# fnzhan/EMLight

Hardware: AMD Instinct MI355X
Metric: training images/sec (regression step: DenseNet-BC fwd + Sinkhorn loss + bwd + Adam) (higher is better)
Workload: dtype f32; 1 GPU; RegressionNetwork train step, BASELINE configs[1]; per_gpu_batch=64, global_batch=64, anchors=128, parallelism=single

## Files before the change

### emlight_amd/RegressionNetwork/dense_engine_bwd.py

```python
import ctypes
import os

import torch

from .. import _lib
from .._knobs import knob_choice, knob_flag


def _r16(v):
    return (v + 15) // 16 * 16


def _side_stream(dev, prio):
    if prio <= 0:
        return torch.cuda.Stream(device=dev, priority=prio)
    hip = ctypes.CDLL("libamdhip64.so")
    h = ctypes.c_void_p()
    with torch.cuda.device(dev):
        rc = hip.hipStreamCreateWithPriority(ctypes.byref(h), ctypes.c_uint(1), ctypes.c_int(prio))
    if rc != 0:
        raise RuntimeError("hipStreamCreateWithPriority failed (%d)" % rc)
    return torch.cuda.ExternalStream(h.value, device=dev)


def _masked_stream(dev, n_cu, keep):
    hip = ctypes.CDLL("libamdhip64.so")
    words = (n_cu + 31) // 32
    mask = (ctypes.c_uint32 * words)()
    for i in range(n_cu):
        if keep(i):
            mask[i // 32] |= 1 << (i % 32)
    h = ctypes.c_void_p()
    with torch.cuda.device(dev):
        rc = hip.hipExtStreamCreateWithCUMask(ctypes.byref(h), ctypes.c_uint32(words), mask)
    if rc != 0:
        raise RuntimeError("hipExtStreamCreateWithCUMask failed (%d)" % rc)
    return torch.cuda.ExternalStream(h.value, device=dev)


class _BwdBuffers:
    def gf12(self, r):
        if self.GF12[r] is None:
            self.GF12[r] = self._gf12_new()
        return self.GF12[r]

    def __init__(self, enc, ws, dev):
        f32 = dict(dtype=torch.float32, device=dev)
        self.G = [torch.zeros(blk["P"], blk["ld"], **f32) for blk in ws.blocks]
        self.GF = torch.zeros(ws.F.shape[0], ws.F.shape[1], **f32)
        maxP = ws.blocks[0]["P"]
        self.DZ = torch.empty(2, maxP, 48, **f32)
        self.ring = max(1, int(os.environ.get("EML_WGRAD_RING", 4))) if enc.overlap_wgrad(dev) else 1
        self.GF12 = [None] * self.ring
        self._gf12_new = lambda: torch.empty(maxP, 12, **f32)
        self.N12 = torch.empty(maxP, 12, **f32)
        self.TOP = torch.empty(2 * maxP * 12, **f32) if knob_flag("EML_DGRAD_TOP", True) else None
        kp, ko, g = enc.kp_max, max(enc.ko_max, 48), enc.grid_max
        self.Wd = [[torch.empty(lay["Kp"] * 48, **f32) for lay in blk["layers"]] for blk in ws.blocks]
        self.WdT = [torch.empty(blk["trans"]["Kp"] * blk["trans"]["Ko"], **f32) for blk in ws.blocks]
        self.permutes = None
        self.coef = torch.zeros(8, max(kp, ko), **f32)
        self.part2 = torch.zeros(2, g * kp * 2, dtype=torch.float64, device=dev)
        self.partW = torch.empty(g * max(kp * 48, 2 * 27 * 256, 4 * 1024), **f32)
        i32 = dict(dtype=torch.int32, device=dev)
        self.cond = [[torch.zeros(lay["Kp"], **i32) for lay in blk["layers"]] for blk in ws.blocks]
        self.condT = [torch.zeros(blk["trans"]["Kp"], **i32) for blk in ws.blocks]
        self.any_ill = torch.zeros(1, **i32)
        self.dg_grid = 128
        self.dg_scratch = torch.empty(self.dg_grid * kp, dtype=torch.float64, device=dev)
        self.side = None
        if enc.overlap_wgrad(dev):
            m = int(os.environ.get("EML_CU_SPLIT", 0))
            self.main_masked = None
            if m > 1:
                n_cu = torch.cuda.get_device_properties(dev).multi_processor_count
                self.side = _masked_stream(dev, n_cu, lambda i: i % m == m - 1)
                self.main_masked = _masked_stream(dev, n_cu, lambda i: i % m != m - 1)
            else:
                self.side = _side_stream(dev, int(os.environ.get("EML_SIDE_PRIO", 0)))
            self.partW3 = [torch.empty(g * 2 * 27 * 256, **f32) for _ in range(self.ring)]
            self.ev_ready = [torch.cuda.Event() for _ in range(self.ring)]
            self.ev_done = [None] * self.ring


def run_backward(enc, ws, x, gpooled, need_x=False, need_params=None):
    if getattr(ws, "bwd", None) is None:
        ws.bwd = _BwdBuffers(enc, ws, x.device)
    masked = getattr(ws.bwd, "main_masked", None)
    if masked is None:
        return _run_backward(enc, ws, x, gpooled, need_x, need_params)
    cur = torch.cuda.current_stream(x.device)
    masked.wait_stream(cur)
    with torch.cuda.stream(masked):
        out = _run_backward(enc, ws, x, gpooled, need_x, need_params)
    cur.wait_stream(masked)
    return out


def _run_backward(enc, ws, x, gpooled, need_x, need_params):
    L, p, st = _lib.lib(), _lib.ptr, _lib.current_stream()
    m = enc.model
    f = m.features
    if not m.training:
        raise NotImplementedError("HIP DenseNet backward is implemented for train-mode BatchNorm "
                                  "(EMLight trains and tests in train mode, train.py:42 / test.py:36-37)")
    dev = x.device
    B, _, H, W = x.shape
    G = enc._grid(dev)
    G3 = enc._grid3(dev)
    G3d = enc._tuned("EML_GRID3_DGRAD", 2 * G3 if knob_flag("EML_D3_SHORT", False) else G3)
    Gw = enc._tuned("EML_GRID_WGRAD1", G)
    Gd = enc._tuned("EML_GRID_DGRAD", G)
    Gb = min(enc.grid_max, 4 * enc._cu)
    bw = ws.bwd
    part = ws.partials
    ring = [0]
    if bw.side is not None:
        main = torch.cuda.current_stream(dev)
        st_side = ctypes.c_void_p(bw.side.cuda_stream)
        G3s = enc._tuned("EML_GRID3_SIDE", G3)
        bw.side.wait_stream(main)
    if bw.permutes is None:
        from .dense_engine import _PermuteTable
        bw.permutes = _PermuteTable()
    items = []
    for bi_, blk_ in enumerate(ws.blocks):
        mod_ = getattr(f, "denseblock%d" % (bi_ + 1))
        for l_, lay_ in enumerate(blk_["layers"]):
            items.append((getattr(mod_, "denselayer%d" % (l_ + 1)).conv1.weight, bw.Wd[bi_][l_], 2, 48, lay_["Cin"],
                          lay_["Kp"], 48))
        tr_ = blk_["trans"]
        items.append((getattr(f, "transition%d" % (bi_ + 1)).conv.weight, bw.WdT[bi_], 2, tr_["Cout"], blk_["Ctot"],
                      tr_["Kp"], tr_["Ko"]))
    bw.permutes.launch(L, st, items)
    params = enc.param_list()
    if need_params is None:
        need_params = [True] * len(params)
    from .._dist import grad_slot
    grads = {}
    for q, need in zip(params, need_params):
        slot = grad_slot(q) if need else None
        grads[id(q)] = slot if slot is not None else torch.empty_like(q)
    gr = lambda q: p(grads[id(q)])
    coefs = [tuple(bw.coef[3 * k + i] for i in range(3)) for k in range(2)]
    cA, cB, cC = coefs[0]
    sB, sC = bw.coef[6], bw.coef[7]

    direct = knob_choice("EML_DGAMMA_DIRECT", "always", ("always", "never")) != "never"
    c3_fold = knob_flag("EML_C3_FOLD", True)
    c3_gf = knob_flag("EML_C3_GF", False)
    bw.any_ill.zero_()

    def dgamma_direct(blk, X_ld, Pin, Hin, Win, pool, DY, ld_dy, Zr, ld_z, co, Cout, conv, Cin, scale1, shift1, cond, bn):
        if not direct:
            return
        a, b, c = co if co is not None else (None, None, None)
        _lib.check(L.eml_dense_bn_dgamma_direct_f32(
            p(blk["X"]), X_ld, Pin, Hin, Win, pool, p(DY), ld_dy, p(Zr), ld_z, p(a), p(b), p(c), Cout, p(conv.weight), Cin,
            p(scale1), p(shift1), p(blk["mean"]), p(blk["istd"]), p(cond), p(bw.dg_scratch), gr(bn.weight), bw.dg_grid, st),
            "eml_dense_bn_dgamma_direct_f32")

    def finalize(R, pstride, count, bn, mean, istd, C, Cpad, coef=0, s_acc=None, src=None, c_lo=0, c_hi=None, conv=None,
                 cond=None):
        a, b, c = coefs[coef] if coef is not None else (None, None, None)
        wargs = (p(bn.bias), p(conv.weight), gr(conv.weight), conv.weight.shape[0]) if conv is not None else (None, None, None, 0)
        _lib.check(L.eml_dense_bn_bwd_finalize_f32(
            p(part if src is None else src), R, pstride, float(count), p(bn.weight), p(mean), p(istd), C, Cpad, 1,
            gr(bn.weight), gr(bn.bias), p(a), p(b), p(c),
            p(sB) if s_acc is not None else None, p(sC) if s_acc is not None else None, int(bool(s_acc)),
            c_lo, Cpad if c_hi is None else c_hi, *wargs, p(cond), p(bw.any_ill) if cond is not None else None, st),
            "eml_dense_bn_bwd_finalize_f32")

    def parr(tensors):
        return (ctypes.c_void_p * len(tensors))(*[t.data_ptr() for t in tensors])

    def materialize(Gbuf, blk, c0, n):
        _lib.check(L.eml_dense_grad_materialize_f32(p(Gbuf), blk["ld"], p(blk["X"]), blk["ld"], p(sB), p(sC), c0, n,
                                                    blk["P"], st), "eml_dense_grad_materialize_f32")

    cf, k = enc.trans_cout[-1], enc.avgpool
    ldF = ws.F.shape[1]
    _lib.check(L.eml_dense_head_pool_bwd_f32(p(gpooled), p(ws.F), ldF, cf, B, ws.hf, ws.wf, k, p(bw.GF), ldF, st),
               "eml_dense_head_pool_bwd_f32")
    dY, ld_dy = bw.GF, ldF
    nb = len(ws.blocks)
    for bi in reversed(range(nb)):
        blk, tr = ws.blocks[bi], ws.blocks[bi]["trans"]
        mod = getattr(f, "denseblock%d" % (bi + 1))
        T, LN = getattr(f, "transition%d" % (bi + 1)), getattr(f, "last_norm%d" % (bi + 1))
        P, Hb, Wb, ld, ctot = blk["P"], blk["H"], blk["W"], blk["ld"], blk["Ctot"]
        cout, Ko, kpt = tr["Cout"], tr["Ko"], tr["Kp"]
        Pn = B * (Hb // 2) * (Wb // 2)
        Gbuf = bw.G[bi]
        gl0 = sum(enc.block_layers[:bi])
        top2 = bw.TOP[:2 * P * 12].view(2, P, 12) if bw.TOP is not None else None
        _lib.check(L.eml_dense_bn_bwd_stats_f32(p(dY), ld_dy, p(tr["T"]), Ko, None, 0, 0, cout, Pn, p(tr["tmean"]),
                                                p(tr["tistd"]), p(part), Gb, st), "eml_dense_bn_bwd_stats_f32")
        finalize(Gb, 2 * cout, Pn, LN, tr["tmean"], tr["tistd"], cout, Ko, coef=0)
        _lib.check(L.eml_dense_conv1x1_bwd_weight_f32(
            p(tr["A"]), kpt, Pn, Hb // 2, Wb // 2, 0, kpt, ctot, p(tr["one"]), p(tr["zero"]), p(dY), ld_dy, p(tr["T"]),
            Ko, p(cA), p(cB), p(cC), cout, p(bw.partW), gr(T.conv.weight), G, None, None, 0, None, 0, None, None, st),
            "eml_dense_conv1x1_bwd_weight_f32")
        _lib.check(L.eml_dense_conv1x1_bwd_data_f32(
            p(dY), ld_dy, p(tr["T"]), Ko, p(cA), p(cB), p(cC), Ko, p(bw.WdT[bi]), None, ld, p(tr["scale"]),
            p(tr["shift"]), None, None, Pn, Hb, Wb, 1, kpt, p(Gbuf), ld, 0, p(part), G, p(tr["mask16"]), st),
            "eml_dense_conv1x1_bwd_data_f32")
        finalize(G, 2 * kpt, P, T.norm, blk["mean"], blk["istd"], ctot, kpt, coef=None, s_acc=False, conv=T.conv,
                 cond=bw.condT[bi])
        dgamma_direct(blk, ld, P, Hb, Wb, 1, dY, ld_dy, tr["T"], Ko, coefs[0], cout, T.conv, ctot, tr["scale"], tr["shift"],
                      bw.condT[bi], T.norm)
        def conv2_backward(l, slot, n12=False, narrow_lo=None, top=False):
            lay = blk["layers"][l]
            Lm = getattr(mod, "denselayer%d" % (l + 1))
            cin, kp, z, dz = lay["Cin"], lay["Kp"], blk["Z"][l], bw.DZ[slot]
            gsrc = (p(bw.N12), 12, 0) if n12 else (p(top2[1]), 12, 0) if top else (p(Gbuf), ld, cin)
            r = ring[0] = (ring[0] + 1) % bw.ring
            if bw.side is not None and bw.ev_done[r] is not None:
                main.wait_event(bw.ev_done[r])
            fold = (bw.side is None and c3_fold
                    and L.eml_dense_conv3x3_bwd_fused_supported(gsrc[1], gsrc[2], ld, cin) == 1)
            q = ws.drop_plan[bi][l] if ws.drop_plan is not None else 0.0
            drop = (ws.drop_key, gl0 + l, q) if q > 0 else ()
            if fold:
                fn = "eml_dense_conv3x3_bwd_fused_drop_f32" if drop else "eml_dense_conv3x3_bwd_fused_f32"
                _lib.check(getattr(L, fn)(*gsrc, p(Lm.conv2.weight), p(z), p(lay["zmean"]), p(lay["zistd"]), p(dz), B, Hb, Wb,
                                          p(part), G3d, p(blk["X"]), ld, cin, p(sB), p(sC), p(bw.gf12(r)) if c3_gf else None,
                                          p(lay["scale2"]), p(lay["shift2"]), p(bw.partW), gr(Lm.conv2.weight), *drop, st), fn)
            else:
                fn = "eml_dense_conv3x3_bwd_data_drop_f32" if drop else "eml_dense_conv3x3_bwd_data_f32"
                _lib.check(getattr(L, fn)(*gsrc, p(Lm.conv2.weight), p(z), p(lay["zmean"]), p(lay["zistd"]), p(dz), B, Hb, Wb,
                                          p(part), G3d, p(blk["X"]), ld, cin, p(sB), p(sC), p(bw.gf12(r)), *drop, st), fn)
            if fold:
                pass
            elif bw.side is None:
                _lib.check(L.eml_dense_conv3x3_bwd_weight_f32(p(bw.gf12(r)), 12, 0, p(z), p(lay["scale2"]),
                                                              p(lay["shift2"]), B, Hb, Wb, p(bw.partW),
                                                              gr(Lm.conv2.weight), G3, st),
                           "eml_dense_conv3x3_bwd_weight_f32")
            else:
                bw.ev_ready[r].record(main)
                bw.side.wait_event(bw.ev_ready[r])
                _lib.check(L.eml_dense_conv3x3_bwd_weight_f32(p(bw.gf12(r)), 12, 0, p(z), p(lay["scale2"]),
                                                              p(lay["shift2"]), B, Hb, Wb, p(bw.partW3[r]),
                                                              gr(Lm.conv2.weight), G3s, st_side),
                           "eml_dense_conv3x3_bwd_weight_f32")
                if bw.ev_done[r] is None:
                    bw.ev_done[r] = torch.cuda.Event()
                bw.ev_done[r].record(bw.side)
            finalize(G3d, 96, P, Lm.norm2, lay["zmean"], lay["zistd"], 48, 48, coef=slot)
            a, b, c = coefs[slot]
            _lib.check(L.eml_dense_conv1x1_bwd_weight_f32(
                p(blk["X"]), ld, P, Hb, Wb, 0, kp, cin, p(lay["scale1"]), p(lay["shift1"]), p(dz), 48, p(z), 48,
                p(a), p(b), p(c), 48, p(bw.partW), gr(Lm.conv1.weight), Gw, p(dz),
                *((p(Lm.conv1.weight), narrow_lo, *((p(top2[0]), 12) if top else (p(Gbuf), ld)), p(bw.N12),
                   p(bw.part2[slot])) if narrow_lo is not None
                  else (None, 0, None, 0, None, None)), st), "eml_dense_conv1x1_bwd_weight_f32")
            return Lm

        def dgrad(layers, slots, k_lo, k_hi, top=False):
            lays = [blk["layers"][l] for l in layers]
            if top:
                _lib.check(L.eml_dense_conv1x1_bwd_data_multi_top_f32(
                    parr([bw.DZ[s_] for s_ in slots]), parr([bw.Wd[bi][l_] for l_ in layers]),
                    parr([y["scale1"] for y in lays]), parr([y["shift1"] for y in lays]),
                    parr([bw.part2[s_] for s_ in slots]), (ctypes.c_int * len(layers))(*[y["Kp"] for y in lays]),
                    P, k_hi, p(Gbuf), ld, Gd, parr([y["mask"] for y in lays]), p(top2), st),
                    "eml_dense_conv1x1_bwd_data_multi_top_f32")
                return
            _lib.check(L.eml_dense_conv1x1_bwd_data_multi_f32(
                len(layers), parr([bw.DZ[s_] for s_ in slots]), None, None, None, None,
                parr([bw.Wd[bi][l_] for l_ in layers]),
                parr([y["scale1"] for y in lays]), parr([y["shift1"] for y in lays]),
                parr([bw.part2[s_] for s_ in slots]), (ctypes.c_int * len(layers))(*[y["Kp"] for y in lays]),
                None, ld, None, None, P, k_lo, k_hi, p(Gbuf), ld, Gd,
                parr([y["mask"] for y in lays]), st),
                "eml_dense_conv1x1_bwd_data_multi_f32")

        def bn1_finalize(l, Lm, slot, c_lo, c_hi, rows=None):
            lay = blk["layers"][l]
            finalize(Gd if rows is None else rows, 2 * lay["Kp"], P, Lm.norm1, blk["mean"], blk["istd"], lay["Cin"], lay["Kp"], coef=None,
                     s_acc=True, src=bw.part2[slot], c_lo=c_lo, c_hi=c_hi, conv=Lm.conv1, cond=bw.cond[bi][l])

        def bn1_direct(l, Lm, slot):
            lay = blk["layers"][l]
            dgamma_direct(blk, ld, P, Hb, Wb, 0, bw.DZ[slot], 48, None, 0, None, 48, Lm.conv1, lay["Cin"], lay["scale1"],
                          lay["shift1"], bw.cond[bi][l], Lm.norm1)

        l = len(blk["layers"]) - 1
        have_top = False
        while l >= 0:
            if l >= 1:
                la, lb = l, l - 1
                cin_a, cin_b = blk["layers"][la]["Cin"], blk["layers"][lb]["Cin"]
                Lma = conv2_backward(la, 0, narrow_lo=cin_b, top=have_top)
                bn1_finalize(la, Lma, 0, cin_b, cin_a, rows=Gw)
                Lmb = conv2_backward(lb, 1, n12=True)
                to_top = (top2 is not None and lb >= 2 and blk["layers"][la]["mask"] is not None and bw.side is None
                          and cin_b >= 24 and cin_b % 4 == 0)
                dgrad([la, lb], [0, 1], 0, cin_b, top=to_top)
                have_top = to_top
                bn1_finalize(la, Lma, 0, 0, cin_b)
                bn1_finalize(lb, Lmb, 1, 0, blk["layers"][lb]["Kp"])
                bn1_direct(la, Lma, 0)
                bn1_direct(lb, Lmb, 1)
                l -= 2
            else:
                Lm0 = conv2_backward(l, 0)
                dgrad([l], [0], 0, blk["layers"][l]["Cin"])
                bn1_finalize(l, Lm0, 0, 0, blk["layers"][l]["Kp"])
                bn1_direct(l, Lm0, 0)
                l -= 1
        c0b = blk["C0"]
        norm0_fused = bi == 0 and knob_flag("EML_NORM0_FUSED", True) and c0b % 4 == 0 and c0b <= 32
        if not norm0_fused:
            materialize(Gbuf, blk, 0, c0b)
        dY, ld_dy = Gbuf, ld
    b0 = ws.blocks[0]
    c0 = enc.c_init
    if norm0_fused:
        _lib.check(L.eml_dense_norm0_bwd_stats_f32(p(dY), ld_dy, p(ws.Y0), c0, p(ws.scale0), p(ws.shift0), p(sB), p(sC), c0,
                                                   b0["P"], p(ws.mean0), p(ws.istd0), p(part), Gb, st),
                   "eml_dense_norm0_bwd_stats_f32")
    else:
        _lib.check(L.eml_dense_bn_bwd_stats_f32(p(dY), ld_dy, p(ws.Y0), c0, p(b0["X"]), b0["ld"], 1, c0, b0["P"],
                                                p(ws.mean0), p(ws.istd0), p(part), Gb, st), "eml_dense_bn_bwd_stats_f32")
    finalize(Gb, 2 * c0, b0["P"], f.norm0, ws.mean0, ws.istd0, c0, _r16(c0), coef=0)
    if norm0_fused:
        _lib.check(L.eml_dense_conv0_bwd_weight_fused_f32(p(x), p(dY), ld_dy, p(ws.Y0), c0, p(ws.scale0), p(ws.shift0), p(sB),
                                                          p(sC), p(cA), p(cB), p(cC), B, H, W, p(bw.partW),
                                                          gr(f.conv0.weight), G, st), "eml_dense_conv0_bwd_weight_fused_f32")
    else:
        _lib.check(L.eml_dense_conv0_bwd_weight_f32(p(x), p(dY), ld_dy, p(b0["X"]), b0["ld"], p(ws.Y0), c0, p(cA), p(cB),
                                                    p(cC), B, H, W, p(bw.partW), gr(f.conv0.weight), G, st),
                   "eml_dense_conv0_bwd_weight_f32")
    dx = None
    if need_x:
        dx = torch.empty(B, 3, H, W, dtype=torch.float32, device=dev)
        X1 = (None, 0) if norm0_fused else (p(b0["X"]), b0["ld"])
        _lib.check(L.eml_dense_conv0_bwd_data_f32(p(dY), ld_dy, *X1, p(ws.Y0), c0, p(ws.scale0), p(ws.shift0), p(sB), p(sC),
                                                  p(cA), p(cB), p(cC), p(f.conv0.weight), B, H, W, p(dx), st),
                   "eml_dense_conv0_bwd_data_f32")
    if bw.side is not None:
        main.wait_stream(bw.side)
    return dx, [grads[id(q)] for q in params]
```

### emlight_amd/_lib.py

```python
import ctypes
import os
import threading

_HERE = os.path.dirname(os.path.abspath(__file__))
LIB_PATH = os.environ.get("EML_LIB_PATH") or os.path.join(_HERE, "libemlight_hip.so")

_f32p = ctypes.c_void_p
_i32p = ctypes.c_void_p
_f64p = ctypes.c_void_p
_stream = ctypes.c_void_p
_int = ctypes.c_int
_u64 = ctypes.c_ulonglong

ABI_VERSION = 31

SIGNATURES = {
    "eml_abi_version": (_int, []),
    "eml_last_error": (ctypes.c_char_p, []),
    "eml_sg_rasterise_f32": (_int, [_f32p, _f32p, _f32p, _f32p, _int, _int, _int, _int, _stream]),
    "eml_sg_rasterise_ex_f32": (_int, [_f32p, _f32p, _f32p, _f32p, _int, _int, _int, _int, _int, ctypes.c_void_p, _stream]),
    "eml_sg_rasterise_bwd_colors_f32": (_int, [_f32p, _f32p, _f32p, _f32p, _int, _int, _int, _int, _stream]),
    "eml_emd_anchor_cost_f32": (_int, [_f32p, _f32p, _int, _stream]),
    "eml_sinkhorn_schedule_f32": (_int, [_f32p, _f32p, ctypes.c_long, ctypes.c_double, ctypes.c_double, _int,
                                         ctypes.c_double, _f32p, _f32p, _i32p, _f32p, _stream]),
    "eml_sinkhorn_work_floats": (ctypes.c_size_t, [_int, _int]),
    "eml_sinkhorn_fwd_f32": (_int, [_f32p, _f32p, _f32p, _f32p, _f32p, _f32p, ctypes.c_double, ctypes.c_double, _int,
                                    ctypes.c_double, _f32p, _f32p, _i32p, _f32p, _f32p, _f32p, _f32p, _f32p, _int, _int,
                                    _stream]),
    "eml_sinkhorn_fwd_ex_f32": (_int, [_f32p, _f32p, _f32p, _f32p, _f32p, _f32p, ctypes.c_double, ctypes.c_double, _int,
                                       ctypes.c_double, _f32p, _f32p, _i32p, _f32p, _f32p, _f32p, _f32p, _f32p, _int, _int,
                                       _int, _stream]),
    "eml_sinkhorn_fwd_rho_f32": (_int, [_f32p, _f32p, _f32p, _f32p, _f32p, _f32p, ctypes.c_double, ctypes.c_double, _int,
                                        ctypes.c_double, _f32p, _f32p, _i32p, _f32p, _f32p, _f32p, _f32p, _f32p, _int, _int,
                                        _int, ctypes.c_double, _f32p, _stream]),
    "eml_sinkhorn_bwd_f32": (_int, [_f32p, _f32p, _f32p, _int, _int, _stream]),
    "eml_sinkhorn_dim_work_floats": (ctypes.c_size_t, [_int, _int, _int]),
    "eml_sinkhorn_fwd_dim_f32": (_int, [_f32p, _f32p, _f32p, _f32p, _f32p, _f32p, ctypes.c_double, ctypes.c_double, _int,
                                        ctypes.c_double, _f32p, _f32p, _i32p, _f32p, _f32p, _f32p, _f32p, _f32p, _int, _int,
                                        _int, _int, ctypes.c_double, _f32p, _stream]),
    "eml_sinkhorn_schedule_dim_f32": (_int, [_f32p, _f32p, ctypes.c_long, _int, ctypes.c_double, ctypes.c_double, _int,
                                             ctypes.c_double, _f32p, _f32p, _i32p, _f32p, _stream]),
    "eml_sinkhorn_bwd_weights_f32": (_int, [_f32p, _f32p, _f32p, _f32p, _int, _int, _stream]),
    "eml_l1_pairs_partial_doubles": (ctypes.c_size_t, [_int]),
    "eml_l1_pairs_fwd_f32": (_int, [_int, ctypes.c_void_p, ctypes.c_void_p, ctypes.c_void_p, ctypes.c_void_p, ctypes.c_void_p,
                                    ctypes.c_void_p, _f64p, _f32p, _stream]),
    "eml_l1_pairs_bwd_f32": (_int, [_int, ctypes.c_void_p, ctypes.c_void_p, ctypes.c_void_p, ctypes.c_void_p, ctypes.c_void_p,
                                    ctypes.c_void_p, _f32p, ctypes.c_void_p, ctypes.c_void_p, ctypes.c_void_p, _stream]),
    "eml_colsum_partial_doubles": (ctypes.c_size_t, [_int]),
    "eml_colsum_f32": (_int, [_f32p, ctypes.c_long, _int, _f64p, _f32p, _stream]),
    "eml_gt_anchor_index_i32": (_int, [_f32p, _int, _int, _int, _i32p, _stream]),
    "eml_gt_parametrise_f64": (_int, [_f32p, _i32p, _i32p, _int, _int, _int, _int, _f32p, _f32p, _f32p, _stream]),
    "eml_pano_crop_f32": (_int, [ctypes.c_void_p, _int, _int, _int, _int, _int, _int, ctypes.c_double, ctypes.c_double, _f64p,
                                 ctypes.c_double, _f64p, _f32p, _stream]),
    "eml_pano_resize_area_f32": (_int, [_f32p, _int, _int, _int, _int, _int, ctypes.c_double, _f64p, _f32p, _stream]),
    "eml_tonemap_work_floats": (ctypes.c_size_t, [_int]),
    "eml_tonemap_f32": (_int, [_f32p, _int, ctypes.c_long, _int, ctypes.c_double, ctypes.c_double, ctypes.c_double, _f32p,
                               _int, _f32p, _f32p, _i32p, _f32p, ctypes.c_void_p, _stream]),
    "eml_sphere_tap_table_f32": (_int, [_f32p, _int, _int, _int, _int, _i32p, _f32p, _stream]),
    "eml_sphere_im2col_f32": (_int, [_f32p, _i32p, _f32p, _f32p, _int, _int, _int, _int, _stream]),
    "eml_sphere_col2im_f32": (_int, [_f32p, _i32p, _i32p, _f32p, _f32p, _int, _int, _int, _int, _stream]),
    "eml_sphere_conv_fwd_fused_f32": (_int, [_f32p, _i32p, _f32p, _f32p, _f32p, _f32p, _int, _int, _int, _int, _int, _int,
                                             _stream]),
    "eml_sphere_conv_fwd_fused_ex_f32": (_int, [_f32p, _i32p, _f32p, _f32p, _f32p, _f32p, _int, _int, _int, _int, _int, _int,
                                                _f32p, ctypes.c_float, _int, _stream]),
    "eml_sphere_conv_small_supported": (_int, [_int, _int]),
    "eml_sphere_conv_small_fwd_f32": (_int, [_f32p, _i32p, _f32p, _f32p, _f32p, _f32p, _int, _int, _int, _int, _int,
                                             ctypes.c_float, _stream]),
    "eml_sphere_conv_small_wgrad_partial_floats": (ctypes.c_size_t, [_int, _int, _int, _int]),
    "eml_sphere_conv_small_wgrad_f32": (_int, [_f32p, _i32p, _f32p, _f32p, _f32p, ctypes.c_float, _f32p, _f32p, _f32p, _int,
                                               _int, _int, _int, _int, _stream]),
    "eml_sphere_conv_small_da9_f32": (_int, [_f32p, _f32p, ctypes.c_float, _f32p, _f32p, ctypes.c_long, _int, _int, _stream]),
    "eml_spade_norm_modulate_up2_fwd_f32": (_int, [_f32p, _f32p, _f32p, _int, _int, _int, _int, ctypes.c_float, _f32p, _f32p,
                                                   _stream]),
    "eml_spade_norm_modulate_bwd_cols_f32": (_int, [_f32p, _f32p, _f32p, _f32p, _f32p, _int, _int, _int, _int, _int,
                                                    ctypes.c_float, _f32p, _f32p, _f32p, _int, _stream]),
    "eml_sg_rasterise_bwd_work_floats": (ctypes.c_size_t, [_int, _int, _int, _int]),
    "eml_sg_rasterise_bwd_colors_ex_f32": (_int, [_f32p, _f32p, _f32p, _f32p, _f32p, _int, _int, _int, _int, _int, _stream]),
    "eml_sg_rasterise_bwd_full_work_floats": (ctypes.c_size_t, [_int, _int, _int, _int]),
    "eml_sg_rasterise_bwd_f32": (_int, [_f32p, _f32p, _f32p, _f32p, _f32p, _f32p, _f32p, _f32p, _int, _int, _int, _int, _int,
                                        _stream]),
    "eml_sphere_conv_narrow_supported": (_int, [_int, _int]),
    "eml_sphere_conv_narrow_fwd_f32": (_int, [_f32p, _i32p, _f32p, _f32p, _f32p, _f32p, _int, _int, _int, _int, _int, _stream]),
    "eml_sphere_conv_narrow_dgrad_f32": (_int, [_f32p, _i32p, _f32p, _int, _f32p, _f32p, _int, _int, _int, _int, _int, _stream]),
    "eml_sphere_conv_narrow_wgrad_partial_floats": (ctypes.c_size_t, [_int, _int, _int, _int]),
    "eml_sphere_conv_narrow_wgrad_f32": (_int, [_f32p, _i32p, _f32p, _f32p, _f32p, _f32p, _int, _int, _int, _int, _int, _stream]),
    "eml_sphere_conv_narrow_scratch_floats": (ctypes.c_size_t, [_int, _int]),
    "eml_sphere_conv_narrow_fwd2_f32": (_int, [_f32p, _i32p, _f32p, _f32p, _f32p, _f32p, _f32p, _int, _int, _int, _int, _int, _stream]),
    "eml_sphere_conv_narrow_wgrad2_partial_floats": (ctypes.c_size_t, [_int, _int, _int]),
    "eml_sphere_conv_narrow_dgrad2_f32": (_int, [_f32p, _i32p, _f32p, _int, ctypes.c_void_p, _f32p, _f32p, _f32p, _int, _int, _int,
                                                 _int, _int, _int, _stream]),
    "eml_sphere_conv_narrow_wgrad2_f32": (_int, [_f32p, _i32p, _f32p, _int, ctypes.c_void_p, _f32p, _f32p, _f32p, _f32p, _int, _int,
                                                 _int, _int, _int, _stream]),
    "eml_sphere_conv_spade_supported": (_int, [_int, _int, ctypes.c_long]),
    "eml_sphere_conv_spade_fwd_f32": (_int, [_f32p, _i32p, _f32p, _f32p, _f32p, _f32p, _f32p, _f32p, _f32p, _f32p, _int, _int,
                                             _int, _int, _int, _int, ctypes.c_float, _int, _stream]),
    "eml_spade_norm_modulate_bwd_y_f32": (_int, [_f32p, _f32p, _f32p, _f32p, _f32p, _f32p, _int, _int, _int, _int, _int,
                                                 ctypes.c_float, _f32p, _f32p, _f32p, _int, _stream]),
    "eml_bn_bwd_apply_up2_f32": (_int, [_f32p, _f32p, _int, _int, _int, _int, _f32p, _f32p, _f32p, _f32p, _stream]),
    "eml_spectral_norm_scratch_floats": (ctypes.c_size_t, [_int, _int]),
    "eml_spectral_norm_w2_f32": (_int, [_f32p, _f32p, _f32p, _int, ctypes.c_float, _f32p, _f32p, _f32p, _f32p, _int, _int,
                                        _stream]),
    "eml_spectral_norm_w2_bwd_f32": (_int, [_f32p, _f32p, _f32p, _f32p, _f32p, _f32p, _f32p, _int, _int, _stream]),
    "eml_spectral_norm_w2_batch_f32": (_int, [_int, ctypes.c_void_p, ctypes.c_void_p, ctypes.c_void_p, _int, ctypes.c_float,
                                              ctypes.c_void_p, ctypes.c_void_p, ctypes.c_void_p, ctypes.c_void_p, ctypes.c_void_p,
                                              ctypes.c_void_p, _stream]),
    "eml_spade_heads_w2_f32": (_int, [_f32p, _f32p, _f32p, _f32p, _f32p, _f32p, _int, _int, _int, _stream]),
    "eml_instance_norm_act_fwd_f32": (_int, [_f32p, _f32p, _f32p, _int, _int, _int, _int, ctypes.c_float, ctypes.c_float,
                                             _stream]),
    "eml_instance_norm_act_bwd_f32": (_int, [_f32p, _f32p, _f32p, _f32p, _int, _int, _int, _int, ctypes.c_float, _stream]),
    "eml_sphere_conv_dgrad_fused_f32": (_int, [_f32p, _i32p, _f32p, _i32p, _int, _f32p, _f32p, _int, _int, _int, _int, _int,
                                               _int, _stream]),
    "eml_sphere_conv_lowres_variant": (_int, [_int, _int, _int, _int]),
    "eml_sphere_conv_lowres_table_i32": (_int, [_i32p, _i32p, _i32p, _int, _int, _stream]),
    "eml_sphere_conv_lowres_partial_floats": (ctypes.c_size_t, [ctypes.c_long, _int, _int]),
    "eml_sphere_conv_lowres_f32": (_int, [_f32p, _i32p, _f32p, _i32p, _int, _i32p, _int, _f32p, _f32p, _f32p, _f32p, _int, _int,
                                          _int, _int, _int, _int, _f32p, ctypes.c_float, _stream]),
    "eml_sphere_conv_wgrad_partial_floats": (ctypes.c_size_t, [_int, _int, _int]),
    "eml_sphere_conv_wgrad_fused_f32": (_int, [_f32p, _i32p, _f32p, _f32p, _f32p, _f32p, _int, _int, _int, _int, _int, _int,
                                               _stream]),
    "eml_spade_modulate_fwd_f32": (_int, [_f32p, _int, _f32p, _int, _f32p, _int, ctypes.c_long, _int, ctypes.c_float,
                                          _stream]),
    "eml_spade_modulate_bwd_f32": (_int, [_f32p, _int, _f32p, _int, _f32p, _int, _f32p, _int, _f32p, _int, ctypes.c_long,
                                          _int, ctypes.c_float, _stream]),
    "eml_bn_stats_f32": (_int, [_f32p, _int, ctypes.c_long, _int, _f32p, _int, _stream]),
    "eml_bn_fold_f64": (_int, [_f32p, _int, _int, _f32p, _stream]),
    "eml_bn_finalize_f32": (_int, [_f32p, _int, ctypes.c_float, ctypes.c_float, _f32p, _f32p, _f32p, _f32p, _stream]),
    "eml_spade_norm_modulate_fwd_f32": (_int, [_f32p, _int, _f32p, _int, _f32p, _int, ctypes.c_long, _int, ctypes.c_float,
                                               _f32p, _f32p, _stream]),
    "eml_bn_bwd_apply_f32": (_int, [_f32p, _int, _f32p, _int, ctypes.c_long, _int, _f32p, _f32p, _f32p, _f32p, _int,
                                    _stream]),
    "eml_dense_conv0_fwd_f32": (_int, [_f32p, _f32p, _f32p, _int, _int, _int, _int, _int, _f32p, _int, _stream]),
    "eml_dense_conv0_fwd_mfma_f32": (_int, [_f32p, _f32p, _f32p, _int, _int, _int, _int, _int, _f32p, _int, _stream]),
    "eml_dense_bn_apply_f32": (_int, [_f32p, _int, _f32p, _int, _int, ctypes.c_long, _f32p, _f32p, _int, _f32p,
                                      _int, _stream]),
    "eml_dense_bn_prepare_f32": (_int, [_f32p, _int, _int, _int, _int, ctypes.c_double, _f32p, _f32p, _f32p, _f32p,
                                        _f32p, _f32p, _f32p, _int, _int, ctypes.c_float, ctypes.c_float, _int,
                                        _f32p, _f32p, _stream]),
    "eml_dense_permute_w1_f32": (_int, [_f32p, _int, _int, _int, _f32p, _stream]),
    "eml_dense_permute_w2_f32": (_int, [_f32p, _int, _f32p, _stream]),
    "eml_dense_permute_batch_f32": (_int, [ctypes.c_void_p, _int, _stream]),
    "eml_dense_conv1x1_fwd_f32": (_int, [_f32p, _int, ctypes.c_long, _int, _int, _int, _int, _f32p, _f32p, _f32p,
                                         _int, _f32p, _int, _f32p, _int, ctypes.c_void_p, _stream]),
    "eml_dense_conv3x3_fwd_f32": (_int, [_f32p, _f32p, _f32p, _f32p, _f32p, _int, _int, _int, _int, _int, _f32p,
                                         _int, _stream]),
    "eml_dense_permute_w2_tp_f32": (_int, [_f32p, _f32p, _stream]),
    "eml_dense_conv3x3_fwd_tp_supported": (_int, [_int, _int, _int]),
    "eml_dense_conv3x3_fwd_tp_f32": (_int, [_f32p, _f32p, _f32p, _f32p, _f32p, _int, _int, _int, _int, _int, _int, _f32p,
                                            _int, _stream]),
    "eml_dense_conv3x3_fwd_drop_f32": (_int, [_f32p, _f32p, _f32p, _f32p, _f32p, _int, _int, _int, _int, _int, _f32p,
                                              _int, _u64, _int, ctypes.c_double, _stream]),
    "eml_dense_conv3x3_fwd_tp_drop_f32": (_int, [_f32p, _f32p, _f32p, _f32p, _f32p, _int, _int, _int, _int, _int, _int, _f32p,
                                                 _int, _u64, _int, ctypes.c_double, _stream]),
    "eml_dense_dropout_mask_u16": (_int, [_u64, _int, ctypes.c_double, ctypes.c_long, ctypes.c_void_p, _stream]),
    "eml_dense_pool_act_f32": (_int, [_f32p, _int, _int, _int, _int, _int, _f32p, _f32p, _f32p, _int, ctypes.c_void_p,
                                      _stream]),
    "eml_dense_head_pool_fwd_f32": (_int, [_f32p, _int, _int, _int, _int, _int, _int, _f32p, _stream]),
    "eml_dense_conv3x3_bwd_data_f32": (_int, [_f32p, _int, _int, _f32p, _f32p, _f32p, _f32p, _f32p, _int, _int, _int,
                                              _f32p, _int, _f32p, _int, _int, _f32p, _f32p, _f32p, _stream]),
    "eml_dense_conv3x3_bwd_fused_supported": (_int, [_int, _int, _int, _int]),
    "eml_dense_conv3x3_bwd_fused_f32": (_int, [_f32p, _int, _int, _f32p, _f32p, _f32p, _f32p, _f32p, _int, _int, _int, _f64p, _int,
                                               _f32p, _int, _int, _f32p, _f32p, _f32p, _f32p, _f32p, _f32p, _f32p, _stream]),
    "eml_dense_conv3x3_bwd_data_drop_f32": (_int, [_f32p, _int, _int, _f32p, _f32p, _f32p, _f32p, _f32p, _int, _int, _int,
                                                   _f32p, _int, _f32p, _int, _int, _f32p, _f32p, _f32p, _u64, _int,
                                                   ctypes.c_double, _stream]),
    "eml_dense_conv3x3_bwd_fused_drop_f32": (_int, [_f32p, _int, _int, _f32p, _f32p, _f32p, _f32p, _f32p, _int, _int, _int,
                                                    _f64p, _int, _f32p, _int, _int, _f32p, _f32p, _f32p, _f32p, _f32p, _f32p,
                                                    _f32p, _u64, _int, ctypes.c_double, _stream]),
    "eml_dense_conv3x3_bwd_weight_f32": (_int, [_f32p, _int, _int, _f32p, _f32p, _f32p, _int, _int, _int, _f32p,
                                                _f32p, _int, _stream]),
    "eml_dense_bn_bwd_finalize_f32": (_int, [_f32p, _int, _int, ctypes.c_double, _f32p, _f32p, _f32p, _int, _int,
                                             _int, _f32p, _f32p, _f32p, _f32p, _f32p, _f32p, _f32p, _int, _int, _int,
                                             _f32p, _f32p, _f32p, _int, _i32p, _i32p, _stream]),
    "eml_dense_bn_dgamma_direct_f32": (_int, [_f32p, _int, ctypes.c_long, _int, _int, _int, _f32p, _int, _f32p, _int,
                                              _f32p, _f32p, _f32p, _int, _f32p, _int, _f32p, _f32p, _f32p, _f32p, _i32p,
                                              _f32p, _f32p, _int, _stream]),
    "eml_dense_conv1x1_bwd_weight_f32": (_int, [_f32p, _int, ctypes.c_long, _int, _int, _int, _int, _int, _f32p,
                                                _f32p, _f32p, _int, _f32p, _int, _f32p, _f32p, _f32p, _int, _f32p,
                                                _f32p, _int, _f32p, _f32p, _int, _f32p, _int, _f32p, _f32p, _stream]),
    "eml_dense_conv1x1_bwd_narrow_f32": (_int, [_f32p, _f32p, _int, _int, _f32p, _int, _f32p, _f32p, _f32p, _f32p,
                                                ctypes.c_long, _f32p, _int, _f32p, _f32p, _int, _int, _stream]),
    "eml_dense_permute_w1_bwd_f32": (_int, [_f32p, _int, _int, _int, _int, _f32p, _stream]),
    "eml_dense_conv1x1_bwd_data_f32": (_int, [_f32p, _int, _f32p, _int, _f32p, _f32p, _f32p, _int, _f32p, _f32p,
                                              _int, _f32p, _f32p, _f32p, _f32p, ctypes.c_long, _int, _int, _int,
                                              _int, _f32p, _int, _int, _f32p, _int, ctypes.c_void_p, _stream]),
    "eml_dense_conv1x1_bwd_data_multi_f32": (_int, [_int] + [ctypes.c_void_p] * 10 + [_f32p, _int, _f32p, _f32p,
                                                    ctypes.c_long, _int, _int, _f32p, _int, _int, ctypes.c_void_p,
                                                    _stream]),
    "eml_dense_conv1x1_bwd_data_multi_top_f32": (_int, [ctypes.c_void_p] * 6 + [ctypes.c_long, _int, _f32p, _int, _int,
                                                        ctypes.c_void_p, _f32p, _stream]),
    "eml_dense_grad_materialize_f32": (_int, [_f32p, _int, _f32p, _int, _f32p, _f32p, _int, _int, ctypes.c_long,
                                              _stream]),
    "eml_dense_bn_bwd_stats_f32": (_int, [_f32p, _int, _f32p, _int, _f32p, _int, _int, _int, ctypes.c_long, _f32p,
                                          _f32p, _f32p, _int, _stream]),
    "eml_dense_norm0_bwd_stats_f32": (_int, [_f32p, _int, _f32p, _int, _f32p, _f32p, _f32p, _f32p, _int, ctypes.c_long, _f32p, _f32p,
                                             ctypes.c_void_p, _int, _stream]),
    "eml_dense_conv0_bwd_weight_fused_f32": (_int, [_f32p, _f32p, _int, _f32p, _int, _f32p, _f32p, _f32p, _f32p, _f32p, _f32p, _f32p,
                                                    _int, _int, _int, _f32p, _f32p, _int, _stream]),
    "eml_dense_conv0_bwd_weight_f32": (_int, [_f32p, _f32p, _int, _f32p, _int, _f32p, _int, _f32p, _f32p, _f32p,
                                              _int, _int, _int, _f32p, _f32p, _int, _stream]),
    "eml_dense_conv0_bwd_data_f32": (_int, [_f32p, _int, _f32p, _int, _f32p, _int, _f32p, _f32p, _f32p, _f32p, _f32p, _f32p,
                                            _f32p, _f32p, _int, _int, _int, _f32p, _stream]),
    "eml_dense_head_pool_bwd_f32": (_int, [_f32p, _f32p, _int, _int, _int, _int, _int, _int, _f32p, _int, _stream]),
}

_lock = threading.Lock()
_lib = None


class EmlightHipError(RuntimeError):
    pass


def lib():
    global _lib
    if _lib is not None:
        return _lib
    with _lock:
        if _lib is not None:
            return _lib
        if not os.path.exists(LIB_PATH):
            raise EmlightHipError(
                "libemlight_hip.so not found at %s -- build it with "
                "`python -c 'import __graft_entry__ as g; g.build()'` or `make -C emlight_amd/csrc`. "
                "There is no CPU fallback." % LIB_PATH)
        handle = ctypes.CDLL(LIB_PATH)
        for name, (res, args) in SIGNATURES.items():
            try:
                fn = getattr(handle, name)
            except AttributeError as e:
                raise EmlightHipError("libemlight_hip.so lacks symbol %s" % name) from e
            fn.restype, fn.argtypes = res, args
        got = handle.eml_abi_version()
        if got != ABI_VERSION:
            raise EmlightHipError("libemlight_hip.so has ABI version %d, this binding expects %d -- rebuild it "
                                  "(make -C emlight_amd/csrc)" % (got, ABI_VERSION))
        _lib = handle
    from . import _gemm_selection
    _gemm_selection.ensure_if_requested()
    return _lib


_DEBUG_SYNC = bool(os.environ.get("EML_DEBUG_SYNC"))


def check(rc, what):
    if rc != 0:
        msg = lib().eml_last_error()
        raise EmlightHipError("%s failed (rc=%d): %s" % (what, rc, msg.decode() if msg else "?"))
    if _DEBUG_SYNC:
        import sys
        import torch
        sys.stderr.write("[eml] %s ... " % what)
        sys.stderr.flush()
        torch.cuda.synchronize()
        sys.stderr.write("ok\n")


def ptr(t):
    if t is None:
        return None
    return ctypes.c_void_p(t.data_ptr())


def current_stream():
    import torch
    return ctypes.c_void_p(torch.cuda.current_stream().cuda_stream)


def require_gpu_tensor(t, name, dtype=None):
    import torch
    if not isinstance(t, torch.Tensor) or not t.is_cuda:
        raise EmlightHipError("%s must be a tensor on the MI355X (got %s); there is no CPU path"
                              % (name, getattr(t, "device", type(t))))
    if t.dtype != (dtype or torch.float32):
        raise EmlightHipError("%s must be %s (got %s)" % (name, dtype or torch.float32, t.dtype))
    return t.contiguous()
```

### emlight_amd/csrc/dense_bwd.hip

```cpp
#include "eml_common.h"
#include "eml_dropout.h"

#include <cstdint>
#include <cstdlib>
#include <type_traits>

namespace {

using f32x4 = __attribute__((ext_vector_type(4))) float;

__device__ __forceinline__ f32x4 mfma16(float a, float b, f32x4 c) {
  return __builtin_amdgcn_mfma_f32_16x16x4f32(a, b, c, 0, 0, 0);
}
__device__ __forceinline__ float f4c(const float4& v, int t) { return t == 0 ? v.x : t == 1 ? v.y : t == 2 ? v.z : v.w; }
__device__ __forceinline__ double shfl_xor_d(double v, int m) { return __shfl_xor(v, m, 64); }

constexpr int kTH = 8, kTW = 32, kHH = kTH + 2, kHW = kTW + 2;

constexpr int kPSG = 14;
constexpr int kBD = 512;
constexpr int kGRows = 2;
constexpr int kGPass = kHH / kGRows;

template <bool FUSE, bool WIDE, int TH, bool DROP = false>
// ... 949 lines not shown
          const int b2 = t2 / (ty_n * tx_n), rem2 = t2 - b2 * (ty_n * tx_n);
#ifndef EML_C3_NOZDMA
#pragma unroll
          for (int it = 0; it < kZI; ++it) z_dma(it, b2, (rem2 / tx_n) * kTH, (rem2 % tx_n) * kTW, cur ^ 1);
#endif
          __builtin_amdgcn_sched_barrier(0);
        }
        const bool pin = 4 * (ks & 7) < (ks < 8 ? xl0 : xl1);
        float bv[3];
#pragma unroll
        for (int n = 0; n < 3; ++n) bv[n] = pin ? fmaf(bz[ks & 1][n], scb[n], shb[n]) : 0.f;
#pragma unroll
        for (int i = 0; i < NT; ++i) {
          const float a = (i < 3 || r < 12) ? av[ks & 1][i] : 0.f;
#pragma unroll
          for (int n = 0; n < 3; ++n) accw[i][n] = mfma16(a, bv[n], accw[i][n]);
        }
        if (ks == 2 || ks == 4 || ks == 6) {
          const int n = (ks - 2) >> 1;
          float l1[4] = {0.f, 0.f, 0.f, 0.f}, l2[4] = {0.f, 0.f, 0.f, 0.f};
#pragma unroll
          for (int m = 0; m < 2; ++m) {
            const float4 z = *reinterpret_cast<const float4*>(zc + (kTW * wave + 16 * m + r) * kZS + 16 * n + 4 * kk);
#pragma unroll
            for (int g = 0; g < 4; ++g) {
              const float v = pv[m] ? acc[m][n][g] : 0.f;
              l1[g] += v;
              l2[g] = fmaf(v, f4c(z, g), l2[g]);
            }
          }
#pragma unroll
          for (int g = 0; g < 4; ++g) {
            const float t1 = eml::row16_sum(l1[g]), t2 = eml::row16_sum(l2[g]);
            if (r == 0) {
              double* d = red + (wave * 48 + 16 * n + 4 * kk + g) * 2;
              d[0] += (double)t1;
              d[1] += (double)t2;
            }
          }
        } else if (ks >= 8 && ks < 14) {
          const int si = ks - 8, m = si / 3, n = si - 3 * m;
          if (pv[m])
            *reinterpret_cast<float4*>(DZ + prow[m] + 16 * n + 4 * kk) =
                make_float4(acc[m][n][0], acc[m][n][1], acc[m][n][2], acc[m][n][3]);
        }
        __builtin_amdgcn_sched_barrier(0);
      }
    };
    if (role == 0) phase_b(std::integral_constant<int, 3>{});
    else phase_b(std::integral_constant<int, 4>{});
    EML_C3_STAMP(2);
    eml::lds_barrier();
    EML_C3_STAMP(3);
#ifdef EML_STAMPS
    st_acc[4] += 1;
#endif
    cur ^= 1;
  }
#ifdef EML_STAMPS
  if (tid == 0)
    for (int i = 0; i < 5; ++i) atomicAdd(&eml_c3_stamps[i], st_acc[i]);
#endif
  asm volatile("s_waitcnt vmcnt(0)" ::: "memory");
  __syncthreads();
  float* wsum = smem;
  for (int w8 = 0; w8 < 8; ++w8) {
    if (wave == w8) {
#pragma unroll
      for (int i = 0; i < 4; ++i)
        if (i < 3 + role) {
#pragma unroll
          for (int n = 0; n < 3; ++n)
#pragma unroll
            for (int g = 0; g < 4; ++g) {
              float* q = wsum + ((((3 * role + i) * 3 + n) * 16 + 4 * kk + g) * 16 + r);
              *q = ((w8 & 3) == 0 ? 0.f : *q) + accw[i][n][g];
            }
        }
    }
    __syncthreads();
  }
  for (int e = tid; e < 21 * 256; e += 512) partialW[(size_t)blockIdx.x * (21 * 256) + e] = wsum[e];
  if (tid < 48) {
    double t1 = 0.0, t2 = 0.0;
#pragma unroll
    for (int w8 = 0; w8 < 8; ++w8) {
      t1 += red[(w8 * 48 + tid) * 2 + 0];
      t2 += red[(w8 * 48 + tid) * 2 + 1];
    }
    partials[(size_t)blockIdx.x * 96 + 2 * tid + 0] = t1;
    partials[(size_t)blockIdx.x * 96 + 2 * tid + 1] = (double)zistd[tid] * (t2 - (double)zmean[tid] * t1);
  }
}


__global__ __launch_bounds__(256) void bn_bwd_finalize_kernel(
    const double* __restrict__ partials, int R, int pstride, double count, const float* __restrict__ gamma,
    const float* __restrict__ mean, const float* __restrict__ istd, int C, int Cpad, int training,
    float* __restrict__ dgamma, float* __restrict__ dbeta, float* __restrict__ cA, float* __restrict__ cB,
    float* __restrict__ cC, float* __restrict__ sB, float* __restrict__ sC, int s_accumulate, int c_lo, int c_hi,
    const float* __restrict__ beta, const float* __restrict__ Wc, const float* __restrict__ dWc, int w_rows,
    int* __restrict__ cond , int* __restrict__ any_cond ) {
  const int lane = threadIdx.x & 63, wave = threadIdx.x >> 6;
  const int c = c_lo + blockIdx.x * 4 + wave;
  if (c >= Cpad || c >= c_hi) return;
  float a = 0.f, b = 0.f, d = 0.f;
  if (c < C) {
    double S1 = 0.0, S2 = 0.0;
    for (int g = lane; g < R; g += 64) {
      S1 += partials[(size_t)g * pstride + 2 * c];
      S2 += partials[(size_t)g * pstride + 2 * c + 1];
    }
    double Q = 0.0;
    if (Wc)
      for (int o = lane; o < w_rows; o += 64) Q += (double)Wc[(size_t)o * C + c] * (double)dWc[(size_t)o * C + c];
#pragma unroll
    for (int o = 32; o > 0; o >>= 1) {
      S1 += __shfl_xor(S1, o, 64);
      S2 += __shfl_xor(S2, o, 64);
      Q += __shfl_xor(Q, o, 64);
    }
    if (Wc) {
      const double ga0 = gamma[c], bs = (double)beta[c] * S1, num = Q - bs;
      S2 = fabs(ga0) >= 1e-12 ? num / ga0 : 0.0;
      if (cond && lane == 0) {
        const int ill = fabs(ga0) < 1e-3 * fabs((double)beta[c]) || ga0 == 0.0;
        cond[c] = ill;
        if (ill && any_cond) *any_cond = 1;
      }
    }
    if (lane == 0) {
      dgamma[c] = (float)S2;
      dbeta[c] = (float)S1;
    }
    const double ga = gamma[c], is = istd[c], mu = mean[c];
    a = (float)(ga * is);
    if (training) {
      b = (float)(-ga * is * is * S2 / count);
      d = (float)(-ga * is * S1 / count + ga * is * is * S2 / count * mu);
    }
  }
  if (lane != 0) return;
  if (cA) {
    cA[c] = a;
    cB[c] = b;
    cC[c] = d;
  }
  if (sB) {
    sB[c] = (s_accumulate ? sB[c] : 0.f) + b;
    sC[c] = (s_accumulate ? sC[c] : 0.f) + d;
  }
}

__global__ __launch_bounds__(256) void reduce_rows_kernel(const float* __restrict__ partial, int R, size_t row_stride,
                                                          int mode, int dim0, int dim1, int n0,
                                                          float* __restrict__ out) {
  __shared__ double red[4][64];
  const int tid = threadIdx.x, e = blockIdx.x * 64 + (tid & 63), slice = tid >> 6;
  size_t src = 0, dst = 0;
  bool valid = false;
  if (mode == 0) {
    const int k = e / 48, o = e - 48 * k;
    valid = k < dim0 && o < dim1;
    src = (size_t)e;
    dst = (size_t)(n0 + o) * dim0 + k;
  } else if (mode == 1) {
    const int o = e & 15, ci = (e >> 4) & 15, pair = e >> 8, tap = pair / 3, mc = pair - 3 * tap;
    valid = pair < 27 && o < 12;
    src = (size_t)e;
    dst = (size_t)(o * 48 + 16 * mc + ci) * 9 + tap;
  } else if (mode == 3) {
    const int j = e & 15, i = (e >> 4) & 15, tn = e >> 8, t = tn / 3, n = tn - 3 * t, row = 16 * t + i;
    valid = tn < 21 && row < 108;
    src = (size_t)e;
    dst = (size_t)((row % 12) * 48 + 16 * n + j) * 9 + row / 12;
  } else {
    const int t = e >> 5, o = e & 31;
    valid = t < 27 && o < dim1;
    src = (size_t)e;
    dst = (size_t)o * 27 + t;
  }
  double s = 0.0;
  if (valid) {
#pragma unroll 8
    for (int r = slice; r < R; r += 4) s += (double)partial[(size_t)r * row_stride + src];
  }
  red[slice][tid & 63] = s;
  __syncthreads();
  if (slice == 0 && valid) out[dst] = (float)((red[0][tid] + red[1][tid]) + (red[2][tid] + red[3][tid]));
}

struct NarrowArgs {
  const float* W1;
  const float* G;
  float* N12;
  double* partials;
  int Cin, k_lo, ldg;
};
template <bool POOL, bool NARROW = false, int VEC = 2>
__global__ __launch_bounds__(256, (NARROW || VEC == 4) ? 2 : 1) void conv1x1_bwd_weight_kernel(
    const float* __restrict__ X, int ldx, int P, int Hin, int Win, int Kp, const float* __restrict__ scale1,
    const float* __restrict__ shift1, const float* __restrict__ DY, int ld_dy, const float* __restrict__ Zr,
    int ld_z, const float* __restrict__ cA, const float* __restrict__ cB, const float* __restrict__ cC, int n_valid,
    int n_load ,
    float* __restrict__ partial ,
    float* __restrict__ dz_out ,
    NarrowArgs na) {
  __shared__ __attribute__((aligned(16))) float dz_l[2][64 * 48];
  const int tid = threadIdx.x, lane = tid & 63, wave = tid >> 6;
  const int r = lane & 15, kk = lane >> 4;
  static_assert(VEC == 2 || (VEC == 4 && !POOL), "float4 operand: dense layers only");
  constexpr int GW = 16 * VEC;
  constexpr int MAXG = VEC == 2 ? 3 : 2;
  const int ngroups = (Kp + GW - 1) / GW;
  float nsk[4] = {0.f, 0.f, 0.f, 0.f}, ntk[4] = {0.f, 0.f, 0.f, 0.f};
  double ns1[4] = {0.0, 0.0, 0.0, 0.0};
  const int kq = min(kk, 2);
  if constexpr (NARROW) {
#pragma unroll
    for (int g = 0; g < 4; ++g) {
      nsk[g] = kk < 3 ? scale1[na.k_lo + 4 * kq + g] : 0.f;
      ntk[g] = kk < 3 ? shift1[na.k_lo + 4 * kq + g] : 0.f;
    }
  }

  float sv[MAXG][VEC], tv[MAXG][VEC];
  int coff[MAXG];
  bool gv[MAXG];
#pragma unroll
  for (int i = 0; i < MAXG; ++i) {
    const int cg = wave + 4 * i;
    const int ch = GW * cg + VEC * r;
    gv[i] = cg < ngroups && ch < Kp;
    coff[i] = gv[i] ? ch : 0;
#pragma unroll
    for (int t = 0; t < VEC; ++t) {
      sv[i][t] = gv[i] ? scale1[ch + t] : 0.f;
      tv[i][t] = gv[i] ? shift1[ch + t] : 0.f;
    }
  }
  const int spix = tid >> 2, sq = tid & 3;
  __shared__ __attribute__((aligned(16))) float co_l[3 * 48];
  __shared__ float wn_l[NARROW ? 12 * 64 : 1];
  constexpr bool CO_LDS = NARROW || VEC == 4;
  float4 sa_r[CO_LDS ? 1 : 3], sb_r[CO_LDS ? 1 : 3], sc_r[CO_LDS ? 1 : 3];
  if constexpr (CO_LDS) {
    if (tid < 48) {
      const bool v = tid < n_valid;
      co_l[tid] = v ? cA[tid] : 0.f;
      co_l[48 + tid] = v ? cB[tid] : 0.f;
      co_l[96 + tid] = v ? cC[tid] : 0.f;
    }
  } else {
#pragma unroll
    for (int j = 0; j < 3; ++j) {
      const int col = 4 * (sq + 4 * j);
      float a[4], b[4], c[4];
#pragma unroll
      for (int e = 0; e < 4; ++e) {
        const bool v = col + e < n_valid;
        a[e] = v ? cA[col + e] : 0.f;
        b[e] = v ? cB[col + e] : 0.f;
        c[e] = v ? cC[col + e] : 0.f;
      }
      sa_r[j] = make_float4(a[0], a[1], a[2], a[3]);
      sb_r[j] = make_float4(b[0], b[1], b[2], b[3]);
      sc_r[j] = make_float4(c[0], c[1], c[2], c[3]);
    }
  }
  if constexpr (NARROW) {
    for (int e = tid; e < 12 * 64; e += 256) {
      const int st = e >> 6, l = e & 63, rr = l & 15, k4 = l >> 4;
      wn_l[e] = rr < 12 ? na.W1[(size_t)(4 * st + k4) * na.Cin + na.k_lo + rr] : 0.f;
    }
  }
  __syncthreads();
  f32x4 acc[MAXG][VEC][3];
#pragma unroll
  for (int i = 0; i < MAXG; ++i)
#pragma unroll
    for (int t = 0; t < VEC; ++t)
#pragma unroll
      for (int n = 0; n < 3; ++n) acc[i][t][n] = f32x4{0.f, 0.f, 0.f, 0.f};

  const int Wo = Win >> 1, Ho = Hin >> 1;
  const int nchunks = (P + 63) >> 6;
  const int ngw = (ngroups > wave) ? (ngroups - wave + 3) >> 2 : 0;

  float4 rdy[3], rzr[3];
  bool rpv = false;
  int rp = 0;
  auto stage_load = [&](int chunk) {
    const int p = chunk * 64 + spix;
    rpv = chunk < nchunks && p < P;
    const size_t pc = rpv ? p : 0;
    rp = (int)pc;
#pragma unroll
    for (int j = 0; j < 3; ++j) {
      const int col = 4 * (sq + 4 * j);
      const bool cv = col < n_load;
      rdy[j] = cv ? *reinterpret_cast<const float4*>(DY + pc * ld_dy + col) : make_float4(0.f, 0.f, 0.f, 0.f);
      rzr[j] = cv ? *reinterpret_cast<const float4*>(Zr + pc * ld_z + col) : make_float4(0.f, 0.f, 0.f, 0.f);
    }
  };
  auto stage_write = [&](float* dzb) {
#pragma unroll
    for (int j = 0; j < 3; ++j) {
      const int col = 4 * (sq + 4 * j);
      float4 sa, sb, sc;
      if constexpr (CO_LDS) {
        sa = *reinterpret_cast<const float4*>(co_l + col);
        sb = *reinterpret_cast<const float4*>(co_l + 48 + col);
        sc = *reinterpret_cast<const float4*>(co_l + 96 + col);
      } else {
        sa = sa_r[j];
        sb = sb_r[j];
        sc = sc_r[j];
      }
      float4 v;
      v.x = rpv ? fmaf(sa.x, rdy[j].x, fmaf(sb.x, rzr[j].x, sc.x)) : 0.f;
      v.y = rpv ? fmaf(sa.y, rdy[j].y, fmaf(sb.y, rzr[j].y, sc.y)) : 0.f;
      v.z = rpv ? fmaf(sa.z, rdy[j].z, fmaf(sb.z, rzr[j].z, sc.z)) : 0.f;
      v.w = rpv ? fmaf(sa.w, rdy[j].w, fmaf(sb.w, rzr[j].w, sc.w)) : 0.f;
      *reinterpret_cast<float4*>(dzb + spix * 48 + col) = v;
      if (dz_out && rpv) *reinterpret_cast<float4*>(dz_out + (size_t)rp * 48 + col) = v;
    }
  };
  auto chunk_loop = [&](auto ngw_c) {
    constexpr int NGW = decltype(ngw_c)::value;
#ifdef EML_WGRAD_DEEP
    constexpr int UQ = POOL ? 1 : 2;
    constexpr int NBUF = POOL ? 2 : 4;
#else
    constexpr int UQ = POOL ? 1 : (VEC == 4 ? 2 : 4);
    constexpr int NBUF = 2;
#endif
    constexpr int NS = POOL ? 4 : 1;
    constexpr int NB = 16 / UQ;
    constexpr int AHEAD = NBUF - 1;
    using xv_t = std::conditional_t<VEC == 2, float2, float4>;
    xv_t xr[NBUF][UQ][NGW > 0 ? NGW : 1][NS];
    auto load_batch = [&](int chunk, int q0, xv_t (&dst)[UQ][NGW > 0 ? NGW : 1][NS]) {
#pragma unroll
      for (int u = 0; u < UQ; ++u) {
        const int pc = min(chunk * 64 + 4 * (q0 + u) + kk, P - 1);
        const float* xp;
        if constexpr (POOL) {
          const int b = pc / (Ho * Wo), rem = pc - b * (Ho * Wo);
          const int oy = rem / Wo, ox = rem - oy * Wo;
          xp = X + ((size_t)(b * Hin + 2 * oy) * Win + 2 * ox) * ldx;
        } else {
          xp = X + (size_t)pc * ldx;
        }
#pragma unroll
        for (int i = 0; i < NGW; ++i)
#pragma unroll
          for (int sub = 0; sub < NS; ++sub)
            dst[u][i][sub] = *reinterpret_cast<const xv_t*>(xp + ((sub >> 1) * (size_t)Win + (sub & 1)) * ldx + coff[i]);
      }
    };
    stage_load(blockIdx.x);
    stage_write(dz_l[0]);
    if constexpr (NGW > 0) {
#pragma unroll
      for (int a = 0; a < AHEAD; ++a) load_batch(min((int)blockIdx.x, nchunks - 1), a * UQ, xr[a]);
    }
    __syncthreads();
    int it = 0;
    for (int chunk = blockIdx.x; chunk < nchunks; chunk += gridDim.x, ++it) {
      const float* dzb = dz_l[it & 1];
      stage_load(chunk + gridDim.x);
      float2 nx[2], ng[2];
      const int pn = chunk * 64 + 16 * wave + r;
      if constexpr (NARROW) {
        const size_t pc = (size_t)min(pn, P - 1);
        const float* xs = X + pc * ldx + na.k_lo + 4 * kq;
        const float* gs = na.G + pc * na.ldg + (na.ldg == 12 ? 0 : na.k_lo) + 4 * kq;
        nx[0] = *reinterpret_cast<const float2*>(xs);
        nx[1] = *reinterpret_cast<const float2*>(xs + 2);
        ng[0] = *reinterpret_cast<const float2*>(gs);
        ng[1] = *reinterpret_cast<const float2*>(gs + 2);
      }
      if constexpr (NGW > 0) {
        float bzq[2][3];
#pragma unroll
        for (int n = 0; n < 3; ++n) bzq[0][n] = dzb[kk * 48 + 16 * n + r];
#pragma unroll
        for (int bi = 0; bi < NB; ++bi) {
          const int q0 = bi * UQ;
          if (bi + AHEAD < NB)
            load_batch(chunk, q0 + AHEAD * UQ, xr[(bi + AHEAD) % NBUF]);
          else
            load_batch(min(chunk + (int)gridDim.x, nchunks - 1), (bi + AHEAD - NB) * UQ, xr[(bi + AHEAD) % NBUF]);
          __builtin_amdgcn_sched_barrier(0);
#pragma unroll
          for (int u = 0; u < UQ; ++u) {
            const int pl = 4 * (q0 + u) + kk;
            const bool pvu = chunk * 64 + pl < P;
            float bz[3];
#pragma unroll
            for (int n = 0; n < 3; ++n) bz[n] = bzq[(q0 + u) & 1][n];
            if (q0 + u + 1 < 16) {
#pragma unroll
              for (int n = 0; n < 3; ++n) bzq[(q0 + u + 1) & 1][n] = dzb[(pl + 4) * 48 + 16 * n + r];
            }
#pragma unroll
            for (int i = 0; i < NGW; ++i) {
              float av[VEC];
#pragma unroll
              for (int t = 0; t < VEC; ++t) av[t] = 0.f;
#pragma unroll
              for (int sub = 0; sub < NS; ++sub) {
                const xv_t xv = xr[bi % NBUF][u][i][sub];
                av[0] += fmaxf(fmaf(xv.x, sv[i][0], tv[i][0]), 0.f);
                av[1] += fmaxf(fmaf(xv.y, sv[i][1], tv[i][1]), 0.f);
                if constexpr (VEC == 4) {
                  av[2] += fmaxf(fmaf(xv.z, sv[i][2], tv[i][2]), 0.f);
                  av[3] += fmaxf(fmaf(xv.w, sv[i][3], tv[i][3]), 0.f);
                }
              }
#pragma unroll
              for (int t = 0; t < VEC; ++t) {
                if constexpr (POOL) av[t] *= 0.25f;
                if (!pvu) av[t] = 0.f;
              }
#pragma unroll
              for (int n = 0; n < 3; ++n)
#pragma unroll
                for (int t = 0; t < VEC; ++t) acc[i][t][n] = mfma16(av[t], bz[n], acc[i][t][n]);
            }
          }
          __builtin_amdgcn_sched_barrier(0);
        }
      }
      if constexpr (NARROW) {
        asm volatile("" ::"v"(ng[0].x), "v"(ng[0].y), "v"(ng[1].x), "v"(ng[1].y), "v"(nx[0].x), "v"(nx[0].y), "v"(nx[1].x), "v"(nx[1].y));
        f32x4 an = f32x4{0.f, 0.f, 0.f, 0.f};
#pragma unroll
        for (int st = 0; st < 12; ++st) an = mfma16(wn_l[st * 64 + lane], dzb[(16 * wave + r) * 48 + 4 * st + kk], an);
        const bool nv = pn < P && kk < 3;
        const float xg[4] = {nx[0].x, nx[0].y, nx[1].x, nx[1].y}, gg[4] = {ng[0].x, ng[0].y, ng[1].x, ng[1].y};
        float o4[4];
#pragma unroll
        for (int g = 0; g < 4; ++g) {
          const float dam = (nv && fmaf(xg[g], nsk[g], ntk[g]) > 0.f) ? an[g] : 0.f;
          o4[g] = fmaf(nsk[g], dam, gg[g]);
          ns1[g] += (double)dam;
        }
        if (nv) *reinterpret_cast<float4*>(na.N12 + ((unsigned)pn * 12u + 4u * (unsigned)kk)) = make_float4(o4[0], o4[1], o4[2], o4[3]);
      }
      stage_write(dz_l[(it + 1) & 1]);
      eml::lds_barrier();
    }
  };
  switch (ngw) {
    case 0: chunk_loop(std::integral_constant<int, 0>{}); break;
    case 1: chunk_loop(std::integral_constant<int, 1>{}); break;
    case 2: chunk_loop(std::integral_constant<int, 2>{}); break;
    default: chunk_loop(std::integral_constant<int, MAXG>{}); break;
  }
  float* out = partial + (size_t)blockIdx.x * Kp * 48;
#pragma unroll
  for (int i = 0; i < MAXG; ++i) {
    const int cg = wave + 4 * i;
#pragma unroll
    for (int t = 0; t < VEC; ++t)
#pragma unroll
      for (int g = 0; g < 4; ++g) {
        const int ch = GW * cg + VEC * (4 * kk + g) + t;
        if (cg < ngroups && ch < Kp) {
#pragma unroll
          for (int n = 0; n < 3; ++n) out[(size_t)ch * 48 + 16 * n + r] = acc[i][t][n][g];
        }
      }
  }
  if constexpr (NARROW) {
    __syncthreads();
    double* red = reinterpret_cast<double*>(&dz_l[0][0]);
#pragma unroll
    for (int g = 0; g < 4; ++g) {
#pragma unroll
      for (int o = 1; o < 16; o <<= 1) ns1[g] += shfl_xor_d(ns1[g], o);
      if (r == 0 && kk < 3) red[wave * 12 + 4 * kk + g] = ns1[g];
    }
    __syncthreads();
    if (tid < 12) {
      double* dst = na.partials + ((size_t)blockIdx.x * Kp + na.k_lo + tid) * 2;
      dst[0] = (red[tid] + red[12 + tid]) + (red[24 + tid] + red[36 + tid]);
      dst[1] = 0.0;
    }
  }
}

template <bool POOL, bool RES , int NCH = 4>
__global__ __launch_bounds__(256) void conv1x1_bwd_data_kernel(
    const float* __restrict__ DY, int ld_dy, const float* __restrict__ Zr, int ld_z, const float* __restrict__ cA,
    const float* __restrict__ cB, const float* __restrict__ cC, int Ko, const float* __restrict__ Wd,
    const float* __restrict__ X, int ldx, const float* __restrict__ scale1, const float* __restrict__ shift1,
    const float* __restrict__ mean, const float* __restrict__ istd, int P, int Hin, int Win, int Kp,
    float* __restrict__ Gd, int ldg, int accumulate, double* __restrict__ partials ) {
  extern __shared__ __attribute__((aligned(16))) float smem[];
  double* sacc = reinterpret_cast<double*>(smem);
  const int tid = threadIdx.x, lane = tid & 63, wave = tid >> 6;
  const int r = lane & 15, kk = lane >> 4;
  for (int e = tid; e < 4 * Kp * 2; e += 256) sacc[e] = 0.0;
  __syncthreads();
  double* my = sacc + (size_t)wave * Kp * 2;
  const int nnt = Kp >> 4, njo = Ko >> 4;
  const int ntiles = (P + 255) >> 8;
  const int Wo = Win >> 1, Ho = Hin >> 1;

  for (int tile = blockIdx.x; tile < ntiles; tile += gridDim.x) {
    const int p0 = tile * 256 + wave * 64;
    long prow[4];
    size_t pin[4];
#pragma unroll
    for (int m = 0; m < 4; ++m) {
      prow[m] = min(p0 + 16 * m + r, P - 1);
      if constexpr (POOL) {
        const int b = (int)(prow[m] / (Ho * Wo)), rem = (int)(prow[m] - (long)b * (Ho * Wo));
        const int oy = rem / Wo, ox = rem - oy * Wo;
        pin[m] = (size_t)(b * Hin + 2 * oy) * Win + 2 * ox;
      } else {
        pin[m] = (size_t)prow[m];
      }
    }
    auto load_dz = [&](int jo, float4 (&dz)[4]) {
      const int ch = 16 * jo + 4 * kk;
      const float4 a4 = *reinterpret_cast<const float4*>(cA + ch);
      const float4 b4 = *reinterpret_cast<const float4*>(cB + ch);
      const float4 c4 = *reinterpret_cast<const float4*>(cC + ch);
#pragma unroll
      for (int m = 0; m < 4; ++m) {
        const float4 dy = *reinterpret_cast<const float4*>(DY + prow[m] * ld_dy + ch);
        const float4 zr = *reinterpret_cast<const float4*>(Zr + prow[m] * ld_z + ch);
        dz[m].x = fmaf(a4.x, dy.x, fmaf(b4.x, zr.x, c4.x));
        dz[m].y = fmaf(a4.y, dy.y, fmaf(b4.y, zr.y, c4.y));
        dz[m].z = fmaf(a4.z, dy.z, fmaf(b4.z, zr.z, c4.z));
        dz[m].w = fmaf(a4.w, dy.w, fmaf(b4.w, zr.w, c4.w));
      }
    };
    float4 dzr[3][4];
    if constexpr (RES) {
#pragma unroll
      for (int jo = 0; jo < 3; ++jo) load_dz(jo, dzr[jo]);
    }
    for (int nt0 = 0; nt0 < nnt; nt0 += NCH) {
      f32x4 acc[4][NCH];
#pragma unroll
      for (int m = 0; m < 4; ++m)
#pragma unroll
        for (int n = 0; n < NCH; ++n) acc[m][n] = f32x4{0.f, 0.f, 0.f, 0.f};
      auto mma = [&](int jo, const float4 (&dz)[4]) {
#pragma unroll
        for (int n = 0; n < NCH; ++n) {
          const int nt = min(nt0 + n, nnt - 1);
          const float4 w = *reinterpret_cast<const float4*>(Wd + ((((size_t)nt * njo + jo) * 4 + kk) * 16 + r) * 4);
#pragma unroll
          for (int t = 0; t < 4; ++t)
#pragma unroll
            for (int m = 0; m < 4; ++m) acc[m][n] = mfma16(f4c(w, t), f4c(dz[m], t), acc[m][n]);
        }
      };
      if constexpr (RES) {
#pragma unroll
        for (int jo = 0; jo < 3; ++jo) mma(jo, dzr[jo]);
      } else {
        for (int jo = 0; jo < njo; ++jo) {
          float4 dz[4];
          load_dz(jo, dz);
          mma(jo, dz);
        }
      }
#pragma unroll
      for (int n = 0; n < NCH; ++n) {
        const int nt = nt0 + n;
        if (nt < nnt) {
          const int k4 = 16 * nt + 4 * kk;
          const float4 sk = *reinterpret_cast<const float4*>(scale1 + k4);
          const float4 tk = *reinterpret_cast<const float4*>(shift1 + k4);
          const float4 mu = *reinterpret_cast<const float4*>(mean + k4);
          const float4 is = *reinterpret_cast<const float4*>(istd + k4);
          float l1[4] = {0.f, 0.f, 0.f, 0.f}, l2[4] = {0.f, 0.f, 0.f, 0.f};
#pragma unroll
          for (int m = 0; m < 4; ++m) {
            if (p0 + 16 * m + r < P) {
              const float da[4] = {acc[m][n][0], acc[m][n][1], acc[m][n][2], acc[m][n][3]};
              constexpr int NSUB = POOL ? 4 : 1;
#pragma unroll
              for (int sub = 0; sub < NSUB; ++sub) {
                const size_t pi = pin[m] + (sub >> 1) * (size_t)Win + (sub & 1);
                const float4 xv = *reinterpret_cast<const float4*>(X + pi * ldx + k4);
                float4* gp = reinterpret_cast<float4*>(Gd + pi * ldg + k4);
                float4 g = accumulate ? *gp : make_float4(0.f, 0.f, 0.f, 0.f);
                const float f = POOL ? 0.25f : 1.0f;
                const float d0 = (fmaf(xv.x, sk.x, tk.x) > 0.f) ? f * da[0] : 0.f;
                const float d1 = (fmaf(xv.y, sk.y, tk.y) > 0.f) ? f * da[1] : 0.f;
                const float d2 = (fmaf(xv.z, sk.z, tk.z) > 0.f) ? f * da[2] : 0.f;
                const float d3 = (fmaf(xv.w, sk.w, tk.w) > 0.f) ? f * da[3] : 0.f;
                g.x = fmaf(sk.x, d0, g.x);
                g.y = fmaf(sk.y, d1, g.y);
                g.z = fmaf(sk.z, d2, g.z);
                g.w = fmaf(sk.w, d3, g.w);
                *gp = g;
                l1[0] += d0;
                l1[1] += d1;
                l1[2] += d2;
                l1[3] += d3;
                l2[0] = fmaf(d0, (xv.x - mu.x) * is.x, l2[0]);
                l2[1] = fmaf(d1, (xv.y - mu.y) * is.y, l2[1]);
                l2[2] = fmaf(d2, (xv.z - mu.z) * is.z, l2[2]);
                l2[3] = fmaf(d3, (xv.w - mu.w) * is.w, l2[3]);
              }
            }
          }
#pragma unroll
          for (int g = 0; g < 4; ++g) {
            l1[g] = eml::row16_sum(l1[g]);
            l2[g] = eml::row16_sum(l2[g]);
            if (r == 0) {
              my[2 * (k4 + g)] += (double)l1[g];
              my[2 * (k4 + g) + 1] += (double)l2[g];
            }
          }
        }
      }
    }
  }
  __syncthreads();
  for (int e = tid; e < Kp * 2; e += 256)
    partials[(size_t)blockIdx.x * Kp * 2 + e] =
        (sacc[e] + sacc[(size_t)Kp * 2 + e]) + (sacc[(size_t)2 * Kp * 2 + e] + sacc[(size_t)3 * Kp * 2 + e]);
}

template <int MT, int NCH, bool ACC , bool MASKED = false, int NJO = 0>
__global__ __launch_bounds__(256, 2) void transition_bwd_data_kernel(
    const float* __restrict__ DY, int ld_dy, const float* __restrict__ Zr, int ld_z, const float* __restrict__ cA,
    const float* __restrict__ cB, const float* __restrict__ cC, int Ko, const float* __restrict__ Wd,
    const float* __restrict__ X, int ldx, const float* __restrict__ scale1, const float* __restrict__ shift1,
    const float* __restrict__ mean, const float* __restrict__ istd, int P, int Hin, int Win, int Kp,
    float* __restrict__ Gd, int ldg, double* __restrict__ partials ,
    const unsigned short* __restrict__ mask16) {
  extern __shared__ __attribute__((aligned(16))) float smem[];
// ... 129 lines not shown
          const float4 c4 = *reinterpret_cast<const float4*>(co_l + 2 * Ko + ch);
          float4 dz[MT];
#pragma unroll
          for (int m = 0; m < MT; ++m) {
            dz[m].x = fmaf(a4.x, ry[m].x, fmaf(b4.x, rz[m].x, c4.x));
            dz[m].y = fmaf(a4.y, ry[m].y, fmaf(b4.y, rz[m].y, c4.y));
            dz[m].z = fmaf(a4.z, ry[m].z, fmaf(b4.z, rz[m].z, c4.z));
            dz[m].w = fmaf(a4.w, ry[m].w, fmaf(b4.w, rz[m].w, c4.w));
          }
          group_step(jo, dz);
        }
      }
      if constexpr (MASKED && !ACC) {
        float l1n[NCH][4];
        float4 skn[NCH];
#pragma unroll
        for (int n = 0; n < NCH; ++n) {
          skn[n] = *reinterpret_cast<const float4*>(vec_l + 16 * min(nt0 + n, nnt - 1) + 4 * kk);
#pragma unroll
          for (int g = 0; g < 4; ++g) l1n[n][g] = 0.f;
        }
        const int piece = lane & 7;
        const bool col_ok = nt0 + (piece >> 2) < nnt;
#pragma unroll
        for (int m = 0; m < MT; ++m) {
#pragma unroll
          for (int sub = 0; sub < 4; ++sub) {
#pragma unroll
            for (int n = 0; n < NCH; ++n) {
              const unsigned b = pv[m] ? mk[m][n] >> (4 * sub) : 0u;
              const float d0 = (b & 1u) ? 0.25f * acc[m][n][0] : 0.f, d1 = (b & 2u) ? 0.25f * acc[m][n][1] : 0.f;
              const float d2 = (b & 4u) ? 0.25f * acc[m][n][2] : 0.f, d3 = (b & 8u) ? 0.25f * acc[m][n][3] : 0.f;
              *reinterpret_cast<f32x4*>(stg + r * 36 + 16 * n + 4 * kk) = f32x4{skn[n].x * d0, skn[n].y * d1, skn[n].z * d2, skn[n].w * d3};
              if (nt0 + n < nnt) {
                l1n[n][0] += d0;
                l1n[n][1] += d1;
                l1n[n][2] += d2;
                l1n[n][3] += d3;
              }
            }
            __builtin_amdgcn_fence(__ATOMIC_RELEASE, "wavefront");
            __builtin_amdgcn_wave_barrier();
            __builtin_amdgcn_fence(__ATOMIC_ACQUIRE, "wavefront");
            const size_t suboff = ((size_t)(sub >> 1) * Win + (sub & 1)) * (size_t)ldg + 16 * nt0 + 4 * piece;
#pragma unroll
            for (int h = 0; h < 2; ++h) {
              const f32x4 v = *reinterpret_cast<const f32x4*>(stg + ((lane >> 3) + 8 * h) * 36 + 4 * piece);
              if (pvx[m][h] && col_ok) *reinterpret_cast<f32x4*>(Gd + pinx[m][h] * ldg + suboff) = v;
            }
            __builtin_amdgcn_fence(__ATOMIC_RELEASE, "wavefront");
            __builtin_amdgcn_wave_barrier();
            __builtin_amdgcn_fence(__ATOMIC_ACQUIRE, "wavefront");
          }
        }
#pragma unroll
        for (int n = 0; n < NCH; ++n) {
          if (nt0 + n < nnt) {
            const int k4 = 16 * (nt0 + n) + 4 * kk;
#pragma unroll
            for (int g = 0; g < 4; ++g) {
              const float t1 = eml::row16_sum(l1n[n][g]);
              if (r == 0) my[2 * (k4 + g)] += (double)t1;
            }
          }
        }
      } else {
#pragma unroll
      for (int n = 0; n < NCH; ++n) {
        const int nt = nt0 + n;
        if (nt < nnt) {
          const int k4 = 16 * nt + 4 * kk;
          const float4 sk = *reinterpret_cast<const float4*>(vec_l + k4);
          const float4 tk = *reinterpret_cast<const float4*>(vec_l + Kp + k4);
          const float4 mu = *reinterpret_cast<const float4*>(vec_l + 2 * Kp + k4);
          const float4 is = *reinterpret_cast<const float4*>(vec_l + 3 * Kp + k4);
          float l1[4] = {0.f, 0.f, 0.f, 0.f}, l2[4] = {0.f, 0.f, 0.f, 0.f};
#pragma unroll
          for (int m = 0; m < MT; ++m) {
            const float da0 = 0.25f * acc[m][n][0], da1 = 0.25f * acc[m][n][1];
            const float da2 = 0.25f * acc[m][n][2], da3 = 0.25f * acc[m][n][3];
#pragma unroll
            for (int sub = 0; sub < 4; ++sub) {
              float4 g = make_float4(0.f, 0.f, 0.f, 0.f);
              if constexpr (ACC) g = gs[m][n][sub];
              float d0, d1, d2, d3;
              float4 x = make_float4(0.f, 0.f, 0.f, 0.f);
              if constexpr (MASKED) {
                const unsigned b = pv[m] ? mk[m][n] >> (4 * sub) : 0u;
                d0 = (b & 1u) ? da0 : 0.f;
                d1 = (b & 2u) ? da1 : 0.f;
                d2 = (b & 4u) ? da2 : 0.f;
                d3 = (b & 8u) ? da3 : 0.f;
              } else {
                x = xv[m][n][sub];
                d0 = (pv[m] && fmaf(x.x, sk.x, tk.x) > 0.f) ? da0 : 0.f;
                d1 = (pv[m] && fmaf(x.y, sk.y, tk.y) > 0.f) ? da1 : 0.f;
                d2 = (pv[m] && fmaf(x.z, sk.z, tk.z) > 0.f) ? da2 : 0.f;
                d3 = (pv[m] && fmaf(x.w, sk.w, tk.w) > 0.f) ? da3 : 0.f;
              }
              g.x = fmaf(sk.x, d0, g.x);
              g.y = fmaf(sk.y, d1, g.y);
              g.z = fmaf(sk.z, d2, g.z);
              g.w = fmaf(sk.w, d3, g.w);
              if (pv[m]) {
                const size_t pi = pin[m] + (sub >> 1) * (size_t)Win + (sub & 1);
                *reinterpret_cast<float4*>(Gd + pi * ldg + k4) = g;
              }
              l1[0] += d0;
              l1[1] += d1;
              l1[2] += d2;
              l1[3] += d3;
              if constexpr (!MASKED) {
                l2[0] = fmaf(d0, (x.x - mu.x) * is.x, l2[0]);
                l2[1] = fmaf(d1, (x.y - mu.y) * is.y, l2[1]);
                l2[2] = fmaf(d2, (x.z - mu.z) * is.z, l2[2]);
                l2[3] = fmaf(d3, (x.w - mu.w) * is.w, l2[3]);
              }
            }
          }
#pragma unroll
          for (int g = 0; g < 4; ++g) {
            l1[g] = eml::row16_sum(l1[g]);
            if constexpr (!MASKED) l2[g] = eml::row16_sum(l2[g]);
            if (r == 0) {
              my[2 * (k4 + g)] += (double)l1[g];
              if constexpr (!MASKED) my[2 * (k4 + g) + 1] += (double)l2[g];
            }
          }
        }
      }
      }
    }
  }
  __syncthreads();
  for (int e = tid; e < Kp * 2; e += 256)
    partials[(size_t)blockIdx.x * Kp * 2 + e] =
        (sacc[e] + sacc[(size_t)Kp * 2 + e]) + (sacc[(size_t)2 * Kp * 2 + e] + sacc[(size_t)3 * Kp * 2 + e]);
}

struct BwdLayer {
  const float* DZ;
  const float* Zr;
  const float* cA;
  const float* cB;
  const float* cC;
  const float* Wd;
  const float* scale1;
  const float* shift1;
  double* partials;
  int Kp;
};

template <int NL, int MT , bool RAW = false ,
          bool MASKED = false, bool TOP = false>
__global__ __launch_bounds__(256, 2) void conv1x1_bwd_data_multi_kernel(BwdLayer L0, BwdLayer L1,
                                                                        const float* __restrict__ X, int ldx,
                                                                        const float* __restrict__ mean,
                                                                        const float* __restrict__ istd, int P,
                                                                        int k_lo, int k_hi, float* __restrict__ Gd,
                                                                        int ldg, int KpMax,
                                                                        const unsigned long long* __restrict__ M0,
                                                                        const unsigned long long* __restrict__ M1,
                                                                        float* __restrict__ Top) {
  extern __shared__ __attribute__((aligned(16))) float smem[];
  double* sacc = reinterpret_cast<double*>(smem);
  float* vec_l = reinterpret_cast<float*>(sacc + (size_t)NL * 4 * KpMax * 2);
  const int tid = threadIdx.x, lane = tid & 63, wave = tid >> 6;
  const int r = lane & 15, kk = lane >> 4;
  const BwdLayer Ls[2] = {L0, L1};
  for (int e = tid; e < NL * 4 * KpMax * 2; e += 256) sacc[e] = 0.0;
  for (int e = tid; e < KpMax; e += 256) {
    vec_l[e] = MASKED ? 0.f : mean[e];
    vec_l[KpMax + e] = MASKED ? 0.f : istd[e];
#pragma unroll
    for (int j = 0; j < NL; ++j) {
      vec_l[(2 + 2 * j) * KpMax + e] = e < Ls[j].Kp ? Ls[j].scale1[e] : 0.f;
      vec_l[(3 + 2 * j) * KpMax + e] = e < Ls[j].Kp ? Ls[j].shift1[e] : 0.f;
    }
  }
  __syncthreads();
  constexpr int TP = 64 * MT;
  const int ntiles = (P + TP - 1) / TP;
  const int nt_lo = k_lo >> 4, nt_hi = (k_hi + 15) >> 4;
  constexpr int NCH = 2;

  float4 wq[2][3][NCH];
  auto load_w = [&](int j, int nt0, float4 (&dst)[3][NCH]) {
    const int nnt = Ls[j].Kp >> 4;
#pragma unroll
    for (int jo = 0; jo < 3; ++jo)
#pragma unroll
      for (int n = 0; n < NCH; ++n) {
        const int nt = min(nt0 + n, nnt - 1);
        dst[jo][n] = *reinterpret_cast<const float4*>(Ls[j].Wd + ((((size_t)nt * 3 + jo) * 4 + kk) * 16 + r) * 4);
      }
  };
  load_w(0, nt_lo, wq[0]);
  int wsel = 0;

  for (int tile = blockIdx.x; tile < ntiles; tile += gridDim.x) {
    const int p0 = tile * TP + wave * 16 * MT;
    long prow[MT];
    bool pv[MT];
#pragma unroll
    for (int m = 0; m < MT; ++m) {
      pv[m] = p0 + 16 * m + r < P;
      prow[m] = min(p0 + 16 * m + r, P - 1);
    }
    unsigned long long pvb[MT];
#pragma unroll
    for (int m = 0; m < MT; ++m) pvb[m] = MASKED ? __ballot(pv[m]) : 0ull;
    float4 dz[NL][3][MT];
#pragma unroll
    for (int j = 0; j < NL; ++j)
#pragma unroll
      for (int jo = 0; jo < 3; ++jo) {
        const int ch = 16 * jo + 4 * kk;
        if constexpr (RAW) {
#pragma unroll
          for (int m = 0; m < MT; ++m) dz[j][jo][m] = *reinterpret_cast<const float4*>(Ls[j].DZ + prow[m] * 48 + ch);
        } else {
          const float4 a4 = *reinterpret_cast<const float4*>(Ls[j].cA + ch);
          const float4 b4 = *reinterpret_cast<const float4*>(Ls[j].cB + ch);
          const float4 c4 = *reinterpret_cast<const float4*>(Ls[j].cC + ch);
#pragma unroll
          for (int m = 0; m < MT; ++m) {
            const float4 dy = *reinterpret_cast<const float4*>(Ls[j].DZ + prow[m] * 48 + ch);
            const float4 zr = *reinterpret_cast<const float4*>(Ls[j].Zr + prow[m] * 48 + ch);
            dz[j][jo][m].x = fmaf(a4.x, dy.x, fmaf(b4.x, zr.x, c4.x));
            dz[j][jo][m].y = fmaf(a4.y, dy.y, fmaf(b4.y, zr.y, c4.y));
            dz[j][jo][m].z = fmaf(a4.z, dy.z, fmaf(b4.z, zr.z, c4.z));
            dz[j][jo][m].w = fmaf(a4.w, dy.w, fmaf(b4.w, zr.w, c4.w));
          }
        }
      }
    for (int nt0 = nt_lo; nt0 < nt_hi; nt0 += NCH) {
      float4 gs[MT][NCH], xv[MT][NCH];
#pragma unroll
      for (int n = 0; n < NCH; ++n) {
        const int k4 = 16 * min(nt0 + n, nt_hi - 1) + 4 * kk;
        const int k4l = (k4 + 3 >= k_lo && k4 < k_hi) ? k4 : (k_lo & ~3);
#pragma unroll
        for (int m = 0; m < MT; ++m) {
          gs[m][n] = *reinterpret_cast<const float4*>(Gd + prow[m] * ldg + k4l);
          if constexpr (!MASKED) xv[m][n] = *reinterpret_cast<const float4*>(X + prow[m] * ldx + k4l);
        }
      }
      const int nt_next = nt0 + NCH < nt_hi ? nt0 + NCH : nt_lo;
#pragma unroll
      for (int j = 0; j < NL; ++j) {
        const int nnt = Ls[j].Kp >> 4;
        unsigned long long mk[MT][NCH][4];
        if constexpr (MASKED) {
          const unsigned long long* __restrict__ Mj = j == 0 ? M0 : M1;
#pragma unroll
          for (int m = 0; m < MT; ++m)
#pragma unroll
            for (int n = 0; n < NCH; ++n) {
              const size_t wi =
                  ((size_t)__builtin_amdgcn_readfirstlane((p0 >> 4) + m) * nnt + min(nt0 + n, nnt - 1)) * 4;
#pragma unroll
              for (int g = 0; g < 4; ++g) mk[m][n][g] = Mj[wi + g];
            }
        }
        const int cur = NL == 2 ? j : wsel;
        if (j + 1 < NL)
          load_w(j + 1, nt0, wq[cur ^ 1]);
        else
          load_w(0, nt_next, wq[cur ^ 1]);
        __builtin_amdgcn_sched_barrier(0);
        f32x4 acc[MT][NCH];
#pragma unroll
        for (int m = 0; m < MT; ++m)
#pragma unroll
          for (int n = 0; n < NCH; ++n) acc[m][n] = f32x4{0.f, 0.f, 0.f, 0.f};
#pragma unroll
        for (int jo = 0; jo < 3; ++jo)
#pragma unroll
          for (int t = 0; t < 4; ++t)
#pragma unroll
            for (int n = 0; n < NCH; ++n)
#pragma unroll
              for (int m = 0; m < MT; ++m) acc[m][n] = mfma16(f4c(wq[cur][jo][n], t), f4c(dz[j][jo][m], t), acc[m][n]);
        if (NL == 1) wsel ^= 1;
        double* my = sacc + ((size_t)(j * 4 + wave) * KpMax) * 2;
#pragma unroll
        for (int n = 0; n < NCH; ++n) {
          const int nt = nt0 + n;
          if (nt < nnt && nt < nt_hi) {
            const int k4 = 16 * nt + 4 * kk;
            const float4 mu = *reinterpret_cast<const float4*>(vec_l + k4);
            const float4 is = *reinterpret_cast<const float4*>(vec_l + KpMax + k4);
            const float4 sk = *reinterpret_cast<const float4*>(vec_l + (2 + 2 * j) * KpMax + k4);
            const float4 tk = *reinterpret_cast<const float4*>(vec_l + (3 + 2 * j) * KpMax + k4);
            const bool in0 = k4 + 0 >= k_lo && k4 + 0 < k_hi, in1 = k4 + 1 >= k_lo && k4 + 1 < k_hi;
            const bool in2 = k4 + 2 >= k_lo && k4 + 2 < k_hi, in3 = k4 + 3 >= k_lo && k4 + 3 < k_hi;
            unsigned long long inb[4] = {0ull, 0ull, 0ull, 0ull};
            if constexpr (MASKED) {
              inb[0] = __ballot(in0);
              inb[1] = __ballot(in1);
              inb[2] = __ballot(in2);
              inb[3] = __ballot(in3);
            }
            float l1[4] = {0.f, 0.f, 0.f, 0.f}, l2[4] = {0.f, 0.f, 0.f, 0.f};
#pragma unroll
            for (int m = 0; m < MT; ++m) {
              float d0, d1, d2, d3;
              if constexpr (MASKED) {
                d0 = __builtin_amdgcn_inverse_ballot_w64(mk[m][n][0] & pvb[m] & inb[0]) ? acc[m][n][0] : 0.f;
                d1 = __builtin_amdgcn_inverse_ballot_w64(mk[m][n][1] & pvb[m] & inb[1]) ? acc[m][n][1] : 0.f;
                d2 = __builtin_amdgcn_inverse_ballot_w64(mk[m][n][2] & pvb[m] & inb[2]) ? acc[m][n][2] : 0.f;
                d3 = __builtin_amdgcn_inverse_ballot_w64(mk[m][n][3] & pvb[m] & inb[3]) ? acc[m][n][3] : 0.f;
              } else {
                const float4 x = xv[m][n];
                d0 = (pv[m] && in0 && fmaf(x.x, sk.x, tk.x) > 0.f) ? acc[m][n][0] : 0.f;
                d1 = (pv[m] && in1 && fmaf(x.y, sk.y, tk.y) > 0.f) ? acc[m][n][1] : 0.f;
                d2 = (pv[m] && in2 && fmaf(x.z, sk.z, tk.z) > 0.f) ? acc[m][n][2] : 0.f;
                d3 = (pv[m] && in3 && fmaf(x.w, sk.w, tk.w) > 0.f) ? acc[m][n][3] : 0.f;
                l2[0] = fmaf(d0, (x.x - mu.x) * is.x, l2[0]);
                l2[1] = fmaf(d1, (x.y - mu.y) * is.y, l2[1]);
                l2[2] = fmaf(d2, (x.z - mu.z) * is.z, l2[2]);
                l2[3] = fmaf(d3, (x.w - mu.w) * is.w, l2[3]);
              }
              gs[m][n].x = fmaf(sk.x, d0, gs[m][n].x);
              gs[m][n].y = fmaf(sk.y, d1, gs[m][n].y);
              gs[m][n].z = fmaf(sk.z, d2, gs[m][n].z);
              gs[m][n].w = fmaf(sk.w, d3, gs[m][n].w);
              l1[0] += d0;
              l1[1] += d1;
              l1[2] += d2;
              l1[3] += d3;
            }
#pragma unroll
            for (int g = 0; g < 4; ++g) {
              l1[g] = eml::row16_sum(l1[g]);
              if constexpr (!MASKED) l2[g] = eml::row16_sum(l2[g]);
              if (r == 0) {
                my[2 * (k4 + g)] += (double)l1[g];
                if constexpr (!MASKED) my[2 * (k4 + g) + 1] += (double)l2[g];
              }
            }
          }
        }
      }
#pragma unroll
      for (int n = 0; n < NCH; ++n) {
        const int nt = nt0 + n;
        if (nt < nt_hi) {
          const int k4 = 16 * nt + 4 * kk;
          const bool act = k4 + 3 >= k_lo && k4 < k_hi;
          if constexpr (TOP) {
            const int t = k4 - (k_hi - 24);
            float* cdst = Top + (t >= 12 ? (size_t)P * 12 + (t - 12) : (size_t)max(t, 0));
#pragma unroll
            for (int m = 0; m < MT; ++m) {
              float* dst = t >= 0 ? cdst + prow[m] * 12 : Gd + prow[m] * ldg + k4;
              if (pv[m] && act) *reinterpret_cast<float4*>(dst) = gs[m][n];
            }
          } else {
#pragma unroll
            for (int m = 0; m < MT; ++m) {
              if (pv[m] && act) *reinterpret_cast<float4*>(Gd + prow[m] * ldg + k4) = gs[m][n];
            }
          }
        }
      }
    }
  }
  __syncthreads();
#pragma unroll
  for (int j = 0; j < NL; ++j) {
    const int Kp = Ls[j].Kp;
    const double* base = sacc + (size_t)j * 4 * KpMax * 2;
    for (int e = tid; e < Kp * 2; e += 256)
      Ls[j].partials[(size_t)blockIdx.x * Kp * 2 + e] = (base[e] + base[(size_t)KpMax * 2 + e]) +
                                                        (base[(size_t)2 * KpMax * 2 + e] + base[(size_t)3 * KpMax * 2 + e]);
  }
}

template <int MT>
__global__ __launch_bounds__(256, 2) void conv1x1_bwd_narrow_kernel(
    const float* __restrict__ DZ, const float* __restrict__ W1 , int Cin, int k_lo,
    const float* __restrict__ X, int ldx, const float* __restrict__ scale1, const float* __restrict__ shift1,
    const float* __restrict__ mean, const float* __restrict__ istd, int P, const float* __restrict__ Gd, int ldg,
    float* __restrict__ N12, double* __restrict__ partials , int Kp) {
  __shared__ double red[4][12][2];
  const int tid = threadIdx.x, lane = tid & 63, wave = tid >> 6;
  const int r = lane & 15, kk = lane >> 4;
  float aw[3][4];
#pragma unroll
  for (int jo = 0; jo < 3; ++jo)
#pragma unroll
    for (int t = 0; t < 4; ++t) aw[jo][t] = r < 12 ? W1[(size_t)(16 * jo + 4 * kk + t) * Cin + k_lo + r] : 0.f;
  const bool cv = kk < 3;
  const int cq = k_lo + 4 * (cv ? kk : 2);
  float sk[4], tk[4], mu[4], is[4];
#pragma unroll
  for (int g = 0; g < 4; ++g) {
    sk[g] = scale1[cq + g];
    tk[g] = shift1[cq + g];
    mu[g] = mean[cq + g];
    is[g] = istd[cq + g];
  }
  double s1[4] = {0.0, 0.0, 0.0, 0.0}, s2[4] = {0.0, 0.0, 0.0, 0.0};
  constexpr int TP = 64 * MT;
  const int ntiles = (P + TP - 1) / TP;
  for (int tile = blockIdx.x; tile < ntiles; tile += gridDim.x) {
    const int p0 = tile * TP + wave * 16 * MT;
    size_t prow[MT];
    bool pv[MT];
    float4 dz[MT][3];
    float2 xa[MT], xb[MT], ga[MT], gb[MT];
#pragma unroll
    for (int m = 0; m < MT; ++m) {
      pv[m] = p0 + 16 * m + r < P;
      prow[m] = (size_t)min(p0 + 16 * m + r, P - 1);
#pragma unroll
      for (int jo = 0; jo < 3; ++jo) dz[m][jo] = *reinterpret_cast<const float4*>(DZ + prow[m] * 48 + 16 * jo + 4 * kk);
      xa[m] = *reinterpret_cast<const float2*>(X + prow[m] * ldx + cq);
      xb[m] = *reinterpret_cast<const float2*>(X + prow[m] * ldx + cq + 2);
      ga[m] = *reinterpret_cast<const float2*>(Gd + prow[m] * ldg + cq);
      gb[m] = *reinterpret_cast<const float2*>(Gd + prow[m] * ldg + cq + 2);
    }
    f32x4 acc[MT];
#pragma unroll
    for (int m = 0; m < MT; ++m) acc[m] = f32x4{0.f, 0.f, 0.f, 0.f};
#pragma unroll
    for (int jo = 0; jo < 3; ++jo)
#pragma unroll
      for (int t = 0; t < 4; ++t)
#pragma unroll
        for (int m = 0; m < MT; ++m) acc[m] = mfma16(aw[jo][t], f4c(dz[m][jo], t), acc[m]);
#pragma unroll
    for (int m = 0; m < MT; ++m) {
      const float x[4] = {xa[m].x, xa[m].y, xb[m].x, xb[m].y};
      const float gold[4] = {ga[m].x, ga[m].y, gb[m].x, gb[m].y};
      float o[4];
#pragma unroll
      for (int g = 0; g < 4; ++g) {
        const float d = (pv[m] && cv && fmaf(x[g], sk[g], tk[g]) > 0.f) ? acc[m][g] : 0.f;
        o[g] = fmaf(sk[g], d, gold[g]);
        s1[g] += (double)d;
        s2[g] += (double)(d * ((x[g] - mu[g]) * is[g]));
      }
      if (pv[m] && cv) *reinterpret_cast<float4*>(N12 + prow[m] * 12 + 4 * kk) = make_float4(o[0], o[1], o[2], o[3]);
    }
  }
#pragma unroll
  for (int g = 0; g < 4; ++g) {
#pragma unroll
    for (int o = 1; o < 16; o <<= 1) {
      s1[g] += shfl_xor_d(s1[g], o);
      s2[g] += shfl_xor_d(s2[g], o);
    }
    if (r == 0 && cv) {
      red[wave][4 * kk + g][0] = s1[g];
      red[wave][4 * kk + g][1] = s2[g];
    }
  }
  __syncthreads();
  if (tid < 24) {
    const int c = tid >> 1, e = tid & 1;
    partials[((size_t)blockIdx.x * Kp + k_lo + c) * 2 + e] = (red[0][c][e] + red[1][c][e]) + (red[2][c][e] + red[3][c][e]);
  }
}

__global__ void permute_w1_bwd_kernel(const float* __restrict__ W, int Cout, int Cin, int Kp, int Ko,
                                      float* __restrict__ Wd) {
  const size_t total = (size_t)Kp * Ko;
  for (size_t e = (size_t)blockIdx.x * blockDim.x + threadIdx.x; e < total; e += (size_t)gridDim.x * blockDim.x) {
    const int t = (int)(e & 3), col = (int)((e >> 2) & 15), kk = (int)((e >> 6) & 3);
    const size_t rest = e >> 8;
    const int jo = (int)(rest % (Ko >> 4)), nt = (int)(rest / (Ko >> 4));
    const int o = 16 * jo + 4 * kk + t, k = 16 * nt + col;
    Wd[e] = (o < Cout && k < Cin) ? W[(size_t)o * Cin + k] : 0.f;
  }
}

__global__ __launch_bounds__(256) void grad_materialize_kernel(float* __restrict__ Gd, int ldg,
                                                               const float* __restrict__ X, int ldx,
                                                               const float* __restrict__ sB,
                                                               const float* __restrict__ sC, int c0, int n, size_t P) {
  const int nh = n >> 1;
  const size_t total = P * nh;
  for (size_t e = (size_t)blockIdx.x * 256 + threadIdx.x; e < total; e += (size_t)gridDim.x * 256) {
    const size_t p = e / nh;
    const int c = c0 + 2 * (int)(e - p * nh);
    const float2 x = *reinterpret_cast<const float2*>(X + p * ldx + c);
    float2* gp = reinterpret_cast<float2*>(Gd + p * ldg + c);
    float2 g = *gp;
    g.x += fmaf(sB[c], x.x, sC[c]);
    g.y += fmaf(sB[c + 1], x.y, sC[c + 1]);
    *gp = g;
  }
}

__global__ __launch_bounds__(256) void bn_bwd_stats_kernel(const float* __restrict__ DY, int ld_dy,
                                                           const float* __restrict__ raw, int ld_raw,
                                                           const float* __restrict__ out, int ld_out, int relu, int C,
                                                           size_t P, const float* __restrict__ mean,
                                                           const float* __restrict__ istd,
                                                           double* __restrict__ partials ) {
  extern __shared__ __attribute__((aligned(16))) float smem[];
  double* red = reinterpret_cast<double*>(smem);
  const int tid = threadIdx.x, lane = tid & 63, wave = tid >> 6;
  const int nk = (C + 63) >> 6;
  float mu[6], is[6];
  double a1[6], a2[6];
#pragma unroll
  for (int k = 0; k < 6; ++k) {
    const int c = lane + 64 * k;
    mu[k] = (k < nk && c < C) ? mean[c] : 0.f;
    is[k] = (k < nk && c < C) ? istd[c] : 0.f;
    a1[k] = a2[k] = 0.0;
  }
  constexpr int kUN = 4;
  for (size_t p0 = ((size_t)blockIdx.x * 4 + wave) * kUN; p0 < P; p0 += (size_t)gridDim.x * 4 * kUN) {
#pragma unroll
    for (int k = 0; k < 6; ++k) {
      if (k < nk) {
// ... 382 lines not shown
    co[2][o] = Zr ? cC[o] : 0.f;
  }
  const long per = (P + gridDim.x - 1) / gridDim.x, p_lo = (long)blockIdx.x * per, p_hi = min(P, p_lo + per);
  const int Ho = Hin >> 1, Wo = Win >> 1;
  for (int li = 0; li < n; ++li) {
    const int c = list[li];
    __syncthreads();
    for (int o = tid; o < Cout; o += 256) wcol[o] = W[(size_t)o * Cin + c];
    __syncthreads();
    const float s1 = scale1[c], t1 = shift1[c];
    const double mu = mean[c], is = istd[c];
    double acc = 0.0;
    for (long p = p_lo + tid; p < p_hi; p += 256) {
      const float x = X[(size_t)p * ldx + c];
      if (fmaf(x, s1, t1) > 0.f) {
        long pp = p;
        if (pool) {
          const long b = p / ((long)Hin * Win), rem = p - b * (long)Hin * Win;
          const int y = (int)(rem / Win), xx = (int)(rem - (long)y * Win);
          pp = (b * Ho + (y >> 1)) * Wo + (xx >> 1);
        }
        const float* dy = DY + (size_t)pp * ld_dy;
        const float* zr = Zr ? Zr + (size_t)pp * ld_z : dy;
        double d = 0.0;
        for (int o = 0; o < Cout; ++o) d += (double)wcol[o] * (double)fmaf(co[0][o], dy[o], fmaf(co[1][o], zr[o], co[2][o]));
        if (pool) d *= 0.25;
        acc += d * (((double)x - mu) * is);
      }
    }
#pragma unroll
    for (int o = 32; o > 0; o >>= 1) acc += shfl_xor_d(acc, o);
    if ((tid & 63) == 0) red[tid >> 6] = acc;
    __syncthreads();
    if (tid == 0) partial[(size_t)blockIdx.x * Cin + c] = (red[0] + red[1]) + (red[2] + red[3]);
  }
}

__global__ __launch_bounds__(256) void bn_dgamma_direct_reduce_kernel(const double* __restrict__ partial, int R, int Cin,
                                                                      const int* __restrict__ cond,
                                                                      float* __restrict__ dgamma) {
  const int c = blockIdx.x * 256 + threadIdx.x;
  if (c >= Cin || !cond[c]) return;
  double s = 0.0;
  for (int g = 0; g < R; ++g) s += partial[(size_t)g * Cin + c];
  dgamma[c] = (float)s;
}

extern "C" int eml_dense_conv3x3_bwd_data_f32(const float* G, int ldg, int c0, const float* W2, const float* Z,
                                              const float* zmean, const float* zistd, float* DZ, int B, int H, int W,
                                              double* partials, int grid, const float* X, int ldx, int cx,
                                              const float* sB, const float* sC, float* GF, eml_stream_t stream) {
  if (!G || !W2 || !Z || !zmean || !zistd || !DZ || !partials || B < 1 || H < 1 || W < 1 || grid < 1 || (c0 & 1) ||
      (ldg & 1))
    return eml::fail(EML_EINVAL, "eml_dense_conv3x3_bwd_data_f32: bad arguments");
  if (X) {
    if (!sB || !sC || !GF || (ldx & 1))
      return eml::fail(EML_EINVAL, "eml_dense_conv3x3_bwd_data_f32: fused affine needs X, sB, sC, GF");
    if (cx < 0 || (cx & 1)) return eml::fail(EML_EINVAL, "eml_dense_conv3x3_bwd_data_f32: cx must be even");
  }
  static const bool narrow = [] { const char* v = getenv("EML_D3_NARROW"); return v && v[0] == '1'; }();
  static const bool tall = [] { const char* v = getenv("EML_D3_SHORT"); return !(v && v[0] == '1'); }();
  const auto al16 = [](const void* q) { return (reinterpret_cast<uintptr_t>(q) & 15) == 0; };
  const bool wide = !narrow && (ldg & 3) == 0 && (c0 & 3) == 0 && al16(G) &&
                    (!X || ((ldx & 3) == 0 && (cx & 3) == 0 && al16(X) && al16(sB) && al16(sC) && al16(GF)));
#define EML_LAUNCH_D3(FUSEV, WIDEV, THV)                                                                                \
  hipLaunchKernelGGL((conv3x3_bwd_data_kernel<FUSEV, WIDEV, THV>), dim3(grid), dim3(THV * 64), 0, (hipStream_t)stream, G, ldg, \
                     c0, W2, Z, zmean, zistd, DZ, B, H, W, partials, X, ldx, cx, sB, sC, GF, eml::DropKey{})
  if (X) {
    if (tall) { if (wide) EML_LAUNCH_D3(true, true, 8); else EML_LAUNCH_D3(true, false, 8); }
    else      { EML_LAUNCH_D3(true, false, 4); }
  } else {
    if (tall) { if (wide) EML_LAUNCH_D3(false, true, 8); else EML_LAUNCH_D3(false, false, 8); }
    else      { if (wide) EML_LAUNCH_D3(false, true, 4); else EML_LAUNCH_D3(false, false, 4); }
  }
#undef EML_LAUNCH_D3
  return eml::check_launch("eml_dense_conv3x3_bwd_data_f32");
}

extern "C" int eml_dense_conv3x3_bwd_data_drop_f32(const float* G, int ldg, int c0, const float* W2, const float* Z,
                                                   const float* zmean, const float* zistd, float* DZ, int B, int H, int W,
                                                   double* partials, int grid, const float* X, int ldx, int cx,
                                                   const float* sB, const float* sC, float* GF, unsigned long long seed,
                                                   int layer, double p, eml_stream_t stream) {
  if (!G || !W2 || !Z || !zmean || !zistd || !DZ || !partials || B < 1 || H < 1 || W < 1 || grid < 1 || (c0 & 1) ||
      (ldg & 1))
    return eml::fail(EML_EINVAL, "eml_dense_conv3x3_bwd_data_drop_f32: bad arguments");
  if (!X || !sB || !sC || !GF || (ldx & 1))
    return eml::fail(EML_EINVAL, "eml_dense_conv3x3_bwd_data_drop_f32: fused affine needs X, sB, sC, GF");
  if (cx < 0 || (cx & 1)) return eml::fail(EML_EINVAL, "eml_dense_conv3x3_bwd_data_drop_f32: cx must be even");
  if (!(p >= 0.0 && p <= 1.0) || layer < 0)
    return eml::fail(EML_EINVAL, "eml_dense_conv3x3_bwd_data_drop_f32: p must be in [0, 1] and layer >= 0 (p = %g, layer = %d)", p,
                     layer);
  if ((long long)B * H * W > 0x7FFFFFFFll)
    return eml::fail(EML_EINVAL, "eml_dense_conv3x3_bwd_data_drop_f32: B*H*W must fit the 32-bit pixel counter");
  static const bool narrow = [] { const char* v = getenv("EML_D3_NARROW"); return v && v[0] == '1'; }();
  static const bool tall = [] { const char* v = getenv("EML_D3_SHORT"); return !(v && v[0] == '1'); }();
  const auto al16 = [](const void* q) { return (reinterpret_cast<uintptr_t>(q) & 15) == 0; };
  const bool wide = !narrow && (ldg & 3) == 0 && (c0 & 3) == 0 && al16(G) && (ldx & 3) == 0 && (cx & 3) == 0 && al16(X) &&
                    al16(sB) && al16(sC) && al16(GF);
  const eml::DropKey dk = eml_drop_key(seed, layer, p);
#define EML_LAUNCH_D3(WIDEV, THV)                                                                                       \
  hipLaunchKernelGGL((conv3x3_bwd_data_kernel<true, WIDEV, THV, true>), dim3(grid), dim3(THV * 64), 0, (hipStream_t)stream, G, \
                     ldg, c0, W2, Z, zmean, zistd, DZ, B, H, W, partials, X, ldx, cx, sB, sC, GF, dk)
  if (tall) { if (wide) EML_LAUNCH_D3(true, 8); else EML_LAUNCH_D3(false, 8); }
  else      { EML_LAUNCH_D3(false, 4); }
#undef EML_LAUNCH_D3
  return eml::check_launch("eml_dense_conv3x3_bwd_data_drop_f32");
}

extern "C" int eml_dense_conv3x3_bwd_weight_f32(const float* G, int ldg, int c0, const float* Z, const float* scale2,
                                                const float* shift2, int B, int H, int W, float* partial, float* dW2,
                                                int grid, eml_stream_t stream) {
  if (!G || !Z || !scale2 || !shift2 || !partial || !dW2 || B < 1 || H < 1 || W < 1 || grid < 1)
    return eml::fail(EML_EINVAL, "eml_dense_conv3x3_bwd_weight_f32: bad arguments");
  static const bool greg = [] { const char* v = getenv("EML_W3_GREG"); return v && v[0] == '1'; }();
  if (!greg && (ldg & 3) == 0 && (c0 & 3) == 0 && (reinterpret_cast<uintptr_t>(G) & 15) == 0) {
    const size_t lds = (size_t)(2 * kHH * kHW * kPSW + 2 * kGL) * sizeof(float);
    EML_ENSURE_LDS((&conv3x3_bwd_weight_kernel<true>), lds);
    hipLaunchKernelGGL(conv3x3_bwd_weight_kernel<true>, dim3(grid), dim3(kBW), lds, (hipStream_t)stream, G, ldg, c0, Z,
                       scale2, shift2, B, H, W, partial);
  } else {
    const size_t lds = (size_t)(2 * kHH * kHW * kPSW) * sizeof(float);
    EML_ENSURE_LDS((&conv3x3_bwd_weight_kernel<false>), lds);
    hipLaunchKernelGGL(conv3x3_bwd_weight_kernel<false>, dim3(grid), dim3(kBW), lds, (hipStream_t)stream, G, ldg, c0, Z,
                       scale2, shift2, B, H, W, partial);
  }
  int rc = eml::check_launch("eml_dense_conv3x3_bwd_weight_f32");
  if (rc) return rc;
  hipLaunchKernelGGL(reduce_rows_kernel, dim3(27 * 256 / 64), dim3(256), 0, (hipStream_t)stream, partial, 2 * grid,
                     (size_t)27 * 256, 1, 0, 0, 0, dW2);
  return eml::check_launch("eml_dense_conv3x3_bwd_weight_f32(reduce)");
}

#ifdef EML_STAMPS
extern "C" int eml_c3_read_stamps(unsigned long long* out, int reset) {
  if (hipMemcpyFromSymbol(out, HIP_SYMBOL(eml_c3_stamps), 8 * sizeof(unsigned long long)) != hipSuccess) return -1;
  if (reset) {
    const unsigned long long z[8] = {0};
    if (hipMemcpyToSymbol(HIP_SYMBOL(eml_c3_stamps), z, sizeof(z)) != hipSuccess) return -1;
  }
  return 0;
}
#endif
extern "C" int eml_dense_conv3x3_bwd_fused_supported(int ldg, int c0, int ldx, int cx) {
  return ((ldg & 1) == 0 && (c0 & 1) == 0 && (ldx & 1) == 0 && (cx & 1) == 0) ? 1 : 0;
}
template <bool DROP>
static int conv3x3_bwd_fused_launch(const char* name, const float* G, int ldg, int c0, const float* W2, const float* Z,
                                    const float* zmean, const float* zistd, float* DZ, int B, int H, int W, double* partials,
                                    int grid, const float* X, int ldx, int cx, const float* sB, const float* sC, float* GF,
                                    const float* scale2, const float* shift2, float* partialW, float* dW2, eml::DropKey dk,
                                    eml_stream_t stream) {
  if (!G || !W2 || !Z || !zmean || !zistd || !DZ || !partials || !X || !sB || !sC || !scale2 || !shift2 || !partialW ||
      !dW2 || B < 1 || H < 1 || W < 1 || grid < 1 || cx < 0)
    return eml::fail(EML_EINVAL, "%s: bad arguments", name);
  const auto al16 = [](const void* q) { return (reinterpret_cast<uintptr_t>(q) & 15) == 0; };
  if (!eml_dense_conv3x3_bwd_fused_supported(ldg, c0, ldx, cx) || !al16(G) || !al16(X) || !al16(GF) || !al16(Z) || !al16(scale2) ||
      !al16(shift2))
    return eml::fail(EML_EINVAL, "%s: needs even ldg, c0, ldx, cx and 16-byte aligned buffers", name);
  const bool a16 = (ldg & 3) == 0 && (c0 & 3) == 0 && (ldx & 3) == 0 && (cx & 3) == 0;
#ifndef EML_C3_WTP
#define EML_C3_WTP 1
#endif
#if EML_C3_WTP
  const size_t lds = (size_t)(2 * kHH * kHW * kPSG + 2 * kTH * kTW * 48 + 27 * 3 * 64 + 32) * sizeof(float) + 8 * 48 * 2 * sizeof(double);
  if (a16) {
    if (GF) {
      EML_ENSURE_LDS((&conv3x3_bwd_fused_tp_kernel<true, DROP, true>), lds);
      hipLaunchKernelGGL((conv3x3_bwd_fused_tp_kernel<true, DROP, true>), dim3(grid), dim3(512), lds, (hipStream_t)stream, G, ldg, c0, W2, Z,
                         zmean, zistd, DZ, B, H, W, partials, X, ldx, cx, sB, sC, GF, scale2, shift2, partialW, dk);
    } else {
      EML_ENSURE_LDS((&conv3x3_bwd_fused_tp_kernel<true, DROP, false>), lds);
      hipLaunchKernelGGL((conv3x3_bwd_fused_tp_kernel<true, DROP, false>), dim3(grid), dim3(512), lds, (hipStream_t)stream, G, ldg, c0, W2, Z,
                         zmean, zistd, DZ, B, H, W, partials, X, ldx, cx, sB, sC, GF, scale2, shift2, partialW, dk);
    }
  } else {
    if (GF) {
      EML_ENSURE_LDS((&conv3x3_bwd_fused_tp_kernel<false, DROP, true>), lds);
      hipLaunchKernelGGL((conv3x3_bwd_fused_tp_kernel<false, DROP, true>), dim3(grid), dim3(512), lds, (hipStream_t)stream, G, ldg, c0, W2, Z,
                         zmean, zistd, DZ, B, H, W, partials, X, ldx, cx, sB, sC, GF, scale2, shift2, partialW, dk);
    } else {
      EML_ENSURE_LDS((&conv3x3_bwd_fused_tp_kernel<false, DROP, false>), lds);
      hipLaunchKernelGGL((conv3x3_bwd_fused_tp_kernel<false, DROP, false>), dim3(grid), dim3(512), lds, (hipStream_t)stream, G, ldg, c0, W2, Z,
                         zmean, zistd, DZ, B, H, W, partials, X, ldx, cx, sB, sC, GF, scale2, shift2, partialW, dk);
    }
  }
  int rc = eml::check_launch(name);
  if (rc) return rc;
  hipLaunchKernelGGL(reduce_rows_kernel, dim3(21 * 256 / 64), dim3(256), 0, (hipStream_t)stream, partialW, grid,
                     (size_t)21 * 256, 3, 0, 0, 0, dW2);
  return eml::check_launch(DROP ? "eml_dense_conv3x3_bwd_fused_drop_f32(reduce)" : "eml_dense_conv3x3_bwd_fused_f32(reduce)");
#else
  const size_t lds = (size_t)(2 * kHH * kHW * kPSG + kHH * kHW * kPSW + 27 * 3 * 64 + 32) * sizeof(float) + 8 * 48 * 2 * sizeof(double);
  if (a16) {
    if (GF) {
      EML_ENSURE_LDS((&conv3x3_bwd_fused_kernel<true, DROP, true>), lds);
      hipLaunchKernelGGL((conv3x3_bwd_fused_kernel<true, DROP, true>), dim3(grid), dim3(512), lds, (hipStream_t)stream, G, ldg, c0, W2, Z, zmean,
                         zistd, DZ, B, H, W, partials, X, ldx, cx, sB, sC, GF, scale2, shift2, partialW, dk);
    } else {
      EML_ENSURE_LDS((&conv3x3_bwd_fused_kernel<true, DROP, false>), lds);
      hipLaunchKernelGGL((conv3x3_bwd_fused_kernel<true, DROP, false>), dim3(grid), dim3(512), lds, (hipStream_t)stream, G, ldg, c0, W2, Z, zmean,
                         zistd, DZ, B, H, W, partials, X, ldx, cx, sB, sC, GF, scale2, shift2, partialW, dk);
    }
  } else {
    if (GF) {
      EML_ENSURE_LDS((&conv3x3_bwd_fused_kernel<false, DROP, true>), lds);
      hipLaunchKernelGGL((conv3x3_bwd_fused_kernel<false, DROP, true>), dim3(grid), dim3(512), lds, (hipStream_t)stream, G, ldg, c0, W2, Z, zmean,
                         zistd, DZ, B, H, W, partials, X, ldx, cx, sB, sC, GF, scale2, shift2, partialW, dk);
    } else {
      EML_ENSURE_LDS((&conv3x3_bwd_fused_kernel<false, DROP, false>), lds);
      hipLaunchKernelGGL((conv3x3_bwd_fused_kernel<false, DROP, false>), dim3(grid), dim3(512), lds, (hipStream_t)stream, G, ldg, c0, W2, Z, zmean,
                         zistd, DZ, B, H, W, partials, X, ldx, cx, sB, sC, GF, scale2, shift2, partialW, dk);
    }
  }
  int rc = eml::check_launch(name);
  if (rc) return rc;
  hipLaunchKernelGGL(reduce_rows_kernel, dim3(27 * 256 / 64), dim3(256), 0, (hipStream_t)stream, partialW, 2 * grid,
                     (size_t)27 * 256, 1, 0, 0, 0, dW2);
  return eml::check_launch(DROP ? "eml_dense_conv3x3_bwd_fused_drop_f32(reduce)" : "eml_dense_conv3x3_bwd_fused_f32(reduce)");
#endif
}

extern "C" int eml_dense_conv3x3_bwd_fused_f32(const float* G, int ldg, int c0, const float* W2, const float* Z,
                                               const float* zmean, const float* zistd, float* DZ, int B, int H, int W,
                                               double* partials, int grid, const float* X, int ldx, int cx,
                                               const float* sB, const float* sC, float* GF, const float* scale2,
                                               const float* shift2, float* partialW, float* dW2, eml_stream_t stream) {
  return conv3x3_bwd_fused_launch<false>("eml_dense_conv3x3_bwd_fused_f32", G, ldg, c0, W2, Z, zmean, zistd, DZ, B, H, W, partials,
                                         grid, X, ldx, cx, sB, sC, GF, scale2, shift2, partialW, dW2, eml::DropKey{}, stream);
}

extern "C" int eml_dense_conv3x3_bwd_fused_drop_f32(const float* G, int ldg, int c0, const float* W2, const float* Z,
                                                    const float* zmean, const float* zistd, float* DZ, int B, int H, int W,
                                                    double* partials, int grid, const float* X, int ldx, int cx,
                                                    const float* sB, const float* sC, float* GF, const float* scale2,
                                                    const float* shift2, float* partialW, float* dW2, unsigned long long seed,
                                                    int layer, double p, eml_stream_t stream) {
  if (!(p >= 0.0 && p <= 1.0) || layer < 0)
    return eml::fail(EML_EINVAL, "eml_dense_conv3x3_bwd_fused_drop_f32: p must be in [0, 1] and layer >= 0 (p = %g, layer = %d)", p,
                     layer);
  if ((long long)B * H * W > 0x7FFFFFFFll)
    return eml::fail(EML_EINVAL, "eml_dense_conv3x3_bwd_fused_drop_f32: B*H*W must fit the 32-bit pixel counter");
  return conv3x3_bwd_fused_launch<true>("eml_dense_conv3x3_bwd_fused_drop_f32", G, ldg, c0, W2, Z, zmean, zistd, DZ, B, H, W,
                                        partials, grid, X, ldx, cx, sB, sC, GF, scale2, shift2, partialW, dW2,
                                        eml_drop_key(seed, layer, p), stream);
}

namespace {
__global__ __launch_bounds__(256) void dropout_mask_kernel(eml::DropKey dk, unsigned P, unsigned short* __restrict__ out) {
  for (unsigned q = blockIdx.x * 256u + threadIdx.x; q < P; q += gridDim.x * 256u) {
    unsigned m = 0;
#pragma unroll
    for (unsigned grp = 0; grp < 3; ++grp) {
      const uint4 d = eml::drop_draws(dk, q, grp);
#pragma unroll
      for (int w = 0; w < 4; ++w)
        if ((unsigned long long)eml::draw_word(d, w) >= dk.thr) m |= 1u << (4 * grp + w);
    }
    out[q] = (unsigned short)m;
  }
}
}

extern "C" int eml_dense_dropout_mask_u16(unsigned long long seed, int layer, double p, long P, unsigned short* mask,
                                          eml_stream_t stream) {
  if (!mask || P < 1 || P > 0x7FFFFFFFl || layer < 0 || !(p >= 0.0 && p <= 1.0))
    return eml::fail(EML_EINVAL, "eml_dense_dropout_mask_u16: bad arguments (mask null, P outside [1, 2^31), layer < 0 or p "
                                 "outside [0, 1])");
  const unsigned grid = (unsigned)std::min<long>((P + 255) / 256, 4096);
  hipLaunchKernelGGL(dropout_mask_kernel, dim3(grid), dim3(256), 0, (hipStream_t)stream, eml_drop_key(seed, layer, p), (unsigned)P,
                     mask);
  return eml::check_launch("eml_dense_dropout_mask_u16");
}

extern "C" int eml_dense_bn_bwd_finalize_f32(const double* partials, int R, int pstride, double count,
                                             const float* gamma, const float* mean, const float* istd, int C, int Cpad,
                                             int training, float* dgamma, float* dbeta, float* cA, float* cB,
                                             float* cC, float* sB, float* sC, int s_accumulate, int c_lo,
                                             int c_hi, const float* beta, const float* W, const float* dW, int w_rows,
                                             int* cond, int* any_cond, eml_stream_t stream) {
  if (!partials || !gamma || !mean || !istd || !dgamma || !dbeta || C < 1 || Cpad < C || R < 1 ||
      (cA && (!cB || !cC)) || (sB && !sC) || c_lo < 0 || c_hi <= c_lo)
    return eml::fail(EML_EINVAL, "eml_dense_bn_bwd_finalize_f32: bad arguments");
  if (W && (!dW || !beta || w_rows < 1))
    return eml::fail(EML_EINVAL, "eml_dense_bn_bwd_finalize_f32: W given without dW / beta / w_rows");
  if (c_hi > Cpad) c_hi = Cpad;
  hipLaunchKernelGGL(bn_bwd_finalize_kernel, dim3((c_hi - c_lo + 3) / 4), dim3(256), 0, (hipStream_t)stream, partials,
                     R, pstride, count, gamma, mean, istd, C, Cpad, training, dgamma, dbeta, cA, cB, cC, sB, sC,
                     s_accumulate, c_lo, c_hi, beta, W, dW, w_rows, W ? cond : nullptr, W ? any_cond : nullptr);
  return eml::check_launch("eml_dense_bn_bwd_finalize_f32");
}

extern "C" int eml_dense_bn_dgamma_direct_f32(const float* X, int ldx, long P, int Hin, int Win, int pool, const float* DY,
                                              int ld_dy, const float* Zr, int ld_z, const float* cA, const float* cB,
                                              const float* cC, int Cout, const float* W, int Cin, const float* scale1,
                                              const float* shift1, const float* mean, const float* istd, const int* cond,
                                              double* scratch, float* dgamma, int grid, eml_stream_t stream) {
  if (!X || !DY || !W || !scale1 || !shift1 || !mean || !istd || !cond || !scratch || !dgamma || P < 1 || grid < 1 ||
      Cin < 1 || Cin > 384 || Cout < 1 || Cout > 192 || Cin > ldx || Cout > ld_dy || (Zr && (!cA || !cB || !cC || Cout > ld_z)) ||
      (pool && ((Hin | Win) & 1)))
    return eml::fail(EML_EINVAL, "eml_dense_bn_dgamma_direct_f32: bad arguments (Cin <= 384, Cout <= 192, even maps when pooled)");
  hipLaunchKernelGGL(bn_dgamma_direct_partial_kernel, dim3(grid), dim3(256), 0, (hipStream_t)stream, X, ldx, P, Hin, Win,
                     pool, DY, ld_dy, Zr, ld_z, cA, cB, cC, Cout, W, Cin, scale1, shift1, mean, istd, cond, scratch);
  int rc = eml::check_launch("eml_dense_bn_dgamma_direct_f32(partial)");
  if (rc) return rc;
  hipLaunchKernelGGL(bn_dgamma_direct_reduce_kernel, dim3((Cin + 255) / 256), dim3(256), 0, (hipStream_t)stream, scratch,
                     grid, Cin, cond, dgamma);
  return eml::check_launch("eml_dense_bn_dgamma_direct_f32(reduce)");
}

extern "C" int eml_dense_conv1x1_bwd_weight_f32(const float* X, int ldx, long P, int Hin, int Win, int pool, int Kp,
                                                int Cin, const float* scale1, const float* shift1, const float* DY,
                                                int ld_dy, const float* Zr, int ld_z, const float* cA, const float* cB,
                                                const float* cC, int Cout, float* partial, float* dW, int grid,
                                                float* dz_out, const float* W1, int k_lo, const float* G, int ldg,
                                                float* N12, double* partials_n, eml_stream_t stream) {
  if (dz_out && (Cout != 48 || pool))
    return eml::fail(EML_EINVAL, "eml_dense_conv1x1_bwd_weight_f32: dz_out is for dense layers (Cout == 48, no pool)");
  if (N12 && (Cout != 48 || pool || !W1 || !G || !partials_n || k_lo < 0 || (k_lo & 1) || k_lo + 12 > Cin || (ldg & 1) ||
              (ldg != 12 && k_lo + 12 > ldg)))
    return eml::fail(EML_EINVAL, "eml_dense_conv1x1_bwd_weight_f32: fused narrow pass needs a dense layer, W1, G, partials_n "
                                 "and an even k_lo with k_lo + 12 <= Cin (k_lo=%d, Cin=%d)", k_lo, Cin);
  if (!X || !scale1 || !shift1 || !DY || !Zr || !cA || !cB || !cC || !partial || !dW || P < 1 || grid < 1 || Kp < 32 ||
      (Kp & 15) || Cin > Kp || Cout < 1)
    return eml::fail(EML_EINVAL, "eml_dense_conv1x1_bwd_weight_f32: bad arguments");
  const int nchunks = (Cout + 47) / 48;
  for (int ch = 0; ch < nchunks; ++ch) {
    const int n0 = ch * 48, nv = (Cout - n0 < 48) ? Cout - n0 : 48;
    int n_load = ((ld_dy < ld_z ? ld_dy : ld_z) - n0) & ~3;
    if (n_load > 48) n_load = 48;
    if (n_load < nv) return eml::fail(EML_EINVAL, "eml_dense_conv1x1_bwd_weight_f32: DY/Zr rows narrower than Cout");
    const NarrowArgs na{W1, G, N12, partials_n, Cin, k_lo, ldg};
    static const int vec_env = [] { const char* v = getenv("EML_W1_VEC"); return v ? atoi(v) : 0; }();
    const bool vec4 = !pool && (ldx & 3) == 0 && (reinterpret_cast<uintptr_t>(X) & 15) == 0 &&
                      vec_env == 4;
    if (vec4 && N12 && vec_env == 4)
      hipLaunchKernelGGL((conv1x1_bwd_weight_kernel<false, true, 4>), dim3(grid), dim3(256), 0, (hipStream_t)stream, X, ldx,
                         (int)P, Hin, Win, Kp, scale1, shift1, DY + n0, ld_dy, Zr + n0, ld_z, cA + n0, cB + n0, cC + n0,
                         nv, n_load, partial, dz_out, na);
    else if (vec4 && !N12)
      hipLaunchKernelGGL((conv1x1_bwd_weight_kernel<false, false, 4>), dim3(grid), dim3(256), 0, (hipStream_t)stream, X, ldx,
                         (int)P, Hin, Win, Kp, scale1, shift1, DY + n0, ld_dy, Zr + n0, ld_z, cA + n0, cB + n0, cC + n0,
                         nv, n_load, partial, dz_out, na);
    else if (pool)
      hipLaunchKernelGGL((conv1x1_bwd_weight_kernel<true, false>), dim3(grid), dim3(256), 0, (hipStream_t)stream, X, ldx,
                         (int)P, Hin, Win, Kp, scale1, shift1, DY + n0, ld_dy, Zr + n0, ld_z, cA + n0, cB + n0, cC + n0,
                         nv, n_load, partial, nullptr, na);
    else if (N12)
      hipLaunchKernelGGL((conv1x1_bwd_weight_kernel<false, true>), dim3(grid), dim3(256), 0, (hipStream_t)stream, X, ldx,
                         (int)P, Hin, Win, Kp, scale1, shift1, DY + n0, ld_dy, Zr + n0, ld_z, cA + n0, cB + n0, cC + n0,
                         nv, n_load, partial, dz_out, na);
    else
      hipLaunchKernelGGL((conv1x1_bwd_weight_kernel<false, false>), dim3(grid), dim3(256), 0, (hipStream_t)stream, X, ldx,
                         (int)P, Hin, Win, Kp, scale1, shift1, DY + n0, ld_dy, Zr + n0, ld_z, cA + n0, cB + n0, cC + n0,
                         nv, n_load, partial, dz_out, na);
    int rc = eml::check_launch("eml_dense_conv1x1_bwd_weight_f32");
    if (rc) return rc;
    hipLaunchKernelGGL(reduce_rows_kernel, dim3((Cin * 48 + 63) / 64), dim3(256), 0, (hipStream_t)stream, partial,
                       grid, (size_t)Kp * 48, 0, Cin, nv, n0, dW);
    rc = eml::check_launch("eml_dense_conv1x1_bwd_weight_f32(reduce)");
    if (rc) return rc;
  }
  return EML_OK;
}

extern "C" int eml_dense_permute_w1_bwd_f32(const float* W, int Cout, int Cin, int Kp, int Ko, float* Wd,
                                            eml_stream_t stream) {
  if (!W || !Wd || Cout < 1 || Cin < 1 || Kp < Cin || (Kp & 15) || Ko < Cout || (Ko & 15))
    return eml::fail(EML_EINVAL, "eml_dense_permute_w1_bwd_f32: bad arguments");
  hipLaunchKernelGGL(permute_w1_bwd_kernel, dim3(64), dim3(256), 0, (hipStream_t)stream, W, Cout, Cin, Kp, Ko, Wd);
  return eml::check_launch("eml_dense_permute_w1_bwd_f32");
}

extern "C" int eml_dense_conv1x1_bwd_data_f32(const float* DY, int ld_dy, const float* Zr, int ld_z, const float* cA,
                                              const float* cB, const float* cC, int Ko, const float* Wd,
                                              const float* X, int ldx, const float* scale1, const float* shift1,
                                              const float* mean, const float* istd, long P, int Hin, int Win, int pool,
                                              int Kp, float* G, int ldg, int accumulate, double* partials, int grid,
                                              const unsigned short* relu_mask16, eml_stream_t stream) {
  if (!DY || !Zr || !cA || !cB || !cC || !Wd || (!relu_mask16 && (!X || !mean || !istd)) || !scale1 || !shift1 || !G ||
      !partials || P < 1 || grid < 1 || (Kp & 15) || (Ko & 15) || Ko > ld_dy || Ko > ld_z || (ld_dy & 3) || (ld_z & 3) ||
      (ldx & 3) || (ldg & 3) || (!relu_mask16 && Kp > ldx) || Kp > ldg)
    return eml::fail(EML_EINVAL, "eml_dense_conv1x1_bwd_data_f32: bad arguments");
  if (relu_mask16 && !(pool && Ko != 48))
    return eml::fail(EML_EINVAL, "eml_dense_conv1x1_bwd_data_f32: relu_mask16 is for the transition form (pool, Ko != 48)");
  const size_t lds = (size_t)4 * Kp * 2 * sizeof(double);
#define EML_LAUNCH_BWD_DATA(POOLV, RESV, NCHV)                                                                        \
  hipLaunchKernelGGL((conv1x1_bwd_data_kernel<POOLV, RESV, NCHV>), dim3(grid), dim3(256), lds, (hipStream_t)stream, DY, \
                     ld_dy, Zr, ld_z, cA, cB, cC, Ko, Wd, X, ldx, scale1, shift1, mean, istd, (int)P, Hin, Win, Kp, G, \
                     ldg, accumulate, partials)
  if (pool) {
    if (Ko == 48) {
      EML_LAUNCH_BWD_DATA(true, true, 4);
    } else {
      const size_t lds_t = lds + (size_t)(4 * Kp + 3 * Ko + 4 * 16 * 36) * sizeof(float);
#define EML_LAUNCH_TRANSITION(ACCV, MSKV)                                                                              \
  do {                                                                                                                \
    EML_ENSURE_LDS((&transition_bwd_data_kernel<2, 2, ACCV, MSKV>), lds_t);                                 \
    hipLaunchKernelGGL((transition_bwd_data_kernel<2, 2, ACCV, MSKV>), dim3(grid), dim3(256), lds_t,                   \
                       (hipStream_t)stream, DY, ld_dy, Zr, ld_z, cA, cB, cC, Ko, Wd, X, ldx, scale1, shift1, mean, istd, \
                       (int)P, Hin, Win, Kp, G, ldg, partials, relu_mask16);                                           \
  } while (0)
#define EML_LAUNCH_TRANSITION_RES(NJOV)                                                                                \
  do {                                                                                                                \
    EML_ENSURE_LDS((&transition_bwd_data_kernel<2, 2, false, true, NJOV>), lds_t);                                     \
    hipLaunchKernelGGL((transition_bwd_data_kernel<2, 2, false, true, NJOV>), dim3(grid), dim3(256), lds_t,            \
                       (hipStream_t)stream, DY, ld_dy, Zr, ld_z, cA, cB, cC, Ko, Wd, X, ldx, scale1, shift1, mean, istd, \
                       (int)P, Hin, Win, Kp, G, ldg, partials, relu_mask16);                                           \
  } while (0)
      if (relu_mask16 && !accumulate && Ko == 112) EML_LAUNCH_TRANSITION_RES(7);
      else if (relu_mask16 && !accumulate && Ko == 160) EML_LAUNCH_TRANSITION_RES(10);
      else if (relu_mask16 && !accumulate && Ko == 176) EML_LAUNCH_TRANSITION_RES(11);
      else if (relu_mask16) {
        if (accumulate) EML_LAUNCH_TRANSITION(true, true); else EML_LAUNCH_TRANSITION(false, true);
      } else {
        if (accumulate) EML_LAUNCH_TRANSITION(true, false); else EML_LAUNCH_TRANSITION(false, false);
      }
#undef EML_LAUNCH_TRANSITION
#undef EML_LAUNCH_TRANSITION_RES
    }
  } else {
    if (Ko == 48) EML_LAUNCH_BWD_DATA(false, true, 2); else EML_LAUNCH_BWD_DATA(false, false, 4);
  }
#undef EML_LAUNCH_BWD_DATA
  return eml::check_launch("eml_dense_conv1x1_bwd_data_f32");
}

namespace {
int launch_bwd_data_multi(int n_layers, const float* const* DZ, const float* const* Zr, const float* const* cA,
                          const float* const* cB, const float* const* cC, const float* const* Wd,
                          const float* const* scale1, const float* const* shift1, double* const* partials, const int* Kp,
                          const float* X, int ldx, const float* mean, const float* istd, long P, int k_lo, int k_hi,
                          float* G, int ldg, int grid, const unsigned long long* const* relu_masks, float* top,
                          eml_stream_t stream) {
  if (top && (n_layers != 2 || !relu_masks || Zr || k_lo != 0 || k_hi < 24 || (k_hi & 3) || P * 12 > 2147483647L))
    return eml::fail(EML_EINVAL, "eml_dense_conv1x1_bwd_data_multi_top_f32: the compact top-24 output needs two layers, "
                                 "relu_masks, materialised dz, k_lo == 0 and k_hi >= 24, a multiple of 4 (k_hi=%d)", k_hi);
  if (n_layers < 1 || n_layers > 2 || !DZ || !Wd || !scale1 || !shift1 || !partials ||
      !Kp || (!relu_masks && (!X || !mean || !istd)) || !G || P < 1 || grid < 1 || k_lo < 0 || k_hi <= k_lo ||
      (ldx & 3) || (ldg & 3))
    return eml::fail(EML_EINVAL, "eml_dense_conv1x1_bwd_data_multi_f32: bad arguments");
  const bool raw = Zr == nullptr;
  if (!raw && (!cA || !cB || !cC))
    return eml::fail(EML_EINVAL, "eml_dense_conv1x1_bwd_data_multi_f32: Zr given without cA/cB/cC");
  if (relu_masks && !raw)
    return eml::fail(EML_EINVAL, "eml_dense_conv1x1_bwd_data_multi_f32: relu_masks needs the materialised dz (Zr == NULL)");
  BwdLayer L[2];
  const unsigned long long* Mk[2] = {nullptr, nullptr};
  int kmax = 0;
  for (int j = 0; j < 2; ++j) {
    const int s = j < n_layers ? j : 0;
    const unsigned long long* mk = relu_masks ? relu_masks[s] : nullptr;
    Mk[j] = mk;
    L[j] = raw ? BwdLayer{DZ[s], nullptr, nullptr, nullptr, nullptr, Wd[s], scale1[s], shift1[s], partials[s], Kp[s]}
               : BwdLayer{DZ[s], Zr[s], cA[s], cB[s], cC[s], Wd[s], scale1[s], shift1[s], partials[s], Kp[s]};
    if (!DZ[s] || (!raw && !Zr[s]) || !Wd[s] || !partials[s] || (relu_masks && !mk) || (Kp[s] & 15) ||
        (!relu_masks && Kp[s] > ldx) || Kp[s] > ldg)
      return eml::fail(EML_EINVAL, "eml_dense_conv1x1_bwd_data_multi_f32: bad layer %d", s);
    if (Kp[s] > kmax) kmax = Kp[s];
  }
  if (((k_hi + 15) & ~15) > kmax) return eml::fail(EML_EINVAL, "eml_dense_conv1x1_bwd_data_multi_f32: range beyond Kp");
  const size_t lds = (size_t)n_layers * 4 * kmax * 2 * sizeof(double) + (size_t)(2 + 2 * n_layers) * kmax * sizeof(float);
  if (lds > 80 * 1024) return eml::fail(EML_EINVAL, "eml_dense_conv1x1_bwd_data_multi_f32: Kp=%d does not fit LDS", kmax);
#define EML_LAUNCH_MULTI(NLV, MTV, RAWV, MSKV)                                                                       \
  do {                                                                                                              \
    EML_ENSURE_LDS((&conv1x1_bwd_data_multi_kernel<NLV, MTV, RAWV, MSKV>), lds);                                 \
    hipLaunchKernelGGL((conv1x1_bwd_data_multi_kernel<NLV, MTV, RAWV, MSKV>), dim3(grid), dim3(256), lds,            \
                       (hipStream_t)stream, L[0], L[1], X, ldx, mean, istd, (int)P, k_lo, k_hi, G, ldg, kmax,        \
                       Mk[0], Mk[1], (float*)nullptr);                                                              \
  } while (0)
  if (n_layers == 1) {
    if (relu_masks) EML_LAUNCH_MULTI(1, 4, true, true);
    else if (raw) EML_LAUNCH_MULTI(1, 4, true, false);
    else EML_LAUNCH_MULTI(1, 4, false, false);
  } else if (top) {
    EML_ENSURE_LDS((&conv1x1_bwd_data_multi_kernel<2, 2, true, true, true>), lds);
    hipLaunchKernelGGL((conv1x1_bwd_data_multi_kernel<2, 2, true, true, true>), dim3(grid), dim3(256), lds,
                       (hipStream_t)stream, L[0], L[1], X, ldx, mean, istd, (int)P, k_lo, k_hi, G, ldg, kmax, Mk[0], Mk[1],
                       top);
  } else {
    if (relu_masks) EML_LAUNCH_MULTI(2, 2, true, true);
    else if (raw) EML_LAUNCH_MULTI(2, 2, true, false);
    else EML_LAUNCH_MULTI(2, 2, false, false);
  }
#undef EML_LAUNCH_MULTI
  return eml::check_launch("eml_dense_conv1x1_bwd_data_multi_f32");
}
}

extern "C" int eml_dense_conv1x1_bwd_data_multi_f32(int n_layers, const float* const* DZ, const float* const* Zr,
                                                    const float* const* cA, const float* const* cB,
                                                    const float* const* cC, const float* const* Wd,
                                                    const float* const* scale1, const float* const* shift1,
                                                    double* const* partials, const int* Kp, const float* X, int ldx,
                                                    const float* mean, const float* istd, long P, int k_lo, int k_hi,
                                                    float* G, int ldg, int grid,
                                                    const unsigned long long* const* relu_masks, eml_stream_t stream) {
  return launch_bwd_data_multi(n_layers, DZ, Zr, cA, cB, cC, Wd, scale1, shift1, partials, Kp, X, ldx, mean, istd, P, k_lo,
                               k_hi, G, ldg, grid, relu_masks, nullptr, stream);
}

extern "C" int eml_dense_conv1x1_bwd_data_multi_top_f32(const float* const* DZ, const float* const* Wd,
                                                        const float* const* scale1, const float* const* shift1,
                                                        double* const* partials, const int* Kp, long P, int k_hi,
                                                        float* G, int ldg, int grid,
                                                        const unsigned long long* const* relu_masks, float* top,
                                                        eml_stream_t stream) {
  if (!top) return eml::fail(EML_EINVAL, "eml_dense_conv1x1_bwd_data_multi_top_f32: top is NULL");
  return launch_bwd_data_multi(2, DZ, nullptr, nullptr, nullptr, nullptr, Wd, scale1, shift1, partials, Kp, nullptr, 0,
                               nullptr, nullptr, P, 0, k_hi, G, ldg, grid, relu_masks, top, stream);
}

extern "C" int eml_dense_conv1x1_bwd_narrow_f32(const float* DZ, const float* W1, int Cin, int k_lo, const float* X,
                                                int ldx, const float* scale1, const float* shift1, const float* mean,
                                                const float* istd, long P, const float* G, int ldg, float* N12,
                                                double* partials, int Kp, int grid, eml_stream_t stream) {
  if (!DZ || !W1 || !X || !scale1 || !shift1 || !mean || !istd || !G || !N12 || !partials || P < 1 || grid < 1 ||
      k_lo < 0 || (k_lo & 1) || k_lo + 12 > Cin || Cin > Kp || (ldx & 1) || (ldg & 1) || Kp > ldx || Kp > ldg)
    return eml::fail(EML_EINVAL, "eml_dense_conv1x1_bwd_narrow_f32: bad arguments");
  hipLaunchKernelGGL((conv1x1_bwd_narrow_kernel<4>), dim3(grid), dim3(256), 0, (hipStream_t)stream, DZ, W1, Cin, k_lo, X,
                     ldx, scale1, shift1, mean, istd, (int)P, G, ldg, N12, partials, Kp);
  return eml::check_launch("eml_dense_conv1x1_bwd_narrow_f32");
}

extern "C" int eml_dense_grad_materialize_f32(float* G, int ldg, const float* X, int ldx, const float* sB,
                                              const float* sC, int c0, int n, long P, eml_stream_t stream) {
  if (!G || !X || !sB || !sC || P < 1 || n < 2 || (n & 1) || (c0 & 1) || (ldg & 1) || (ldx & 1))
    return eml::fail(EML_EINVAL, "eml_dense_grad_materialize_f32: bad arguments");
  const size_t total = (size_t)P * (n >> 1);
  const int grid = (int)((total + 255) / 256 < 8192 ? (total + 255) / 256 : 8192);
  hipLaunchKernelGGL(grad_materialize_kernel, dim3(grid), dim3(256), 0, (hipStream_t)stream, G, ldg, X, ldx, sB, sC, c0,
                     n, (size_t)P);
  return eml::check_launch("eml_dense_grad_materialize_f32");
}

extern "C" int eml_dense_bn_bwd_stats_f32(const float* DY, int ld_dy, const float* raw, int ld_raw, const float* out,
                                          int ld_out, int relu, int C, long P, const float* mean, const float* istd,
                                          double* partials, int grid, eml_stream_t stream) {
  if (!DY || !raw || !mean || !istd || !partials || (relu && !out) || C < 1 || C > 384 || P < 1 || grid < 1)
    return eml::fail(EML_EINVAL, "eml_dense_bn_bwd_stats_f32: bad arguments");
  auto a16 = [](const void* q) { return (reinterpret_cast<size_t>(q) & 15) == 0; };
  if (C <= 32 && (C & 3) == 0 && ((ld_dy | ld_raw | (relu ? ld_out : 0)) & 3) == 0 && a16(DY) && a16(raw) && (!relu || a16(out)) &&
      a16(mean) && a16(istd)) {
    hipLaunchKernelGGL(bn_bwd_stats_small_kernel, dim3(grid), dim3(256), 0, (hipStream_t)stream, DY, ld_dy, raw, ld_raw, out, ld_out,
                       relu, C, (size_t)P, mean, istd, partials);
    return eml::check_launch("eml_dense_bn_bwd_stats_f32");
  }
  const size_t lds = (size_t)4 * ((C + 63) / 64) * 64 * 2 * sizeof(double);
  hipLaunchKernelGGL(bn_bwd_stats_kernel, dim3(grid), dim3(256), lds, (hipStream_t)stream, DY, ld_dy, raw, ld_raw, out,
                     ld_out, relu, C, (size_t)P, mean, istd, partials);
  return eml::check_launch("eml_dense_bn_bwd_stats_f32");
}

extern "C" int eml_dense_conv0_bwd_weight_f32(const float* x, const float* G, int ldg, const float* X1, int ldx,
                                              const float* Y0, int C0, const float* cA, const float* cB,
                                              const float* cC, int B, int H, int W, float* partial, float* dW0,
                                              int grid, eml_stream_t stream) {
  if (!x || !G || !X1 || !Y0 || !cA || !cB || !cC || !partial || !dW0 || C0 < 1 || C0 > 32 || B < 1 || grid < 1)
    return eml::fail(EML_EINVAL, "eml_dense_conv0_bwd_weight_f32: bad arguments");
  hipLaunchKernelGGL(conv0_bwd_weight_kernel<false>, dim3(grid), dim3(256), 0, (hipStream_t)stream, x, G, ldg, X1, ldx, Y0, C0,
                     cA, cB, cC, B, H, W, partial, nullptr, nullptr, nullptr, nullptr);
  int rc = eml::check_launch("eml_dense_conv0_bwd_weight_f32");
  if (rc) return rc;
  hipLaunchKernelGGL(reduce_rows_kernel, dim3(27 * 32 / 64 + 1), dim3(256), 0, (hipStream_t)stream, partial, grid * 4,
                     (size_t)1024, 2, 0, C0, 0, dW0);
  return eml::check_launch("eml_dense_conv0_bwd_weight_f32(reduce)");
}

extern "C" int eml_dense_head_pool_bwd_f32(const float* gpooled, const float* F, int ldf, int C, int B, int H, int W,
                                           int k, float* dF, int ldd, eml_stream_t stream) {
  if (!gpooled || !F || !dF || C < 1 || B < 1 || k < 1) return eml::fail(EML_EINVAL, "eml_dense_head_pool_bwd_f32: bad arguments");
  const size_t total = (size_t)B * H * W * C;
  const int grid = (int)((total + 255) / 256 < 4096 ? (total + 255) / 256 : 4096);
  hipLaunchKernelGGL(head_pool_bwd_kernel, dim3(grid), dim3(256), 0, (hipStream_t)stream, gpooled, F, ldf, C, B, H, W, k,
                     dF, ldd);
  return eml::check_launch("eml_dense_head_pool_bwd_f32");
}

extern "C" int eml_dense_norm0_bwd_stats_f32(const float* G, int ldg, const float* Y0, int ld_y0, const float* scale0,
                                             const float* shift0, const float* sB, const float* sC, int C, long P,
                                             const float* mean, const float* istd, double* partials, int grid,
                                             eml_stream_t stream) {
  auto a16 = [](const void* q) { return (reinterpret_cast<size_t>(q) & 15) == 0; };
  if (!G || !Y0 || !scale0 || !shift0 || !sB || !sC || !mean || !istd || !partials || C < 4 || C > 32 || (C & 3) || P < 1 ||
      grid < 1 || ((ldg | ld_y0) & 3) || !a16(G) || !a16(Y0) || !a16(scale0) || !a16(shift0) || !a16(sB) || !a16(sC) || !a16(mean) ||
      !a16(istd))
    return eml::fail(EML_EINVAL, "eml_dense_norm0_bwd_stats_f32: bad arguments (C a multiple of 4 <= 32, 16-byte aligned operands)");
  hipLaunchKernelGGL(norm0_bwd_stats_kernel, dim3(grid), dim3(256), 0, (hipStream_t)stream, G, ldg, Y0, ld_y0, scale0, shift0, sB,
                     sC, C, (size_t)P, mean, istd, partials);
  return eml::check_launch("eml_dense_norm0_bwd_stats_f32");
}

extern "C" int eml_dense_conv0_bwd_weight_fused_f32(const float* x, const float* G, int ldg, const float* Y0, int C0,
                                                    const float* scale0, const float* shift0, const float* sB, const float* sC,
                                                    const float* cA, const float* cB, const float* cC, int B, int H, int W,
                                                    float* partial, float* dW0, int grid, eml_stream_t stream) {
  if (!x || !G || !Y0 || !scale0 || !shift0 || !sB || !sC || !cA || !cB || !cC || !partial || !dW0 || C0 < 1 || C0 > 32 || B < 1 ||
      grid < 1)
    return eml::fail(EML_EINVAL, "eml_dense_conv0_bwd_weight_fused_f32: bad arguments");
  hipLaunchKernelGGL(conv0_bwd_weight_kernel<true>, dim3(grid), dim3(256), 0, (hipStream_t)stream, x, G, ldg, nullptr, 0, Y0, C0, cA,
                     cB, cC, B, H, W, partial, scale0, shift0, sB, sC);
  int rc = eml::check_launch("eml_dense_conv0_bwd_weight_fused_f32");
  if (rc) return rc;
  hipLaunchKernelGGL(reduce_rows_kernel, dim3(27 * 32 / 64 + 1), dim3(256), 0, (hipStream_t)stream, partial, grid * 4,
                     (size_t)1024, 2, 0, C0, 0, dW0);
  return eml::check_launch("eml_dense_conv0_bwd_weight_fused_f32(reduce)");
}

extern "C" int eml_dense_conv0_bwd_data_f32(const float* G, int ldg, const float* X1, int ldx, const float* Y0, int C0,
                                            const float* scale0, const float* shift0, const float* sB, const float* sC,
                                            const float* cA, const float* cB, const float* cC, const float* W0, int B, int H,
                                            int W, float* dX, eml_stream_t stream) {
  auto a16 = [](const void* q) { return (reinterpret_cast<size_t>(q) & 15) == 0; };
  const bool fused = X1 == nullptr;
  if (!G || !Y0 || !cA || !cB || !cC || !W0 || !dX || (fused && (!scale0 || !shift0 || !sB || !sC)))
    return eml::fail(EML_EINVAL, "eml_dense_conv0_bwd_data_f32: null pointer");
  if (C0 != kC0dC || B < 1 || H < 1 || W < 1 || ldg < C0 || (ldg & 3) || (!fused && (ldx < C0 || (ldx & 3))))
    return eml::fail(EML_EINVAL, "eml_dense_conv0_bwd_data_f32: bad shape (C0 == 24, B, H, W >= 1, ldg / ldx >= 24 and multiples of 4)");
  if (!a16(G) || !a16(Y0) || (!fused && !a16(X1)) || !a16(cA) || !a16(cB) || !a16(cC) ||
      (fused && (!a16(scale0) || !a16(shift0) || !a16(sB) || !a16(sC))))
    return eml::fail(EML_EINVAL, "eml_dense_conv0_bwd_data_f32: G, X1, Y0 and the coefficient vectors must be 16-byte aligned");
  const size_t tiles = (size_t)B * ((H + kC0dTH - 1) / kC0dTH) * ((W + kC0dTW - 1) / kC0dTW);
  if (tiles > 0x7fffffff) return eml::fail(EML_EINVAL, "eml_dense_conv0_bwd_data_f32: more than 2^31 - 1 tiles of 8 x 32 pixels");
  const int grid = (int)tiles;
  if (fused)
    hipLaunchKernelGGL(conv0_bwd_data_kernel<true>, dim3(grid), dim3(256), 0, (hipStream_t)stream, G, ldg, nullptr, 0, Y0,
                       scale0, shift0, sB, sC, cA, cB, cC, W0, B, H, W, dX);
  else
    hipLaunchKernelGGL(conv0_bwd_data_kernel<false>, dim3(grid), dim3(256), 0, (hipStream_t)stream, G, ldg, X1, ldx, Y0,
                       nullptr, nullptr, nullptr, nullptr, cA, cB, cC, W0, B, H, W, dX);
  return eml::check_launch("eml_dense_conv0_bwd_data_f32");
}
```

### include/emlight_hip.h

```cpp
#ifndef EMLIGHT_HIP_H
#define EMLIGHT_HIP_H

#include <stddef.h>
#include <stdint.h>

#ifdef __cplusplus
extern "C" {
#endif

typedef void* eml_stream_t;

#define EML_OK 0
#define EML_EINVAL (-1)
#define EML_ELAUNCH (-2)

#define EML_MAX_EPS 64

#define EML_ABI_VERSION 31
int eml_abi_version(void);
const char* eml_last_error(void);

int eml_sg_rasterise_f32(const float* dirs, const float* sizes, const float* colors,
                         float* out, int B, int N, int H, int W, eml_stream_t stream);

#define EML_SG_EXHAUSTIVE 1
int eml_sg_rasterise_ex_f32(const float* dirs, const float* sizes, const float* colors, float* out,
                            int B, int N, int H, int W, int flags, unsigned long long* executed_exp,
                            eml_stream_t stream);

int eml_sg_rasterise_bwd_colors_f32(const float* dirs, const float* sizes, const float* gout,
                                    float* gcolors, int B, int N, int H, int W,
                                    eml_stream_t stream);
size_t eml_sg_rasterise_bwd_work_floats(int B, int N, int H, int W);
int eml_sg_rasterise_bwd_colors_ex_f32(const float* dirs, const float* sizes, const float* gout, float* gcolors, float* work,
                                       int B, int N, int H, int W, int flags, eml_stream_t stream);
size_t eml_sg_rasterise_bwd_full_work_floats(int B, int N, int H, int W);
int eml_sg_rasterise_bwd_f32(const float* dirs, const float* sizes, const float* colors, const float* gout, float* gdirs,
                             float* gsizes, float* gcolors, float* work, int B, int N, int H, int W, int flags,
                             eml_stream_t stream);

int eml_emd_anchor_cost_f32(const float* anchors, float* M, int N, eml_stream_t stream);

int eml_sinkhorn_schedule_f32(const float* x, const float* y, long n, double blur,
                              double scaling, int p, double diameter, const float* range_lo_hi,
                              float* eps_out, int* n_eps_out, float* diameter_out, eml_stream_t stream);

size_t eml_sinkhorn_work_floats(int B, int N);
int eml_sinkhorn_fwd_f32(const float* x, const float* y, const float* M, const float* Mt,
                         const float* alpha, const float* beta, double blur, double scaling, int p,
                         double diameter, const float* range_lo_hi, float* eps_out, int* n_eps_out,
                         float* diameter_out, float* loss, float* gx, float* gy, float* work, int B, int N,
                         eml_stream_t stream);

#define EML_SINKHORN_NO_SPLIT 1
#define EML_SINKHORN_FORCE_SPLIT 2
#define EML_SINKHORN_TEST_STALL 4
int eml_sinkhorn_fwd_ex_f32(const float* x, const float* y, const float* M, const float* Mt,
                            const float* alpha, const float* beta, double blur, double scaling, int p,
                            double diameter, const float* range_lo_hi, float* eps_out, int* n_eps_out,
                            float* diameter_out, float* loss, float* gx, float* gy, float* work, int B, int N,
                            int flags, eml_stream_t stream);

int eml_sinkhorn_fwd_rho_f32(const float* x, const float* y, const float* M, const float* Mt,
                             const float* alpha, const float* beta, double blur, double scaling, int p,
                             double diameter, const float* range_lo_hi, float* eps_out, int* n_eps_out,
                             float* diameter_out, float* loss, float* gx, float* gy, float* work, int B, int N,
                             int flags, double rho, float* lam_out, eml_stream_t stream);

int eml_sinkhorn_bwd_f32(const float* gloss, const float* gunit, float* gout, int B, int N,
                         eml_stream_t stream);

#define EML_SINKHORN_MAX_DIM 8
size_t eml_sinkhorn_dim_work_floats(int B, int N, int D);
int eml_sinkhorn_fwd_dim_f32(const float* x, const float* y, const float* M, const float* Mt,
                             const float* alpha, const float* beta, double blur, double scaling, int p,
                             double diameter, const float* range_lo_hi, float* eps_out, int* n_eps_out,
                             float* diameter_out, float* loss, float* gx, float* gy, float* work, int B, int N,
                             int D, int flags, double rho, float* lam_out, eml_stream_t stream);

int eml_sinkhorn_schedule_dim_f32(const float* x, const float* y, long n, int D, double blur, double scaling, int p,
                                  double diameter, const float* range_lo_hi, float* eps_out, int* n_eps_out,
                                  float* diameter_out, eml_stream_t stream);

int eml_sinkhorn_bwd_weights_f32(const float* gloss, const float* work, float* galpha, float* gbeta, int B, int N,
                                 eml_stream_t stream);



int eml_dense_conv0_fwd_f32(const float* x, const float* w0, float* X, int ldx, int B, int H, int W,
                            int C0, double* partials, int grid, eml_stream_t stream);
int eml_dense_conv0_fwd_mfma_f32(const float* x, const float* w0, float* X, int ldx, int B, int H, int W,
                                 int C0, double* partials, int grid, eml_stream_t stream);

int eml_dense_bn_apply_f32(const float* src, int ld_src, float* dst, int ld_dst, int C, long P,
                           const float* scale, const float* shift, int relu, double* partials,
                           int grid, eml_stream_t stream);

int eml_dense_bn_prepare_f32(const double* partials, int G, int pstride, int n_new, int c_new0,
                             double count, float* mean, float* var, float* istd, const float* gamma,
                             const float* beta, float* rmean, float* rvar, int C, int Cpad, float eps,
                             float momentum, int training, float* scale, float* shift,
                             eml_stream_t stream);

int eml_dense_permute_w1_f32(const float* W, int Cout, int Cin, int Kp, float* Wp, eml_stream_t stream);
int eml_dense_permute_w2_f32(const float* W2, int Cout, float* W2p, eml_stream_t stream);

typedef struct eml_permute_desc {
  const float* src;
  float* dst;
  int kind, Cout, Cin, Kp, Ko, reserved;
} eml_permute_desc;
int eml_dense_permute_batch_f32(const eml_permute_desc* descs, int n, eml_stream_t stream);

int eml_dense_conv1x1_fwd_f32(const float* X, int ldx, long P, int Hin, int Win, int pool, int Kp,
                              const float* scale, const float* shift, const float* Wp, int Cout,
                              float* out, int ldo, double* partials, int grid,
                              unsigned long long* relu_mask, eml_stream_t stream);

int eml_dense_conv3x3_fwd_f32(const float* Z, const float* scale2, const float* shift2,
                              const float* W2p, float* X, int ldx, int c_out0, int B, int H, int W,
                              double* partials, int grid, eml_stream_t stream);

int eml_dense_permute_w2_tp_f32(const float* W2, float* W2t, eml_stream_t stream);
int eml_dense_conv3x3_fwd_tp_supported(int B, int H, int W);
int eml_dense_conv3x3_fwd_tp_f32(const float* Z, const float* scale2, const float* shift2,
                                 const float* W2t, float* X, int ldx, int c_out0, int B, int H, int W,
                                 int band_rows, double* partials, int grid, eml_stream_t stream);

int eml_dense_conv3x3_fwd_drop_f32(const float* Z, const float* scale2, const float* shift2,
                                   const float* W2p, float* X, int ldx, int c_out0, int B, int H, int W,
                                   double* partials, int grid, unsigned long long seed, int layer, double p,
                                   eml_stream_t stream);
int eml_dense_conv3x3_fwd_tp_drop_f32(const float* Z, const float* scale2, const float* shift2,
                                      const float* W2t, float* X, int ldx, int c_out0, int B, int H, int W,
                                      int band_rows, double* partials, int grid, unsigned long long seed, int layer,
                                      double p, eml_stream_t stream);
int eml_dense_dropout_mask_u16(unsigned long long seed, int layer, double p, long P, unsigned short* mask,
                               eml_stream_t stream);

int eml_dense_pool_act_f32(const float* X, int ldx, int B, int Hin, int Win, int Kp, const float* scale,
                           const float* shift, float* A, int lda, unsigned short* relu_mask16,
                           eml_stream_t stream);

int eml_dense_head_pool_fwd_f32(const float* F, int ldf, int C, int B, int H, int W, int k,
                                float* out, eml_stream_t stream);


int eml_dense_conv3x3_bwd_data_f32(const float* G, int ldg, int c0, const float* W2, const float* Z,
                                   const float* zmean, const float* zistd, float* DZ, int B, int H,
                                   int W, double* partials, int grid, const float* X, int ldx, int cx,
                                   const float* sB, const float* sC, float* GF, eml_stream_t stream);

int eml_dense_conv3x3_bwd_fused_supported(int ldg, int c0, int ldx, int cx);
int eml_dense_conv3x3_bwd_fused_f32(const float* G, int ldg, int c0, const float* W2, const float* Z,
                                    const float* zmean, const float* zistd, float* DZ, int B, int H, int W,
                                    double* partials, int grid, const float* X, int ldx, int cx,
                                    const float* sB, const float* sC, float* GF, const float* scale2,
                                    const float* shift2, float* partialW, float* dW2, eml_stream_t stream);

int eml_dense_conv3x3_bwd_data_drop_f32(const float* G, int ldg, int c0, const float* W2, const float* Z,
                                        const float* zmean, const float* zistd, float* DZ, int B, int H,
                                        int W, double* partials, int grid, const float* X, int ldx, int cx,
                                        const float* sB, const float* sC, float* GF, unsigned long long seed,
                                        int layer, double p, eml_stream_t stream);
int eml_dense_conv3x3_bwd_fused_drop_f32(const float* G, int ldg, int c0, const float* W2, const float* Z,
                                         const float* zmean, const float* zistd, float* DZ, int B, int H, int W,
                                         double* partials, int grid, const float* X, int ldx, int cx,
                                         const float* sB, const float* sC, float* GF, const float* scale2,
                                         const float* shift2, float* partialW, float* dW2, unsigned long long seed,
                                         int layer, double p, eml_stream_t stream);

int eml_dense_conv3x3_bwd_weight_f32(const float* G, int ldg, int c0, const float* Z,
                                     const float* scale2, const float* shift2, int B, int H, int W,
                                     float* partial, float* dW2, int grid, eml_stream_t stream);

int eml_dense_bn_bwd_finalize_f32(const double* partials, int R, int pstride, double count,
                                  const float* gamma, const float* mean, const float* istd, int C,
                                  int Cpad, int training, float* dgamma, float* dbeta, float* cA,
                                  float* cB, float* cC, float* sB, float* sC, int s_accumulate,
                                  int c_lo, int c_hi, const float* beta, const float* W, const float* dW,
                                  int w_rows, int* cond, int* any_cond, eml_stream_t stream);

int eml_dense_bn_dgamma_direct_f32(const float* X, int ldx, long P, int Hin, int Win, int pool,
                                   const float* DY, int ld_dy, const float* Zr, int ld_z, const float* cA,
                                   const float* cB, const float* cC, int Cout, const float* W, int Cin,
                                   const float* scale1, const float* shift1, const float* mean,
                                   const float* istd, const int* cond, double* scratch, float* dgamma,
                                   int grid, eml_stream_t stream);

int eml_dense_conv1x1_bwd_weight_f32(const float* X, int ldx, long P, int Hin, int Win, int pool,
                                     int Kp, int Cin, const float* scale1, const float* shift1,
                                     const float* DY, int ld_dy, const float* Zr, int ld_z,
                                     const float* cA, const float* cB, const float* cC, int Cout,
                                     float* partial, float* dW, int grid, float* dz_out,
                                     const float* W1, int k_lo, const float* G, int ldg, float* N12,
                                     double* partials_n, eml_stream_t stream);

int eml_dense_permute_w1_bwd_f32(const float* W, int Cout, int Cin, int Kp, int Ko, float* Wd,
                                 eml_stream_t stream);

int eml_dense_conv1x1_bwd_data_f32(const float* DY, int ld_dy, const float* Zr, int ld_z,
                                   const float* cA, const float* cB, const float* cC, int Ko,
                                   const float* Wd, const float* X, int ldx, const float* scale1,
                                   const float* shift1, const float* mean, const float* istd, long P,
                                   int Hin, int Win, int pool, int Kp, float* G, int ldg,
                                   int accumulate, double* partials, int grid,
                                   const unsigned short* relu_mask16, eml_stream_t stream);

int eml_dense_conv1x1_bwd_data_multi_f32(int n_layers, const float* const* DZ, const float* const* Zr,
                                         const float* const* cA, const float* const* cB,
                                         const float* const* cC, const float* const* Wd,
                                         const float* const* scale1, const float* const* shift1,
                                         double* const* partials, const int* Kp, const float* X, int ldx,
                                         const float* mean, const float* istd, long P, int k_lo,
                                         int k_hi, float* G, int ldg, int grid,
                                         const unsigned long long* const* relu_masks, eml_stream_t stream);

int eml_dense_conv1x1_bwd_data_multi_top_f32(const float* const* DZ, const float* const* Wd,
                                             const float* const* scale1, const float* const* shift1,
                                             double* const* partials, const int* Kp, long P, int k_hi, float* G,
                                             int ldg, int grid, const unsigned long long* const* relu_masks,
                                             float* top, eml_stream_t stream);

int eml_dense_conv1x1_bwd_narrow_f32(const float* DZ, const float* W1, int Cin, int k_lo, const float* X,
                                     int ldx, const float* scale1, const float* shift1,
                                     const float* mean, const float* istd, long P, const float* G, int ldg,
                                     float* N12, double* partials, int Kp, int grid, eml_stream_t stream);

int eml_dense_grad_materialize_f32(float* G, int ldg, const float* X, int ldx, const float* sB,
                                   const float* sC, int c0, int n, long P, eml_stream_t stream);

int eml_dense_bn_bwd_stats_f32(const float* DY, int ld_dy, const float* raw, int ld_raw,
                               const float* out, int ld_out, int relu, int C, long P,
                               const float* mean, const float* istd, double* partials, int grid,
                               eml_stream_t stream);

int eml_dense_conv0_bwd_weight_f32(const float* x, const float* G, int ldg, const float* X1, int ldx,
                                   const float* Y0, int C0, const float* cA, const float* cB,
                                   const float* cC, int B, int H, int W, float* partial, float* dW0,
                                   int grid, eml_stream_t stream);

int eml_dense_norm0_bwd_stats_f32(const float* G, int ldg, const float* Y0, int ld_y0, const float* scale0,
                                  const float* shift0, const float* sB, const float* sC, int C, long P,
                                  const float* mean, const float* istd, double* partials, int grid, eml_stream_t stream);
int eml_dense_conv0_bwd_weight_fused_f32(const float* x, const float* G, int ldg, const float* Y0, int C0,
                                         const float* scale0, const float* shift0, const float* sB, const float* sC,
                                         const float* cA, const float* cB, const float* cC, int B, int H, int W,
                                         float* partial, float* dW0, int grid, eml_stream_t stream);

int eml_dense_conv0_bwd_data_f32(const float* G, int ldg, const float* X1, int ldx, const float* Y0, int C0,
                                 const float* scale0, const float* shift0, const float* sB, const float* sC,
                                 const float* cA, const float* cB, const float* cC, const float* W0, int B, int H, int W,
                                 float* dX, eml_stream_t stream);

int eml_dense_head_pool_bwd_f32(const float* gpooled, const float* F, int ldf, int C, int B, int H,
                                int W, int k, float* dF, int ldd, eml_stream_t stream);


int eml_sphere_tap_table_f32(const float* grid, int H, int W, int Ho, int Wo, int* idx, float* wgt,
                             eml_stream_t stream);

int eml_sphere_im2col_f32(const float* X, const int* idx, const float* wgt, float* A9, int B, int HW,
                          int Po, int C, eml_stream_t stream);

int eml_sphere_col2im_f32(const float* dA9, const int* ptr, const int* src, const float* w, float* dX,
                          int B, int HW, int Po, int C, eml_stream_t stream);

int eml_sphere_conv_fwd_fused_f32(const float* X, const int* idx, const float* wgt, const float* W2,
                                  const float* bias, float* Y, int B, int HW, int Po, int C, int O, int ke,
                                  eml_stream_t stream);
#define EML_TAP_ROWSHARE 1
int eml_sphere_conv_fwd_fused_ex_f32(const float* X, const int* idx, const float* wgt, const float* W2,
                                     const float* bias, float* Y, int B, int HW, int Po, int C, int O, int ke,
                                     const float* residual, float act_slope, int table_flags, eml_stream_t stream);
int eml_sphere_conv_small_supported(int C, int O);
int eml_sphere_conv_small_fwd_f32(const float* X, const int* idx, const float* wgt, const float* W2, const float* bias,
                                  float* Y, int B, int HW, int Po, int C, int O, float act_slope, eml_stream_t stream);
size_t eml_sphere_conv_small_wgrad_partial_floats(int B, int Po, int C, int O);
int eml_sphere_conv_small_wgrad_f32(const float* X, const int* idx, const float* wgt, const float* dY, const float* Yact,
                                    float act_slope, float* partial, float* dW2, float* db, int B, int HW, int Po, int C,
                                    int O, eml_stream_t stream);
int eml_sphere_conv_small_da9_f32(const float* dY, const float* Yact, float act_slope, const float* W2, float* dA9, long M,
                                  int C, int O, eml_stream_t stream);
int eml_sphere_conv_narrow_supported(int C, int O);
int eml_sphere_conv_narrow_fwd_f32(const float* X, const int* idx, const float* wgt, const float* W2, const float* bias, float* Y,
                                   int B, int HW, int Po, int C, int O, eml_stream_t stream);
int eml_sphere_conv_narrow_dgrad_f32(const float* dY, const int* tidx, const float* twgt, int ke, const float* W2, float* dX, int B,
                                     int HW, int Po, int C, int O, eml_stream_t stream);
size_t eml_sphere_conv_narrow_wgrad_partial_floats(int B, int Po, int C, int O);
int eml_sphere_conv_narrow_wgrad_f32(const float* X, const int* idx, const float* wgt, const float* dY, float* partial, float* dW2,
                                     int B, int HW, int Po, int C, int O, eml_stream_t stream);

size_t eml_sphere_conv_narrow_scratch_floats(int B, int HW);
int eml_sphere_conv_narrow_fwd2_f32(const float* X, const int* idx, const float* wgt, const float* W2, const float* bias,
                                    float* Y, float* scratch, int B, int HW, int Po, int C, int O, eml_stream_t stream);
size_t eml_sphere_conv_narrow_wgrad2_partial_floats(int B, int HW, int C);
int eml_sphere_conv_narrow_wgrad2_f32(const float* X, const int* tidx, const float* twgt, int ke,
                                      const unsigned char* rowmax, const float* dY, float* scratch, float* partial, float* dW2, int B, int HW, int Po, int C, int O,
                                      eml_stream_t stream);
int eml_sphere_conv_narrow_dgrad2_f32(const float* dY, const int* tidx, const float* twgt, int ke,
                                      const unsigned char* rowmax, const float* W2, float* dX, float* scratch,
                                      int scratch_has_v, int B, int HW, int Po, int C, int O, eml_stream_t stream);
int eml_sphere_conv_dgrad_fused_f32(const float* dY, const int* tidx, const float* twgt, const unsigned char* rowmax,
                                    int ke, const float* W2t, float* dX, int B, int HW, int Po, int C, int O,
                                    int table_flags, eml_stream_t stream);
int eml_sphere_conv_lowres_variant(int C, int O, int Po, int fp_max);
int eml_sphere_conv_lowres_table_i32(const int* idx, const int* fp, int* lidx, int Po, int ke, eml_stream_t stream);
size_t eml_sphere_conv_lowres_partial_floats(long M, int O, int split);
int eml_sphere_conv_lowres_f32(const float* X, const int* lidx, const float* wgt, const unsigned char* rowmax, int ke,
                               const int* fp, int fp_max, const float* W2, const float* bias, float* Y, float* partial,
                               int split, int B, int HW, int Po, int C, int O, const float* residual, float act_slope,
                               eml_stream_t stream);
size_t eml_sphere_conv_wgrad_partial_floats(int C, int O, int split_k);
int eml_sphere_conv_wgrad_fused_f32(const float* X, const int* idx, const float* wgt, const float* dY,
                                    float* partial, float* dW2, int B, int HW, int Po, int C, int O,
                                    int split_k, eml_stream_t stream);

int eml_spade_modulate_fwd_f32(const float* xn, int ld_x, const float* gb, int ld_gb, float* y, int ld_y,
                               long rows, int C, float slope, eml_stream_t stream);
int eml_spade_modulate_bwd_f32(const float* gy, int ld_gy, const float* xn, int ld_x, const float* gb,
                               int ld_gb, float* dxn, int ld_dx, float* dgb, int ld_dgb, long rows, int C,
                               float slope, eml_stream_t stream);

int eml_bn_stats_f32(const float* x, int ld, long rows, int C, double* partials, int grid, eml_stream_t stream);
int eml_bn_fold_f64(const double* partials, int R, int n, double* sums, eml_stream_t stream);
int eml_bn_finalize_f32(const double* sums, int C, float eps, float momentum, float* mean, float* istd,
                        float* running_mean, float* running_var, eml_stream_t stream);
int eml_spade_norm_modulate_fwd_f32(const float* x, int ld_x, const float* gb, int ld_gb, float* y, int ld_y,
                                    long rows, int C, float slope, const float* mean, const float* istd,
                                    eml_stream_t stream);
int eml_bn_bwd_apply_f32(const float* dxn, int ld_d, const float* x, int ld_x, long rows, int C,
                         const float* mean, const float* istd, const double* sums, float* dx, int ld_o,
                         eml_stream_t stream);

int eml_spade_norm_modulate_up2_fwd_f32(const float* x_lo, const float* gb, float* y, int B, int H, int W, int C, float slope,
                                        const float* mean, const float* istd, eml_stream_t stream);
int eml_bn_bwd_apply_up2_f32(const float* dxn, const float* x_lo, int B, int H, int W, int C, const float* mean,
                             const float* istd, const double* sums, float* dx_lo, eml_stream_t stream);

int eml_spade_norm_modulate_bwd_cols_f32(const float* gy, const float* x, const float* gb, float* dxn, float* dgb, int B, int H,
                                         int W, int C, int up2, float slope, const float* mean, const float* istd,
                                         double* partials, int grid, eml_stream_t stream);

int eml_sphere_conv_spade_supported(int Cin, int Cn, long HW);
int eml_sphere_conv_spade_fwd_f32(const float* actv, const int* idx, const float* wgt, const float* W2r, const float* bias_r,
                                  const float* x, const float* mean, const float* istd, float* Y, float* gamma_out, int B, int H,
                                  int W, int Cin, int Cn, int up2, float act_slope, int table_flags, eml_stream_t stream);
int eml_spade_norm_modulate_bwd_y_f32(const float* gy, const float* x, const float* gamma, const float* y, float* dxn, float* dgb,
                                      int B, int H, int W, int C, int up2, float slope, const float* mean, const float* istd,
// ... 50 lines not shown
```

Measured before the change: 569.1 images/s.

## Add one-pass wide transition wgrad, batched conv3x3 dW reduce, odd-tail dgrad variant

Adds a wide conv1x1 weight-gradient kernel for transition layers. It covers several 48-column output chunks per launch, so the input activations are streamed fewer times. It also defers the per-layer conv3x3 weight-gradient row reductions and issues them together as one batched reduce kernel per dense block, using host-built descriptor arrays. A third change adds an ODD template variant of the multi-layer dgrad kernel to handle an odd number of 16-channel tiles. Together these aim to cut redundant memory passes and kernel launches, in exchange for more scratch memory per layer and more template instantiations.

Result: no change. 566.9 images/s (-0.4%).

```diff
diff --git a/emlight_amd/RegressionNetwork/dense_engine_bwd.py b/emlight_amd/RegressionNetwork/dense_engine_bwd.py
--- a/emlight_amd/RegressionNetwork/dense_engine_bwd.py
+++ b/emlight_amd/RegressionNetwork/dense_engine_bwd.py
@@ -1,10 +1,14 @@
 import ctypes
 import os
 
+import numpy as np
 import torch
 
 from .. import _lib
 from .._knobs import knob_choice, knob_flag
+
+_REDUCE_DESC = np.dtype([("partial", "<u8"), ("dst", "<u8"), ("row_stride", "<u8"), ("rows", "<i4"), ("mode", "<i4"),
+                         ("dim0", "<i4"), ("dim1", "<i4"), ("n0", "<i4"), ("nblocks", "<i4")])
 
 
 def _r16(v):
@@ -39,6 +43,13 @@
 
 
 class _BwdBuffers:
+    def part_w2(self, i, grid):
+        while len(self.partW2) <= i:
+            self.partW2.append(None)
+        if self.partW2[i] is None or self.partW2[i].numel() < grid * 21 * 256:
+            self.partW2[i] = self._partW2_new(grid)
+        return self.partW2[i]
+
     def gf12(self, r):
         if self.GF12[r] is None:
             self.GF12[r] = self._gf12_new()
@@ -61,7 +72,13 @@
         self.permutes = None
         self.coef = torch.zeros(8, max(kp, ko), **f32)
         self.part2 = torch.zeros(2, g * kp * 2, dtype=torch.float64, device=dev)
-        self.partW = torch.empty(g * max(kp * 48, 2 * 27 * 256, 4 * 1024), **f32)
+        self.trans_onepass = knob_flag("EML_TRANS_WGRAD_ONEPASS", True)
+        wide = [_lib.lib().eml_dense_conv1x1_bwd_weight_wide_scratch_floats(g, blk["trans"]["Kp"], blk["trans"]["Cout"])
+                for blk in ws.blocks] if self.trans_onepass else []
+        self.partW = torch.empty(max([g * max(kp * 48, 2 * 27 * 256, 4 * 1024)] + wide), **f32)
+        self.dw2_batch = knob_flag("EML_C3_DW2_BATCH", True)
+        self.partW2 = []
+        self._partW2_new = lambda grid: torch.empty(grid * 21 * 256, **f32)
         i32 = dict(dtype=torch.int32, device=dev)
         self.cond = [[torch.zeros(lay["Kp"], **i32) for lay in blk["layers"]] for blk in ws.blocks]
         self.condT = [torch.zeros(blk["trans"]["Kp"], **i32) for blk in ws.blocks]
@@ -197,10 +214,15 @@
         _lib.check(L.eml_dense_bn_bwd_stats_f32(p(dY), ld_dy, p(tr["T"]), Ko, None, 0, 0, cout, Pn, p(tr["tmean"]),
                                                 p(tr["tistd"]), p(part), Gb, st), "eml_dense_bn_bwd_stats_f32")
         finalize(Gb, 2 * cout, Pn, LN, tr["tmean"], tr["tistd"], cout, Ko, coef=0)
-        _lib.check(L.eml_dense_conv1x1_bwd_weight_f32(
-            p(tr["A"]), kpt, Pn, Hb // 2, Wb // 2, 0, kpt, ctot, p(tr["one"]), p(tr["zero"]), p(dY), ld_dy, p(tr["T"]),
-            Ko, p(cA), p(cB), p(cC), cout, p(bw.partW), gr(T.conv.weight), G, None, None, 0, None, 0, None, None, st),
-            "eml_dense_conv1x1_bwd_weight_f32")
+        if bw.trans_onepass:
+            _lib.check(L.eml_dense_conv1x1_bwd_weight_wide_f32(
+                p(tr["A"]), kpt, Pn, kpt, ctot, p(tr["one"]), p(tr["zero"]), p(dY), ld_dy, p(tr["T"]), Ko, p(cA), p(cB),
+                p(cC), cout, p(bw.partW), bw.partW.numel(), gr(T.conv.weight), G, st), "eml_dense_conv1x1_bwd_weight_wide_f32")
+        else:
+            _lib.check(L.eml_dense_conv1x1_bwd_weight_f32(
+                p(tr["A"]), kpt, Pn, Hb // 2, Wb // 2, 0, kpt, ctot, p(tr["one"]), p(tr["zero"]), p(dY), ld_dy, p(tr["T"]),
+                Ko, p(cA), p(cB), p(cC), cout, p(bw.partW), gr(T.conv.weight), G, None, None, 0, None, 0, None, None, st),
+                "eml_dense_conv1x1_bwd_weight_f32")
         _lib.check(L.eml_dense_conv1x1_bwd_data_f32(
             p(dY), ld_dy, p(tr["T"]), Ko, p(cA), p(cB), p(cC), Ko, p(bw.WdT[bi]), None, ld, p(tr["scale"]),
             p(tr["shift"]), None, None, Pn, Hb, Wb, 1, kpt, p(Gbuf), ld, 0, p(part), G, p(tr["mask16"]), st),
@@ -223,9 +245,13 @@
             drop = (ws.drop_key, gl0 + l, q) if q > 0 else ()
             if fold:
                 fn = "eml_dense_conv3x3_bwd_fused_drop_f32" if drop else "eml_dense_conv3x3_bwd_fused_f32"
+                pw = bw.part_w2(len(dw2_pending), G3d) if bw.dw2_batch else bw.partW
                 _lib.check(getattr(L, fn)(*gsrc, p(Lm.conv2.weight), p(z), p(lay["zmean"]), p(lay["zistd"]), p(dz), B, Hb, Wb,
                                           p(part), G3d, p(blk["X"]), ld, cin, p(sB), p(sC), p(bw.gf12(r)) if c3_gf else None,
-                                          p(lay["scale2"]), p(lay["shift2"]), p(bw.partW), gr(Lm.conv2.weight), *drop, st), fn)
+                                          p(lay["scale2"]), p(lay["shift2"]), p(pw),
+                                          None if bw.dw2_batch else gr(Lm.conv2.weight), *drop, st), fn)
+                if bw.dw2_batch:
+                    dw2_pending.append((pw, grads[id(Lm.conv2.weight)]))
             else:
                 fn = "eml_dense_conv3x3_bwd_data_drop_f32" if drop else "eml_dense_conv3x3_bwd_data_f32"
                 _lib.check(getattr(L, fn)(*gsrc, p(Lm.conv2.weight), p(z), p(lay["zmean"]), p(lay["zistd"]), p(dz), B, Hb, Wb,
@@ -286,6 +312,7 @@
             dgamma_direct(blk, ld, P, Hb, Wb, 0, bw.DZ[slot], 48, None, 0, None, 48, Lm.conv1, lay["Cin"], lay["scale1"],
                           lay["shift1"], bw.cond[bi][l], Lm.norm1)
 
+        dw2_pending = []
         l = len(blk["layers"]) - 1
         have_top = False
         while l >= 0:
@@ -310,6 +337,12 @@
                 bn1_finalize(l, Lm0, 0, 0, blk["layers"][l]["Kp"])
                 bn1_direct(l, Lm0, 0)
                 l -= 1
+        for i in range(0, len(dw2_pending), 32):
+            host = np.zeros(len(dw2_pending[i:i + 32]), dtype=_REDUCE_DESC)
+            for j, (pw, dw) in enumerate(dw2_pending[i:i + 32]):
+                host[j] = (pw.data_ptr(), dw.data_ptr(), 21 * 256, G3d, 3, 0, 0, 0, 21 * 256 // 64)
+            _lib.check(L.eml_dense_reduce_rows_batch_f32(host.ctypes.data_as(ctypes.c_void_p), len(host), st),
+                       "eml_dense_reduce_rows_batch_f32")
         c0b = blk["C0"]
         norm0_fused = bi == 0 and knob_flag("EML_NORM0_FUSED", True) and c0b % 4 == 0 and c0b <= 32
         if not norm0_fused:
diff --git a/emlight_amd/_lib.py b/emlight_amd/_lib.py
--- a/emlight_amd/_lib.py
+++ b/emlight_amd/_lib.py
@@ -174,6 +174,11 @@
     "eml_dense_bn_dgamma_direct_f32": (_int, [_f32p, _int, ctypes.c_long, _int, _int, _int, _f32p, _int, _f32p, _int,
                                               _f32p, _f32p, _f32p, _int, _f32p, _int, _f32p, _f32p, _f32p, _f32p, _i32p,
                                               _f32p, _f32p, _int, _stream]),
+    "eml_dense_conv1x1_bwd_weight_wide_scratch_floats": (ctypes.c_size_t, [_int, _int, _int]),
+    "eml_dense_conv1x1_bwd_weight_wide_f32": (_int, [_f32p, _int, ctypes.c_long, _int, _int, _f32p, _f32p, _f32p, _int, _f32p,
+                                                     _int, _f32p, _f32p, _f32p, _int, _f32p, ctypes.c_size_t, _f32p, _int,
+                                                     _stream]),
+    "eml_dense_reduce_rows_batch_f32": (_int, [ctypes.c_void_p, _int, _stream]),
     "eml_dense_conv1x1_bwd_weight_f32": (_int, [_f32p, _int, ctypes.c_long, _int, _int, _int, _int, _int, _f32p,
                                                 _f32p, _f32p, _int, _f32p, _int, _f32p, _f32p, _f32p, _int, _f32p,
                                                 _f32p, _int, _f32p, _f32p, _int, _f32p, _int, _f32p, _f32p, _stream]),
diff --git a/emlight_amd/csrc/dense_bwd.hip b/emlight_amd/csrc/dense_bwd.hip
--- a/emlight_amd/csrc/dense_bwd.hip
+++ b/emlight_amd/csrc/dense_bwd.hip
@@ -1125,11 +1125,10 @@
   }
 }
 
-__global__ __launch_bounds__(256) void reduce_rows_kernel(const float* __restrict__ partial, int R, size_t row_stride,
-                                                          int mode, int dim0, int dim1, int n0,
-                                                          float* __restrict__ out) {
-  __shared__ double red[4][64];
-  const int tid = threadIdx.x, e = blockIdx.x * 64 + (tid & 63), slice = tid >> 6;
+__device__ __forceinline__ void reduce_rows_block(const float* __restrict__ partial, int R, size_t row_stride, int mode,
+                                                  int dim0, int dim1, int n0, float* __restrict__ out, int bx,
+                                                  double (&red)[4][64]) {
+  const int tid = threadIdx.x, e = bx * 64 + (tid & 63), slice = tid >> 6;
   size_t src = 0, dst = 0;
   bool valid = false;
   if (mode == 0) {
@@ -1161,6 +1160,24 @@
   red[slice][tid & 63] = s;
   __syncthreads();
   if (slice == 0 && valid) out[dst] = (float)((red[0][tid] + red[1][tid]) + (red[2][tid] + red[3][tid]));
+}
+__global__ __launch_bounds__(256) void reduce_rows_kernel(const float* __restrict__ partial, int R, size_t row_stride,
+                                                          int mode, int dim0, int dim1, int n0,
+                                                          float* __restrict__ out) {
+  __shared__ double red[4][64];
+  reduce_rows_block(partial, R, row_stride, mode, dim0, dim1, n0, out, blockIdx.x, red);
+}
+constexpr int kReduceBatchMax = 32;
+struct ReduceBatchArgs {
+  eml_reduce_desc d[kReduceBatchMax];
+};
+__global__ __launch_bounds__(256) void reduce_rows_batch_kernel(const ReduceBatchArgs args) {
+  __shared__ double red[4][64];
+  const eml_reduce_desc& d = args.d[blockIdx.y];
+  for (int bx = blockIdx.x; bx < d.nblocks; bx += gridDim.x) {
+    if (bx != (int)blockIdx.x) __syncthreads();
+    reduce_rows_block(d.partial, d.rows, (size_t)d.row_stride, d.mode, d.dim0, d.dim1, d.n0, d.dst, bx, red);
+  }
 }
 
 struct NarrowArgs {
@@ -1462,6 +1479,172 @@
       dst[0] = (red[tid] + red[12 + tid]) + (red[24 + tid] + red[36 + tid]);
       dst[1] = 0.0;
     }
+  }
+}
+
+template <int NT , int MAXG >
+__global__ __launch_bounds__(256, 1) void conv1x1_bwd_weight_wide_kernel(
+    const float* __restrict__ X, int ldx, int P, int Kp, const float* __restrict__ scale1, const float* __restrict__ shift1,
+    const float* __restrict__ DY, int ld_dy, const float* __restrict__ Zr, int ld_z, const float* __restrict__ cA,
+    const float* __restrict__ cB, const float* __restrict__ cC, int n_valid,
+    int n_load ,
+    float* __restrict__ partial , size_t chunk_stride ) {
+  constexpr int NCOL = 16 * NT;
+  constexpr int S = (NCOL % 32 == 0) ? NCOL + 16 : NCOL;
+  __shared__ __attribute__((aligned(16))) float dz_l[2][64 * S];
+  __shared__ __attribute__((aligned(16))) float co_l[3 * NCOL];
+  const int tid = threadIdx.x, lane = tid & 63, wave = tid >> 6;
+  const int r = lane & 15, kk = lane >> 4;
+  const int ngroups = (Kp + 31) / 32;
+
+  float sv[MAXG][2], tv[MAXG][2];
+  int coff[MAXG];
+  bool gv[MAXG];
+#pragma unroll
+  for (int i = 0; i < MAXG; ++i) {
+    const int cg = wave + 4 * i;
+    const int ch = 32 * cg + 2 * r;
+    gv[i] = cg < ngroups && ch < Kp;
+    coff[i] = gv[i] ? ch : 0;
+#pragma unroll
+    for (int t = 0; t < 2; ++t) {
+      sv[i][t] = gv[i] ? scale1[ch + t] : 0.f;
+      tv[i][t] = gv[i] ? shift1[ch + t] : 0.f;
+    }
+  }
+  const int spix = tid >> 2, sq = tid & 3;
+  for (int e = tid; e < NCOL; e += 256) {
+    const bool v = e < n_valid;
+    co_l[e] = v ? cA[e] : 0.f;
+    co_l[NCOL + e] = v ? cB[e] : 0.f;
+    co_l[2 * NCOL + e] = v ? cC[e] : 0.f;
+  }
+  __syncthreads();
+  f32x4 acc[MAXG][2][NT];
+#pragma unroll
+  for (int i = 0; i < MAXG; ++i)
+#pragma unroll
+    for (int t = 0; t < 2; ++t)
+#pragma unroll
+      for (int n = 0; n < NT; ++n) acc[i][t][n] = f32x4{0.f, 0.f, 0.f, 0.f};
+
+  const int nchunks = (P + 63) >> 6;
+  const int ngw = (ngroups > wave) ? (ngroups - wave + 3) >> 2 : 0;
+
+  float4 rdy[NT], rzr[NT];
+  bool rpv = false;
+  auto stage_load = [&](int chunk) {
+    const int p = chunk * 64 + spix;
+    rpv = chunk < nchunks && p < P;
+    const size_t pc = rpv ? p : 0;
+#pragma unroll
+    for (int j = 0; j < NT; ++j) {
+      const int col = 4 * (sq + 4 * j);
+      const bool cv = col < n_load;
+      rdy[j] = cv ? *reinterpret_cast<const float4*>(DY + pc * ld_dy + col) : make_float4(0.f, 0.f, 0.f, 0.f);
+      rzr[j] = cv ? *reinterpret_cast<const float4*>(Zr + pc * ld_z + col) : make_float4(0.f, 0.f, 0.f, 0.f);
+    }
+  };
+  auto stage_write = [&](float* dzb) {
+#pragma unroll
+    for (int j = 0; j < NT; ++j) {
+      const int col = 4 * (sq + 4 * j);
+      const float4 sa = *reinterpret_cast<const float4*>(co_l + col);
+      const float4 sb = *reinterpret_cast<const float4*>(co_l + NCOL + col);
+      const float4 sc = *reinterpret_cast<const float4*>(co_l + 2 * NCOL + col);
+      float4 v;
+      v.x = rpv ? fmaf(sa.x, rdy[j].x, fmaf(sb.x, rzr[j].x, sc.x)) : 0.f;
+      v.y = rpv ? fmaf(sa.y, rdy[j].y, fmaf(sb.y, rzr[j].y, sc.y)) : 0.f;
+      v.z = rpv ? fmaf(sa.z, rdy[j].z, fmaf(sb.z, rzr[j].z, sc.z)) : 0.f;
+      v.w = rpv ? fmaf(sa.w, rdy[j].w, fmaf(sb.w, rzr[j].w, sc.w)) : 0.f;
+      *reinterpret_cast<float4*>(dzb + spix * S + col) = v;
+    }
+  };
+  auto chunk_loop = [&](auto ngw_c) {
+    constexpr int NGW = decltype(ngw_c)::value;
+    constexpr int UQ = 4;
+    constexpr int NB = 16 / UQ;
+    float2 xr[2][UQ][NGW > 0 ? NGW : 1];
+    auto load_batch = [&](int chunk, int q0, float2 (&dst)[UQ][NGW > 0 ? NGW : 1]) {
+#pragma unroll
+      for (int u = 0; u < UQ; ++u) {
+        const int pc = min(chunk * 64 + 4 * (q0 + u) + kk, P - 1);
+        const float* xp = X + (size_t)pc * ldx;
+#pragma unroll
+        for (int i = 0; i < NGW; ++i) dst[u][i] = *reinterpret_cast<const float2*>(xp + coff[i]);
+      }
+    };
+    stage_load(blockIdx.x);
+    stage_write(dz_l[0]);
+    if constexpr (NGW > 0) load_batch(min((int)blockIdx.x, nchunks - 1), 0, xr[0]);
+    __syncthreads();
+    int it = 0;
+    for (int chunk = blockIdx.x; chunk < nchunks; chunk += gridDim.x, ++it) {
+      const float* dzb = dz_l[it & 1];
+      stage_load(chunk + gridDim.x);
+      if constexpr (NGW > 0) {
+        float bzq[2][NT];
+#pragma unroll
+        for (int n = 0; n < NT; ++n) bzq[0][n] = dzb[kk * S + 16 * n + r];
+#pragma unroll
+        for (int bi = 0; bi < NB; ++bi) {
+          const int q0 = bi * UQ;
+          if (bi + 1 < NB)
+            load_batch(chunk, q0 + UQ, xr[(bi + 1) & 1]);
+          else
+            load_batch(min(chunk + (int)gridDim.x, nchunks - 1), 0, xr[(bi + 1) & 1]);
+          __builtin_amdgcn_sched_barrier(0);
+#pragma unroll
+          for (int u = 0; u < UQ; ++u) {
+            const int pl = 4 * (q0 + u) + kk;
+            const bool pvu = chunk * 64 + pl < P;
+            float bz[NT];
+#pragma unroll
+            for (int n = 0; n < NT; ++n) bz[n] = bzq[(q0 + u) & 1][n];
+            if (q0 + u + 1 < 16) {
+#pragma unroll
+              for (int n = 0; n < NT; ++n) bzq[(q0 + u + 1) & 1][n] = dzb[(pl + 4) * S + 16 * n + r];
+            }
+#pragma unroll
+            for (int i = 0; i < NGW; ++i) {
+              const float2 xv = xr[bi & 1][u][i];
+              float av[2];
+              av[0] = 0.f + fmaxf(fmaf(xv.x, sv[i][0], tv[i][0]), 0.f);
+              av[1] = 0.f + fmaxf(fmaf(xv.y, sv[i][1], tv[i][1]), 0.f);
+              if (!pvu) av[0] = av[1] = 0.f;
+#pragma unroll
+              for (int n = 0; n < NT; ++n)
+#pragma unroll
+                for (int t = 0; t < 2; ++t) acc[i][t][n] = mfma16(av[t], bz[n], acc[i][t][n]);
+            }
+          }
+          __builtin_amdgcn_sched_barrier(0);
+        }
+      }
+      stage_write(dz_l[(it + 1) & 1]);
+      eml::lds_barrier();
+    }
+  };
+  switch (ngw) {
+    case 0: chunk_loop(std::integral_constant<int, 0>{}); break;
+    case 1: chunk_loop(std::integral_constant<int, 1>{}); break;
+    case 2: chunk_loop(std::integral_constant<int, (MAXG < 2 ? MAXG : 2)>{}); break;
+    default: chunk_loop(std::integral_constant<int, MAXG>{}); break;
+  }
+#pragma unroll
+  for (int i = 0; i < MAXG; ++i) {
+    const int cg = wave + 4 * i;
+#pragma unroll
+    for (int t = 0; t < 2; ++t)
+#pragma unroll
+      for (int g = 0; g < 4; ++g) {
+        const int ch = 32 * cg + 2 * (4 * kk + g) + t;
+        if (cg < ngroups && ch < Kp) {
+#pragma unroll
+          for (int n = 0; n < NT; ++n)
+            partial[(size_t)(n / 3) * chunk_stride + ((size_t)blockIdx.x * Kp + ch) * 48 + 16 * (n % 3) + r] = acc[i][t][n][g];
+        }
+      }
   }
 }
 
@@ -1897,7 +2080,7 @@
 };
 
 template <int NL, int MT , bool RAW = false ,
-          bool MASKED = false, bool TOP = false>
+          bool MASKED = false, bool TOP = false, bool ODD = false>
 __global__ __launch_bounds__(256, 2) void conv1x1_bwd_data_multi_kernel(BwdLayer L0, BwdLayer L1,
                                                                         const float* __restrict__ X, int ldx,
                                                                         const float* __restrict__ mean,
@@ -1930,17 +2113,18 @@
   constexpr int NCH = 2;
 
   float4 wq[2][3][NCH];
-  auto load_w = [&](int j, int nt0, float4 (&dst)[3][NCH]) {
+  auto load_w = [&](auto nc_c, int j, int nt0, float4 (&dst)[3][NCH]) {
+    constexpr int NC = decltype(nc_c)::value;
     const int nnt = Ls[j].Kp >> 4;
 #pragma unroll
     for (int jo = 0; jo < 3; ++jo)
 #pragma unroll
-      for (int n = 0; n < NCH; ++n) {
+      for (int n = 0; n < NC; ++n) {
         const int nt = min(nt0 + n, nnt - 1);
         dst[jo][n] = *reinterpret_cast<const float4*>(Ls[j].Wd + ((((size_t)nt * 3 + jo) * 4 + kk) * 16 + r) * 4);
       }
   };
-  load_w(0, nt_lo, wq[0]);
+  load_w(std::integral_constant<int, NCH>{}, 0, nt_lo, wq[0]);
   int wsel = 0;
 
   for (int tile = blockIdx.x; tile < ntiles; tile += gridDim.x) {
@@ -1979,10 +2163,11 @@
           }
         }
       }
-    for (int nt0 = nt_lo; nt0 < nt_hi; nt0 += NCH) {
-      float4 gs[MT][NCH], xv[MT][NCH];
-#pragma unroll
-      for (int n = 0; n < NCH; ++n) {
+    auto chunk = [&](auto nc_c, const int nt0) {
+      constexpr int NC = decltype(nc_c)::value;
+      float4 gs[MT][NC], xv[MT][NC];
+#pragma unroll
+      for (int n = 0; n < NC; ++n) {
         const int k4 = 16 * min(nt0 + n, nt_hi - 1) + 4 * kk;
         const int k4l = (k4 + 3 >= k_lo && k4 < k_hi) ? k4 : (k_lo & ~3);
 #pragma unroll
@@ -1991,17 +2176,17 @@
           if constexpr (!MASKED) xv[m][n] = *reinterpret_cast<const float4*>(X + prow[m] * ldx + k4l);
         }
       }
-      const int nt_next = nt0 + NCH < nt_hi ? nt0 + NCH : nt_lo;
+      const int nt_next = nt0 + NC < nt_hi ? nt0 + NC : nt_lo;
 #pragma unroll
       for (int j = 0; j < NL; ++j) {
         const int nnt = Ls[j].Kp >> 4;
-        unsigned long long mk[MT][NCH][4];
+        unsigned long long mk[MT][NC][4];
         if constexpr (MASKED) {
           const unsigned long long* __restrict__ Mj = j == 0 ? M0 : M1;
 #pragma unroll
           for (int m = 0; m < MT; ++m)
 #pragma unroll
-            for (int n = 0; n < NCH; ++n) {
+            for (int n = 0; n < NC; ++n) {
               const size_t wi =
                   ((size_t)__builtin_amdgcn_readfirstlane((p0 >> 4) + m) * nnt + min(nt0 + n, nnt - 1)) * 4;
 #pragma unroll
@@ -2010,27 +2195,27 @@
         }
         const int cur = NL == 2 ? j : wsel;
         if (j + 1 < NL)
-          load_w(j + 1, nt0, wq[cur ^ 1]);
+          load_w(nc_c, j + 1, nt0, wq[cur ^ 1]);
         else
-          load_w(0, nt_next, wq[cur ^ 1]);
+          load_w(std::integral_constant<int, NCH>{}, 0, nt_next, wq[cur ^ 1]);
         __builtin_amdgcn_sched_barrier(0);
-        f32x4 acc[MT][NCH];
+        f32x4 acc[MT][NC];
 #pragma unroll
         for (int m = 0; m < MT; ++m)
 #pragma unroll
-          for (int n = 0; n < NCH; ++n) acc[m][n] = f32x4{0.f, 0.f, 0.f, 0.f};
+          for (int n = 0; n < NC; ++n) acc[m][n] = f32x4{0.f, 0.f, 0.f, 0.f};
 #pragma unroll
         for (int jo = 0; jo < 3; ++jo)
 #pragma unroll
           for (int t = 0; t < 4; ++t)
 #pragma unroll
-            for (int n = 0; n < NCH; ++n)
+            for (int n = 0; n < NC; ++n)
 #pragma unroll
               for (int m = 0; m < MT; ++m) acc[m][n] = mfma16(f4c(wq[cur][jo][n], t), f4c(dz[j][jo][m], t), acc[m][n]);
         if (NL == 1) wsel ^= 1;
         double* my = sacc + ((size_t)(j * 4 + wave) * KpMax) * 2;
 #pragma unroll
-        for (int n = 0; n < NCH; ++n) {
+        for (int n = 0; n < NC; ++n) {
           const int nt = nt0 + n;
           if (nt < nnt && nt < nt_hi) {
             const int k4 = 16 * nt + 4 * kk;
@@ -2089,7 +2274,7 @@
         }
       }
 #pragma unroll
-      for (int n = 0; n < NCH; ++n) {
+      for (int n = 0; n < NC; ++n) {
         const int nt = nt0 + n;
         if (nt < nt_hi) {
           const int k4 = 16 * nt + 4 * kk;
@@ -2110,7 +2295,9 @@
           }
         }
       }
-    }
+    };
+    if constexpr (ODD) chunk(std::integral_constant<int, 1>{}, nt_lo);
+    for (int nt0 = nt_lo + (ODD ? 1 : 0); nt0 < nt_hi; nt0 += NCH) chunk(std::integral_constant<int, NCH>{}, nt0);
   }
   __syncthreads();
 #pragma unroll
@@ -2799,8 +2986,11 @@
                                     const float* scale2, const float* shift2, float* partialW, float* dW2, eml::DropKey dk,
                                     eml_stream_t stream) {
   if (!G || !W2 || !Z || !zmean || !zistd || !DZ || !partials || !X || !sB || !sC || !scale2 || !shift2 || !partialW ||
-      !dW2 || B < 1 || H < 1 || W < 1 || grid < 1 || cx < 0)
+      B < 1 || H < 1 || W < 1 || grid < 1 || cx < 0)
     return eml::fail(EML_EINVAL, "%s: bad arguments", name);
+#if defined(EML_C3_WTP) && !EML_C3_WTP
+  if (!dW2) return eml::fail(EML_EINVAL, "%s: dW2 == NULL (deferred fold) needs the tap-packed partial layout", name);
+#endif
   const auto al16 = [](const void* q) { return (reinterpret_cast<uintptr_t>(q) & 15) == 0; };
   if (!eml_dense_conv3x3_bwd_fused_supported(ldg, c0, ldx, cx) || !al16(G) || !al16(X) || !al16(GF) || !al16(Z) || !al16(scale2) ||
       !al16(shift2))
@@ -2833,7 +3023,7 @@
     }
   }
   int rc = eml::check_launch(name);
-  if (rc) return rc;
+  if (rc || !dW2) return rc;
   hipLaunchKernelGGL(reduce_rows_kernel, dim3(21 * 256 / 64), dim3(256), 0, (hipStream_t)stream, partialW, grid,
                      (size_t)21 * 256, 3, 0, 0, 0, dW2);
   return eml::check_launch(DROP ? "eml_dense_conv3x3_bwd_fused_drop_f32(reduce)" : "eml_dense_conv3x3_bwd_fused_f32(reduce)");
@@ -2891,6 +3081,23 @@
   return conv3x3_bwd_fused_launch<true>("eml_dense_conv3x3_bwd_fused_drop_f32", G, ldg, c0, W2, Z, zmean, zistd, DZ, B, H, W,
                                         partials, grid, X, ldx, cx, sB, sC, GF, scale2, shift2, partialW, dW2,
                                         eml_drop_key(seed, layer, p), stream);
+}
+
+extern "C" int eml_dense_reduce_rows_batch_f32(const eml_reduce_desc* descs, int n, eml_stream_t stream) {
+  if (!descs || n < 0 || n > kReduceBatchMax)
+    return eml::fail(EML_EINVAL, "eml_dense_reduce_rows_batch_f32: descs is NULL or n outside [0, %d]", kReduceBatchMax);
+  if (n == 0) return EML_OK;
+  ReduceBatchArgs args;
+  int gx = 1;
+  for (int i = 0; i < n; ++i) {
+    const eml_reduce_desc& d = descs[i];
+    if (!d.partial || !d.dst || d.rows < 1 || d.mode < 0 || d.mode > 3 || d.nblocks < 1 || d.dim0 < 0 || d.dim1 < 0 || d.n0 < 0)
+      return eml::fail(EML_EINVAL, "eml_dense_reduce_rows_batch_f32: bad descriptor %d", i);
+    args.d[i] = d;
+    gx = std::max(gx, std::min(d.nblocks, 128));
+  }
+  hipLaunchKernelGGL(reduce_rows_batch_kernel, dim3(gx, n), dim3(256), 0, (hipStream_t)stream, args);
+  return eml::check_launch("eml_dense_reduce_rows_batch_f32");
 }
 
 namespace {
@@ -3011,6 +3218,90 @@
   return EML_OK;
 }
 
+extern "C" size_t eml_dense_conv1x1_bwd_weight_wide_scratch_floats(int grid, int Kp, int Cout) {
+  if (grid < 1 || Kp < 1 || Cout < 1) return 0;
+  return (size_t)((Cout + 47) / 48) * grid * Kp * 48;
+}
+
+namespace {
+template <int NT, int MAXG>
+void launch_wgrad_wide(int grid, hipStream_t stream, const float* X, int ldx, int P, int Kp, const float* scale1,
+                       const float* shift1, const float* DY, int ld_dy, const float* Zr, int ld_z, const float* cA,
+                       const float* cB, const float* cC, int n_valid, int n_load, float* partial, size_t chunk_stride) {
+  hipLaunchKernelGGL((conv1x1_bwd_weight_wide_kernel<NT, MAXG>), dim3(grid), dim3(256), 0, stream, X, ldx, P, Kp, scale1,
+                     shift1, DY, ld_dy, Zr, ld_z, cA, cB, cC, n_valid, n_load, partial, chunk_stride);
+}
+}
+
+extern "C" int eml_dense_conv1x1_bwd_weight_wide_f32(const float* X, int ldx, long P, int Kp, int Cin, const float* scale1,
+                                                     const float* shift1, const float* DY, int ld_dy, const float* Zr,
+                                                     int ld_z, const float* cA, const float* cB, const float* cC, int Cout,
+                                                     float* partial, size_t partial_floats, float* dW, int grid,
+                                                     eml_stream_t stream) {
+  if (!X || !scale1 || !shift1 || !DY || !Zr || !cA || !cB || !cC || !partial || !dW || P < 1 || P > 0x7FFFFFFFl - 64 ||
+      grid < 1 || Kp < 32 || (Kp & 15) || Kp > 384 || Cin < 1 || Cin > Kp || ldx < Kp || (ldx & 1) || Cout < 1 || Cout > 192 ||
+      (ld_dy & 3) || (ld_z & 3))
+    return eml::fail(EML_EINVAL, "eml_dense_conv1x1_bwd_weight_wide_f32: bad arguments (32 <= Kp <= 384 a multiple of 16, "
+                                 "Cin <= Kp <= ldx, Cout <= 192, row lengths multiples of 4)");
+  const auto al16 = [](const void* q) { return (reinterpret_cast<uintptr_t>(q) & 15) == 0; };
+  if (!al16(DY) || !al16(Zr) || (reinterpret_cast<uintptr_t>(X) & 7))
+    return eml::fail(EML_EINVAL, "eml_dense_conv1x1_bwd_weight_wide_f32: DY / Zr need 16-byte, X 8-byte alignment");
+  const int ld_min = (ld_dy < ld_z ? ld_dy : ld_z) & ~3;
+  if (ld_min < Cout) return eml::fail(EML_EINVAL, "eml_dense_conv1x1_bwd_weight_wide_f32: DY/Zr rows narrower than Cout");
+  const size_t need = eml_dense_conv1x1_bwd_weight_wide_scratch_floats(grid, Kp, Cout);
+  if (partial_floats < need)
+    return eml::fail(EML_EINVAL, "eml_dense_conv1x1_bwd_weight_wide_f32: partial holds %zu floats, %zu needed "
+                                 "(eml_dense_conv1x1_bwd_weight_wide_scratch_floats)", partial_floats, need);
+  const size_t chunk_stride = (size_t)grid * Kp * 48;
+  const int nchunks = (Cout + 47) / 48, ntiles = (Cout + 15) / 16;
+  const bool g3 = Kp > 256;
+  const int cpd = g3 ? 2 : 3;
+  const hipStream_t hs = (hipStream_t)stream;
+  for (int c0 = 0; c0 < nchunks; c0 += cpd) {
+    const int col0 = 48 * c0;
+    const int nt = std::min(3 * cpd, ntiles - 3 * c0);
+    int n_load = ld_min - col0;
+    if (n_load > 16 * nt) n_load = 16 * nt;
+    float* pc = partial + (size_t)c0 * chunk_stride;
+#define EML_WIDE(NTV, MGV)                                                                                              \
+  launch_wgrad_wide<NTV, MGV>(grid, hs, X, ldx, (int)P, Kp, scale1, shift1, DY + col0, ld_dy, Zr + col0, ld_z, cA + col0, \
+                              cB + col0, cC + col0, Cout - col0, n_load, pc, chunk_stride)
+    if (g3) {
+      switch (nt) {
+        case 1: EML_WIDE(1, 3); break;
+        case 2: EML_WIDE(2, 3); break;
+        case 3: EML_WIDE(3, 3); break;
+        case 4: EML_WIDE(4, 3); break;
+        case 5: EML_WIDE(5, 3); break;
+        default: EML_WIDE(6, 3); break;
+      }
+    } else {
+      switch (nt) {
+        case 1: EML_WIDE(1, 2); break;
+        case 2: EML_WIDE(2, 2); break;
+        case 3: EML_WIDE(3, 2); break;
+        case 4: EML_WIDE(4, 2); break;
+        case 5: EML_WIDE(5, 2); break;
+        case 6: EML_WIDE(6, 2); break;
+        case 7: EML_WIDE(7, 2); break;
+        case 8: EML_WIDE(8, 2); break;
+        default: EML_WIDE(9, 2); break;
+      }
+    }
+#undef EML_WIDE
+    int rc = eml::check_launch("eml_dense_conv1x1_bwd_weight_wide_f32");
+    if (rc) return rc;
+  }
+  for (int ch = 0; ch < nchunks; ++ch) {
+    const int n0 = ch * 48, nv = (Cout - n0 < 48) ? Cout - n0 : 48;
+    hipLaunchKernelGGL(reduce_rows_kernel, dim3((Cin * 48 + 63) / 64), dim3(256), 0, hs, partial + (size_t)ch * chunk_stride,
+                       grid, (size_t)Kp * 48, 0, Cin, nv, n0, dW);
+    int rc = eml::check_launch("eml_dense_conv1x1_bwd_weight_wide_f32(reduce)");
+    if (rc) return rc;
+  }
+  return EML_OK;
+}
+
 extern "C" int eml_dense_permute_w1_bwd_f32(const float* W, int Cout, int Cin, int Kp, int Ko, float* Wd,
                                             eml_stream_t stream) {
   if (!W || !Wd || Cout < 1 || Cin < 1 || Kp < Cin || (Kp & 15) || Ko < Cout || (Ko & 15))
@@ -3109,27 +3400,32 @@
   if (((k_hi + 15) & ~15) > kmax) return eml::fail(EML_EINVAL, "eml_dense_conv1x1_bwd_data_multi_f32: range beyond Kp");
   const size_t lds = (size_t)n_layers * 4 * kmax * 2 * sizeof(double) + (size_t)(2 + 2 * n_layers) * kmax * sizeof(float);
   if (lds > 80 * 1024) return eml::fail(EML_EINVAL, "eml_dense_conv1x1_bwd_data_multi_f32: Kp=%d does not fit LDS", kmax);
-#define EML_LAUNCH_MULTI(NLV, MTV, RAWV, MSKV)                                                                       \
+  static const int tail = [] { const char* v = getenv("EML_DGRAD_TAIL"); return (v && v[0] == '0') ? 0 : 1; }();
+  const bool odd = tail && ((((k_hi + 15) >> 4) - (k_lo >> 4)) & 1);
+#define EML_LAUNCH_MULTI_(NLV, MTV, RAWV, MSKV, TOPV, ODDV)                                                         \
   do {                                                                                                              \
-    EML_ENSURE_LDS((&conv1x1_bwd_data_multi_kernel<NLV, MTV, RAWV, MSKV>), lds);                                 \
-    hipLaunchKernelGGL((conv1x1_bwd_data_multi_kernel<NLV, MTV, RAWV, MSKV>), dim3(grid), dim3(256), lds,            \
+    EML_ENSURE_LDS((&conv1x1_bwd_data_multi_kernel<NLV, MTV, RAWV, MSKV, TOPV, ODDV>), lds);                     \
+    hipLaunchKernelGGL((conv1x1_bwd_data_multi_kernel<NLV, MTV, RAWV, MSKV, TOPV, ODDV>), dim3(grid), dim3(256), lds, \
                        (hipStream_t)stream, L[0], L[1], X, ldx, mean, istd, (int)P, k_lo, k_hi, G, ldg, kmax,        \
-                       Mk[0], Mk[1], (float*)nullptr);                                                              \
+                       Mk[0], Mk[1], top);                                                                          \
+  } while (0)
+#define EML_LAUNCH_MULTI(NLV, MTV, RAWV, MSKV, TOPV)                                                                \
+  do {                                                                                                              \
+    if (odd) EML_LAUNCH_MULTI_(NLV, MTV, RAWV, MSKV, TOPV, true);                                                   \
+    else EML_LAUNCH_MULTI_(NLV, MTV, RAWV, MSKV, TOPV, false);                                                      \
   } while (0)
   if (n_layers == 1) {
-    if (relu_masks) EML_LAUNCH_MULTI(1, 4, true, true);
-    else if (raw) EML_LAUNCH_MULTI(1, 4, true, false);
-    else EML_LAUNCH_MULTI(1, 4, false, false);
+    if (relu_masks) EML_LAUNCH_MULTI(1, 4, true, true, false);
+    else if (raw) EML_LAUNCH_MULTI(1, 4, true, false, false);
+    else EML_LAUNCH_MULTI(1, 4, false, false, false);
   } else if (top) {
-    EML_ENSURE_LDS((&conv1x1_bwd_data_multi_kernel<2, 2, true, true, true>), lds);
-    hipLaunchKernelGGL((conv1x1_bwd_data_multi_kernel<2, 2, true, true, true>), dim3(grid), dim3(256), lds,
-                       (hipStream_t)stream, L[0], L[1], X, ldx, mean, istd, (int)P, k_lo, k_hi, G, ldg, kmax, Mk[0], Mk[1],
-                       top);
+    EML_LAUNCH_MULTI(2, 2, true, true, true);
   } else {
-    if (relu_masks) EML_LAUNCH_MULTI(2, 2, true, true);
-    else if (raw) EML_LAUNCH_MULTI(2, 2, true, false);
-    else EML_LAUNCH_MULTI(2, 2, false, false);
-  }
+    if (relu_masks) EML_LAUNCH_MULTI(2, 2, true, true, false);
+    else if (raw) EML_LAUNCH_MULTI(2, 2, true, false, false);
+    else EML_LAUNCH_MULTI(2, 2, false, false, false);
+  }
+#undef EML_LAUNCH_MULTI_
 #undef EML_LAUNCH_MULTI
   return eml::check_launch("eml_dense_conv1x1_bwd_data_multi_f32");
 }
diff --git a/include/emlight_hip.h b/include/emlight_hip.h
--- a/include/emlight_hip.h
+++ b/include/emlight_hip.h
@@ -170,6 +170,14 @@
                                          const float* shift2, float* partialW, float* dW2, unsigned long long seed,
                                          int layer, double p, eml_stream_t stream);
 
+typedef struct eml_reduce_desc {
+  const float* partial;
+  float* dst;
+  uint64_t row_stride;
+  int32_t rows, mode, dim0, dim1, n0, nblocks;
+} eml_reduce_desc;
+int eml_dense_reduce_rows_batch_f32(const eml_reduce_desc* descs, int n, eml_stream_t stream);
+
 int eml_dense_conv3x3_bwd_weight_f32(const float* G, int ldg, int c0, const float* Z,
                                      const float* scale2, const float* shift2, int B, int H, int W,
                                      float* partial, float* dW2, int grid, eml_stream_t stream);
@@ -195,6 +203,13 @@
                                      float* partial, float* dW, int grid, float* dz_out,
                                      const float* W1, int k_lo, const float* G, int ldg, float* N12,
                                      double* partials_n, eml_stream_t stream);
+
+size_t eml_dense_conv1x1_bwd_weight_wide_scratch_floats(int grid, int Kp, int Cout);
+int eml_dense_conv1x1_bwd_weight_wide_f32(const float* X, int ldx, long P, int Kp, int Cin, const float* scale1,
+                                          const float* shift1, const float* DY, int ld_dy, const float* Zr,
+                                          int ld_z, const float* cA, const float* cB, const float* cC, int Cout,
+                                          float* partial, size_t partial_floats, float* dW, int grid,
+                                          eml_stream_t stream);
 
 int eml_dense_permute_w1_bwd_f32(const float* W, int Cout, int Cin, int Kp, int Ko, float* Wd,
                                  eml_stream_t stream);
```
